# BUTSpeechFIT/TS-ASR-Whisper

Measured on AMD Instinct MI355X. Metric: train utterances/sec (30 s clips) whisper-large-v3-turbo DiCoW, higher is better.
Workload: dtype bf16; 1 GPU; whisper-large-v3-turbo DiCoW fine-tune step, per-GPU batch 16, L=128, decoder frozen, bf16 AMP; global_batch=16, parallelism=dp1, split_streams=False, trainable_params=637306880

## Files before the change

include/dicow_hip.h:

```cpp
#ifndef DICOW_HIP_H
#define DICOW_HIP_H

#include <stdint.h>

#ifdef __cplusplus
extern "C" {
#endif

#define DICOW_OK 0
#define DICOW_ERR_INVALID (-1)
#define DICOW_ERR_LAUNCH (-2)

#define DICOW_ABI_VERSION 7

int dicow_abi_version(void);
int dicow_set_gemm_cus(int n);
int dicow_gemm_dispatch_log(char* buf, int cap);
const char* dicow_last_error(void);

int dicow_cast_f32_to_bf16(const float* src, void* dst, int64_t n, void* stream);
int dicow_cast_transpose_f32_to_bf16(const float* src, void* dst, int64_t ld, void* dst_t, int64_t ld_t, int R, int C,
                                     void* stream);
#define DICOW_CAST_GROUP_MAX 8
typedef struct { const float* src; void* dst; void* dst_t; int R, C; int64_t ld, ld_t; } dicow_cast_problem;
// ... 172 lines not shown
    float* dq_colsum; float* dv_colsum; void* cs_ws; int64_t cs_ws_bytes;
    int q_log2;
    void* fused_ws; int64_t fused_ws_bytes;
    int fused_mode;
} dicow_attn_bwd_args;
int dicow_attn_bwd(const dicow_attn_bwd_args* a, void* stream);
int64_t dicow_attn_bwd_colsum_ws_bytes(int B, int H, int Lq, int Lk);
int64_t dicow_attn_bwd_fused_ws_bytes(int B, int H, int Lq, int Lk);
const char* dicow_attn_bwd_route(const dicow_attn_bwd_args* a);
int dicow_attn_bwd_fused_eligible(int B, int H, int Lq, int Lk, int causal, int fused_mode);
int dicow_attn_bwd_fused_status(const void* fused_ws);


typedef struct {
    const void* logits; int64_t ld; int rows; int V;
    const int64_t* labels; const int64_t* upp_labels;
    int soft;
    const int32_t* ts_index;
    const int32_t* ts_ids;
    const float* ts_w;
    int n_ts;
    float* lse; float* row_loss; int32_t* choice;
    float* loss_sum; float* count;
    void* d_logits;
} dicow_ce_args;
int dicow_ce_loss_fwd(const dicow_ce_args* a, void* stream);
int dicow_ce_loss_bwd(const dicow_ce_args* a, const float* grad_scale, void* stream);

typedef struct {
    const void* logits; int64_t ld; int B, Tn, C;
    const int64_t* labels; int Lc; int blank;
    float* lse;
    float* alpha; float* beta;
    int Smax;
    float* nll; float* tlen;
    float* loss_sum;
    void* d_logits;
} dicow_ctc_args;
int64_t dicow_ctc_ws_bytes(int B, int Tn, int Lc);
int dicow_ctc_loss_fwd(const dicow_ctc_args* a, void* stream);
int dicow_ctc_loss_bwd(const dicow_ctc_args* a, const float* grad_scale, void* stream);

int dicow_embed_fwd(const int64_t* ids, const float* tok, const float* pos, float* out, int B, int Lq, int D, void* stream);
int dicow_embed_bwd(const int64_t* ids, const float* g, float* d_tok, float* d_pos, int B, int Lq, int D, void* stream);

int dicow_gelu_bwd_bf16(const void* g, const void* pre, void* out, int64_t n, void* stream);
int dicow_conv2_col2im_gelu_bwd(const void* dA2, const void* pre1, void* d_pre1, int B, int T2, int C, void* stream);

int64_t dicow_logmel_ws_bytes(int B, int n_samples);
int dicow_logmel(const float* wave, int B, int n_samples, const float* tw_cos, const float* tw_sin, const float* fb,
                 const int* mel_range, int M, float* out, void* ws, int64_t ws_bytes, void* stream);

#define DICOW_NOISE_MIX_CHUNK 8192
int64_t dicow_noise_mix_ws_bytes(int n_plan, int max_len);
int dicow_noise_mix(const float* wave, int64_t ld_wave, float* out, int64_t ld_out, const float* bank, const int64_t* clip_start,
                    const int* clip_len, const int* plan_i, const float* plan_snr, int n_plan, void* ws, int64_t ws_bytes, void* stream);

#define DICOW_DIAR_FRAME 320
#define DICOW_DIAR_BIN 1600
#define DICOW_DIAR_WINDOW 300
#define DICOW_DIAR_MAX_SPEAKERS 64
int64_t dicow_diar_table_ws_bytes(int E);
int64_t dicow_diar_targets_ws_bytes(int n_targets);
int64_t dicow_enrollment_windows_ws_bytes(int64_t n_samples, int n_targets);
int dicow_diar_frame_counts(const int64_t* bounds, const uint64_t* active, int E, int S, int64_t n_samples, int32_t* cnt, int32_t* excl,
                            void* ws, int64_t ws_bytes, void* stream);
int dicow_stno_from_counts(const int32_t* cnt, int S, int64_t n_samples, const int* targets, int n_targets, float* out, int64_t ld_out,
                           void* ws, int64_t ws_bytes, void* stream);
int dicow_enrollment_windows(const int32_t* cnt, const int32_t* excl, int S, int64_t n_samples, const int* targets, int n_targets,
                             int32_t* start, int32_t* count, int32_t* fallback, int32_t* weights, int64_t ld_w, void* ws, int64_t ws_bytes,
                             void* stream);

#define DICOW_ENR_MIX_MAX_TRACKS 8
int dicow_enrollment_mix(float* out, int64_t ld_out, int B, int n, const float* bank, const int64_t* clip_start, const int32_t* plan_dev,
                         const int32_t* plan_host, int n_tracks, const int32_t* clip_len_host, int n_clips, void* stream);

#define DICOW_RESAMPLE_LDS_BYTES 49152
#define DICOW_RESAMPLE_MAX_RATIO 1048576
#define DICOW_RESAMPLE_MAX_CHANNELS 512
int64_t dicow_resample_ws_bytes(int n_segs, int n);
int dicow_resample(const void* in, int in_int16, int C, int channel, int64_t in_frames, float* out, int64_t out_samples, const float* taps_t,
                   const int32_t* first, int o, int n, int width, int S, const int64_t* segs, int n_segs, int frames_per_tile, void* ws,
                   int64_t ws_bytes, void* stream);

#define DICOW_EDIT_MAX_LEN 65535
#define DICOW_EDIT_K 8
#define DICOW_EDIT_LANES 512
#define DICOW_EDIT_LANES_NARROW 64
int64_t dicow_edit_distance_ws_bytes(const int64_t* pairs, int n_pairs);
int dicow_edit_distance(const int32_t* ref_ids, int64_t n_ref, const int32_t* hyp_ids, int64_t n_hyp, const int32_t* ref_iv, const int32_t* hyp_iv,
                        const int64_t* pairs, int n_pairs, int32_t* out, int lanes, int along, void* ws, int64_t ws_bytes, void* stream);

#define DICOW_ORC_MAX_STREAMS 8
#define DICOW_ORC_K 8
#define DICOW_ORC_MAX_WORDS 65527
#define DICOW_ORC_MAX_STATES 4194304
#define DICOW_ORC_MAX_WS_BYTES 1073741824LL
#define DICOW_ORC_DESC_BYTES 288
#define DICOW_ORC_UTT_BYTES 16
int64_t dicow_orc_distance_ws_bytes(const int64_t* problems, int n_problems, const int64_t* utts, const int64_t* streams, int want_assignment);
int dicow_orc_distance(const int32_t* ref_ids, int64_t n_ref, const int32_t* hyp_ids, int64_t n_hyp, const int32_t* ref_iv, const int32_t* hyp_iv,
                       const int64_t* problems, int n_problems, const int64_t* utts, const int64_t* streams, int32_t* out, int32_t* assignment,
                       void* ws, int64_t ws_bytes, void* stream);

#define DICOW_DIAR_SCORE_CHUNK 256
#define DICOW_DIAR_SCORE_ROW 12
#define DICOW_DIAR_SCORE_OUT_WORDS 4232
#define DICOW_DIAR_SCORE_DESC_BYTES 120
#define DICOW_DIAR_SCORE_MAX_E 16777216
#define DICOW_DIAR_SCORE_MAX_TICK 1099511627776LL
#define DICOW_DIAR_SCORE_MAX_WS_BYTES 4294967296LL
int64_t dicow_diar_score_ws_bytes(const int64_t* bounds, int64_t n_bounds, const uint64_t* active, int64_t n_active, const int64_t* unscored,
                                  int64_t n_unscored, const int64_t* problems, int n_problems, int chunk);
int dicow_diar_score(const int64_t* bounds, int64_t n_bounds, const uint64_t* active, int64_t n_active, const int64_t* unscored,
                     int64_t n_unscored, const int64_t* problems, int n_problems, int chunk, int64_t* out, void* ws, int64_t ws_bytes,
                     void* stream);

int dicow_stno_noise_rescale(float* stno, const int* rows, const float* noise, int n_rows, int C, int T, float sd,
                             void* stream);
int dicow_stno_segment_augment(float* stno, const int* segs, const float* coef, int n_seg, int C, int T, void* stream);
int dicow_specaug_joint(const float* mel, const float* stno, float* mel_out, float* stno_out, int B, int M, int T, int sub,
                        int center, int warped, const int* fmask, int n_fmask, const int* tmask, int n_tmask,
                        int n_maskable, void* stream);

typedef struct {
    const void* logits; int in_bf16; int64_t ld; const float* lse; const int* alias;
    const int* rows; const int* cs; const int* decoded_len; const int* last; const float* r_prev;
    float* psi; float* r;
    int n, C, T, blank, eos;
} dicow_ctc_prefix_args;
int dicow_ctc_frame_lse(const void* logits, int in_bf16, int64_t rows, int V1, int64_t ld, float* lse, void* stream);
int dicow_ctc_prefix_init(const void* logits, int in_bf16, int64_t ld, const float* lse, int B, int T, int blank_col, float* r0,
                          void* stream);
int dicow_ctc_prefix_score(const dicow_ctc_prefix_args* a, void* stream);

int dicow_whisper_timestamp_rules(float* scores, int64_t ld, int B, int V, const int64_t* input_ids, int L, int begin_index,
                                  int timestamp_begin, int eos, int no_timestamps, int max_initial_timestamp_index,
                                  int detect_from_logprob, void* stream);

int dicow_repetition_rules(float* scores, int64_t ld, int rows, int V, const int64_t* input_ids, int64_t ids_stride, int L,
                           float penalty, int ngram, void* stream);

int dicow_ctc_greedy_decode(const void* logits, int in_bf16, int64_t batch_stride, int64_t ld, int B, int Tn, int V1, int64_t blank,
                            int64_t pad_id, int* ws, int64_t* out, int64_t out_stride, void* stream);

int dicow_sumsq_f32(const float* x, int64_t n, float* out, void* stream);
int dicow_fabric_emulate(void* buf, int64_t bytes, double gbps, int workgroups, int passes, void* stream);
int dicow_adamw_f32(float* p, const float* g, float* m, float* v, int64_t n, float lr, float beta1, float beta2,
                    float eps, float weight_decay, int step, const float* gnorm_sq, float max_norm, void* stream);
int dicow_adamw_hyper(int* counters, float* hyper, const int* is_pre, int n_runs, int preheat_only, double lr, double mult,
                      int warmup_steps, int max_steps, int cosine, double beta1, double beta2, void* stream);
int dicow_adamw_f32_dev(float* p, const float* g, float* m, float* v, int64_t n, const float* hyper, float beta1, float beta2,
                        float eps, float weight_decay, const float* gnorm_sq, float max_norm, void* stream);

#define DICOW_MT_CHUNK 2048
#define DICOW_MT_MAX_CLASSES 32
#define DICOW_MT_ALIGNED_ALL 1
#define DICOW_MT_ALIGNED_G   2
typedef struct {
    float* p; float* g; float* m; float* v;
    int64_t n;
    int32_t cls;
    int32_t flags;
} dicow_mt_tensor;
typedef struct { int64_t start; int32_t tensor; int32_t len; } dicow_mt_chunk;
typedef struct {
    float decay[DICOW_MT_MAX_CLASSES]; float step_size[DICOW_MT_MAX_CLASSES]; float bc2_sqrt[DICOW_MT_MAX_CLASSES];
    float lerp_w[DICOW_MT_MAX_CLASSES]; float beta2[DICOW_MT_MAX_CLASSES]; float one_minus_beta2[DICOW_MT_MAX_CLASSES];
    float eps[DICOW_MT_MAX_CLASSES];
    int32_t n_classes;
} dicow_mt_adamw_classes;
int dicow_multi_chunk_elems(void);
int dicow_multi_adamw_f32(const dicow_mt_tensor* tensors, const dicow_mt_chunk* chunks, int64_t n_chunks,
                          const dicow_mt_adamw_classes* cls, int cls_base, const float* clip_coef, void* stream);
int64_t dicow_multi_sumsq_ws_bytes(int64_t n_chunks);
int dicow_multi_sumsq_f32(const dicow_mt_tensor* tensors, const dicow_mt_chunk* chunks, int64_t n_chunks, void* ws, int64_t ws_bytes,
                          float* out, float max_norm, void* stream);
int dicow_multi_scale_f32(const dicow_mt_tensor* tensors, const dicow_mt_chunk* chunks, int64_t n_chunks, const float* coef, void* stream);


#ifdef DICOW_EXPERIMENTAL_ABI
#define DICOW_EPI_LNSTAT  2048
#define DICOW_EPI_LNFOLD  4096
#define DICOW_LN_SLOTS 16
int dicow_gemm_nt_lnstat_ok(const dicow_gemm_args* a);
int dicow_lnfold_prep(const float* W, const float* gamma, const float* beta, const float* bias, void* Wf, int64_t ldw, float* c, float* bf,
                      int N, int K, void* stream);
#endif

#ifdef __cplusplus
}
#endif
#endif
```

ts-asr-whisper_amd/_lib.py:

```python
import ctypes as C
import os

_HERE = os.path.dirname(os.path.abspath(__file__))
LIB_PATH = os.environ.get("DICOW_HIP_LIB") or os.path.join(_HERE, "libdicow_hip.so")
_lib = None

c_vp, c_i, c_i64, c_f, c_d = C.c_void_p, C.c_int, C.c_int64, C.c_float, C.c_double


class FddtLnFwdArgs(C.Structure):
    _fields_ = [("h_in", c_vp), ("in_bf16", c_i), ("mode", c_i), ("stno", c_vp), ("stno_bstride", c_i64),
                ("w", c_vp * 4), ("b", c_vp * 4), ("pos", c_vp), ("h_out", c_vp), ("ln_w", c_vp), ("ln_b", c_vp),
                ("y_bf16", c_vp), ("y_f32", c_vp), ("mean", c_vp), ("rstd", c_vp),
                ("rows", c_i), ("T", c_i), ("D", c_i), ("eps", c_f)]


class FddtLnBwdArgs(C.Structure):
    _fields_ = [("h_in", c_vp), ("in_bf16", c_i), ("mode", c_i), ("stno", c_vp), ("stno_bstride", c_i64),
                ("w", c_vp * 4), ("b", c_vp * 4), ("pos", c_vp), ("ln_w", c_vp), ("mean", c_vp), ("rstd", c_vp),
                ("d_y", c_vp), ("dy_f32", c_i), ("g_res", c_vp), ("g_out", c_vp), ("g_out_bf16", c_vp),
                ("dln_w", c_vp), ("dln_b", c_vp), ("dw", c_vp * 4), ("db", c_vp * 4), ("colsum_out", c_vp),
                ("dpos_rows", c_vp), ("rows", c_i), ("T", c_i), ("D", c_i), ("ws", c_vp), ("ws_bytes", c_i64)]


class GemmArgs(C.Structure):
    _fields_ = [("A", c_vp), ("B", c_vp), ("C", c_vp), ("bias", c_vp), ("residual", c_vp), ("aux", c_vp),
                ("M", c_i), ("N", c_i), ("K", c_i),
                ("lda", c_i64), ("ldb", c_i64), ("ldc", c_i64), ("ldr", c_i64), ("ldaux", c_i64),
                ("batch", c_i), ("strideA", c_i64), ("strideB", c_i64), ("strideC", c_i64), ("strideAux", c_i64),
                ("flags", c_i), ("scale", c_f), ("scale_ncols", c_i),
                ("colsum_out", c_vp), ("colsum_ws", c_vp), ("colsum_ws_bytes", c_i64),
                ("fddt_w", c_vp * 4), ("fddt_b", c_vp * 4), ("fddt_rowmask", c_vp),
                ("lnstat", c_vp), ("ln_c", c_vp), ("ln_inv_dim", c_f), ("ln_eps", c_f), ("ln_nslots", c_i)]


class GemmTnArgs(C.Structure):
    _fields_ = [("A", c_vp), ("B", c_vp), ("C", c_vp), ("Mk", c_i), ("N1", c_i), ("N2", c_i),
                ("lda", c_i64), ("ldb", c_i64), ("ldc", c_i64),
                ("batch", c_i), ("strideA", c_i64), ("strideB", c_i64), ("accumulate", c_i),
                ("C_seg", c_vp * 2), ("seg_rows", c_i), ("ws", c_vp), ("ws_bytes", c_i64)]


TN_GROUP_MAX = 24
CAST_GROUP_MAX = 8


class CastProblem(C.Structure):
    _fields_ = [("src", c_vp), ("dst", c_vp), ("dst_t", c_vp), ("R", c_i), ("C", c_i), ("ld", c_i64), ("ld_t", c_i64)]


class GemmTnGroupArgs(C.Structure):
    _fields_ = [("n", c_i), ("p", GemmTnArgs * TN_GROUP_MAX), ("ws", c_vp), ("ws_bytes", c_i64)]


class AttnFwdArgs(C.Structure):
    _fields_ = [("q", c_vp), ("k", c_vp), ("v", c_vp), ("o", c_vp), ("lse", c_vp),
                ("q_bs", c_i64), ("q_rs", c_i64), ("k_bs", c_i64), ("k_rs", c_i64),
                ("v_bs", c_i64), ("v_rs", c_i64), ("o_bs", c_i64), ("o_rs", c_i64),
                ("B", c_i), ("H", c_i), ("Lq", c_i), ("Lk", c_i), ("causal", c_i), ("q_log2", c_i)]


class AttnDecodeArgs(C.Structure):
    _fields_ = [("q", c_vp), ("o", c_vp), ("k", c_vp), ("v", c_vp),
                ("q_rs", c_i64), ("o_rs", c_i64), ("k_bs", c_i64), ("k_rs", c_i64), ("v_bs", c_i64), ("v_rs", c_i64),
                ("anc", c_vp), ("anc_rs", c_i64), ("R", c_i), ("H", c_i), ("Lk", c_i), ("group", c_i), ("n_slots", c_i)]


ATTN_DECODE_MAX_GROUP = 8

NOISE_MIX_CHUNK = 8192

DIAR_FRAME, DIAR_BIN, DIAR_WINDOW, DIAR_MAX_SPEAKERS = 320, 1600, 300, 64

ENR_MIX_MAX_TRACKS = 8

RESAMPLE_LDS_BYTES, RESAMPLE_MAX_RATIO, RESAMPLE_MAX_CHANNELS = 49152, 1 << 20, 512

EDIT_MAX_LEN, EDIT_K, EDIT_LANES, EDIT_LANES_NARROW = 65535, 8, 512, 64

ORC_MAX_STREAMS, ORC_K, ORC_MAX_WORDS, ORC_MAX_STATES, ORC_MAX_WS_BYTES, ORC_DESC_BYTES, ORC_UTT_BYTES = 8, 8, 65527, 1 << 22, 1 << 30, 288, 16

DIAR_SCORE_CHUNK, DIAR_SCORE_ROW, DIAR_SCORE_OUT_WORDS, DIAR_SCORE_DESC_BYTES = 256, 12, 4232, 120
DIAR_SCORE_MAX_E, DIAR_SCORE_MAX_TICK, DIAR_SCORE_MAX_WS_BYTES = 1 << 24, 1 << 40, 1 << 32

LORA_MAX_R, LORA_MAX_SEG = 192, 24
LORA_BLOCK, LORA_OUT_F32, LORA_GELU, LORA_MUL_AUX = 1, 2, 4, 8


class LoraDownArgs(C.Structure):
    _fields_ = [("X", c_vp), ("V", c_vp), ("T", c_vp), ("ldx", c_i64), ("ldv", c_i64), ("ldt", c_i64),
                ("M", c_i), ("K", c_i), ("R", c_i), ("r", c_i), ("flags", c_i)]


class LoraUpArgs(C.Structure):
    _fields_ = [("T", c_vp), ("U", c_vp), ("P", c_vp), ("Y", c_vp), ("aux", c_vp),
                ("ldt", c_i64), ("ldu", c_i64), ("ldp", c_i64), ("ldy", c_i64), ("ldaux", c_i64),
                ("M", c_i), ("N", c_i), ("R", c_i), ("r", c_i), ("flags", c_i), ("seg_scale", c_f * LORA_MAX_SEG)]


class LoraWgradArgs(C.Structure):
    _fields_ = [("T", c_vp), ("P", c_vp), ("G", c_vp * LORA_MAX_SEG), ("ldt", c_i64), ("ldp", c_i64), ("g_rs", c_i64), ("g_cs", c_i64),
                ("M", c_i), ("N", c_i), ("R", c_i), ("r", c_i), ("flags", c_i), ("scale", c_f), ("accumulate", c_i),
                ("ws", c_vp), ("ws_bytes", c_i64)]


class AttnBwdArgs(C.Structure):
    _fields_ = [("q", c_vp), ("k", c_vp), ("v", c_vp), ("o", c_vp), ("d_o", c_vp), ("lse", c_vp), ("delta", c_vp),
                ("dq", c_vp), ("dk", c_vp), ("dv", c_vp),
                ("q_bs", c_i64), ("q_rs", c_i64), ("k_bs", c_i64), ("k_rs", c_i64), ("v_bs", c_i64), ("v_rs", c_i64),
                ("o_bs", c_i64), ("o_rs", c_i64), ("do_bs", c_i64), ("do_rs", c_i64),
                ("dq_bs", c_i64), ("dq_rs", c_i64), ("dk_bs", c_i64), ("dk_rs", c_i64), ("dv_bs", c_i64), ("dv_rs", c_i64),
                ("B", c_i), ("H", c_i), ("Lq", c_i), ("Lk", c_i), ("causal", c_i), ("dq_scale", c_f),
                ("dq_colsum", c_vp), ("dv_colsum", c_vp), ("cs_ws", c_vp), ("cs_ws_bytes", c_i64), ("q_log2", c_i),
                ("fused_ws", c_vp), ("fused_ws_bytes", c_i64), ("fused_mode", c_i)]


class CeArgs(C.Structure):
    _fields_ = [("logits", c_vp), ("ld", c_i64), ("rows", c_i), ("V", c_i), ("labels", c_vp), ("upp_labels", c_vp),
                ("soft", c_i), ("ts_index", c_vp), ("ts_ids", c_vp), ("ts_w", c_vp), ("n_ts", c_i),
                ("lse", c_vp), ("row_loss", c_vp), ("choice", c_vp), ("loss_sum", c_vp), ("count", c_vp),
                ("d_logits", c_vp)]


class CtcArgs(C.Structure):
    _fields_ = [("logits", c_vp), ("ld", c_i64), ("B", c_i), ("Tn", c_i), ("C", c_i), ("labels", c_vp), ("Lc", c_i),
                ("blank", c_i), ("lse", c_vp), ("alpha", c_vp), ("beta", c_vp), ("Smax", c_i), ("nll", c_vp), ("tlen", c_vp),
                ("loss_sum", c_vp), ("d_logits", c_vp)]


class CtcPrefixArgs(C.Structure):
    _fields_ = [("logits", c_vp), ("in_bf16", c_i), ("ld", c_i64), ("lse", c_vp), ("alias", c_vp), ("rows", c_vp), ("cs", c_vp),
                ("decoded_len", c_vp), ("last", c_vp), ("r_prev", c_vp), ("psi", c_vp), ("r", c_vp), ("n", c_i), ("C", c_i),
                ("T", c_i), ("blank", c_i), ("eos", c_i)]


MT_MAX_CLASSES = 32


class MtAdamwClasses(C.Structure):
    _fields_ = [("decay", c_f * MT_MAX_CLASSES), ("step_size", c_f * MT_MAX_CLASSES), ("bc2_sqrt", c_f * MT_MAX_CLASSES),
                ("lerp_w", c_f * MT_MAX_CLASSES), ("beta2", c_f * MT_MAX_CLASSES), ("one_minus_beta2", c_f * MT_MAX_CLASSES),
                ("eps", c_f * MT_MAX_CLASSES), ("n_classes", C.c_int32)]


EPI_BIAS, EPI_GELU, EPI_RESIDUAL, EPI_OUT_F32, EPI_SCALE_N, EPI_GELU_BWD, EPI_ACCUM = 1, 2, 4, 8, 16, 32, 64
EPI_GELU_DAUX, EPI_MUL_AUX, EPI_COLSUM, EPI_FDDT = 128, 256, 512, 1024
EPI_LNSTAT, EPI_LNFOLD, LN_SLOTS = 2048, 4096, 16

_SIGS = {
    "dicow_set_gemm_cus": [c_i],
    "dicow_cast_transpose_group": [C.POINTER(CastProblem), c_i, c_vp],
    "dicow_gemm_dispatch_log": [c_vp, c_i],
    "dicow_cast_f32_to_bf16": [c_vp, c_vp, c_i64, c_vp],
    "dicow_cast_transpose_f32_to_bf16": [c_vp, c_vp, c_i64, c_vp, c_i64, c_i, c_i, c_vp],
    "dicow_conv_weight_pack": [c_vp, c_vp, c_vp, c_i, c_i, c_i, c_vp],
    "dicow_conv_weight_unpack_grad": [c_vp, c_vp, c_i, c_i, c_i, c_vp],
    "dicow_mel_to_timemajor": [c_vp, c_vp, c_i, c_i, c_i, c_vp],
    "dicow_colsum_bf16": [c_vp, c_i64, c_vp, c_i, c_i, c_vp, c_i64, c_vp],
    "dicow_sum_over_batch": [c_vp, c_vp, c_i, c_i64, c_vp],
    "dicow_scb_split": [c_vp, c_vp, c_vp, c_vp, c_i64, c_i, c_i, c_i, c_vp],
    "dicow_scb_merge_fwd": [c_vp, c_vp, c_vp, c_vp, c_i, c_i, c_i, c_vp],
    "dicow_scb_gate_bwd": [c_vp, c_vp, c_vp, c_vp, c_vp, c_i, c_i, c_i, c_vp, c_i64, c_vp],
    "dicow_scb_merge_bwd": [c_vp, c_vp, c_vp, c_i64, c_vp, c_vp, c_i, c_i, c_i, c_vp],
    "dicow_fddt_ln_fwd": [C.POINTER(FddtLnFwdArgs), c_vp],
    "dicow_fddt_ln_bwd": [C.POINTER(FddtLnBwdArgs), c_vp],
    "dicow_fddt_full_combine_fwd": [c_vp, c_vp, c_i, c_vp, c_i64, c_i, c_vp, c_i, c_i, c_i, c_vp],
    "dicow_fddt_full_combine_bwd": [c_vp, c_vp, c_i64, c_i, c_vp, c_vp, c_i, c_i, c_i, c_vp],
    "dicow_gemm_nt": [C.POINTER(GemmArgs), c_vp],
    "dicow_gemm_nt_is_persistent": [C.POINTER(GemmArgs)],
    "dicow_gemm_tn": [C.POINTER(GemmTnArgs), c_vp],
    "dicow_gemm_tn_group": [C.POINTER(GemmTnGroupArgs), c_vp],
    "dicow_attn_fwd": [C.POINTER(AttnFwdArgs), c_vp],
    "dicow_attn_decode": [C.POINTER(AttnDecodeArgs), c_vp],
    "dicow_lora_down": [C.POINTER(LoraDownArgs), c_vp],
    "dicow_lora_up": [C.POINTER(LoraUpArgs), c_vp],
    "dicow_lora_wgrad": [C.POINTER(LoraWgradArgs), c_vp],
    "dicow_attn_bwd": [C.POINTER(AttnBwdArgs), c_vp],
    "dicow_attn_bwd_fused_status": [c_vp],
    "dicow_attn_bwd_fused_eligible": [c_i, c_i, c_i, c_i, c_i, c_i],
    "dicow_ce_loss_fwd": [C.POINTER(CeArgs), c_vp],
    "dicow_ce_loss_bwd": [C.POINTER(CeArgs), c_vp, c_vp],
    "dicow_ctc_loss_fwd": [C.POINTER(CtcArgs), c_vp],
    "dicow_ctc_loss_bwd": [C.POINTER(CtcArgs), c_vp, c_vp],
    "dicow_embed_fwd": [c_vp, c_vp, c_vp, c_vp, c_i, c_i, c_i, c_vp],
    "dicow_embed_bwd": [c_vp, c_vp, c_vp, c_vp, c_i, c_i, c_i, c_vp],
    "dicow_gelu_bwd_bf16": [c_vp, c_vp, c_vp, c_i64, c_vp],
    "dicow_conv2_col2im_gelu_bwd": [c_vp, c_vp, c_vp, c_i, c_i, c_i, c_vp],
    "dicow_logmel": [c_vp, c_i, c_i, c_vp, c_vp, c_vp, c_vp, c_i, c_vp, c_vp, c_i64, c_vp],
    "dicow_stno_noise_rescale": [c_vp, c_vp, c_vp, c_i, c_i, c_i, c_f, c_vp],
    "dicow_stno_segment_augment": [c_vp, c_vp, c_vp, c_i, c_i, c_i, c_vp],
    "dicow_specaug_joint": [c_vp, c_vp, c_vp, c_vp, c_i, c_i, c_i, c_i, c_i, c_i, c_vp, c_i, c_vp, c_i, c_i, c_vp],
    "dicow_ctc_frame_lse": [c_vp, c_i, c_i64, c_i, c_i64, c_vp, c_vp],
    "dicow_ctc_prefix_init": [c_vp, c_i, c_i64, c_vp, c_i, c_i, c_i, c_vp, c_vp],
    "dicow_ctc_prefix_score": [C.POINTER(CtcPrefixArgs), c_vp],
    "dicow_whisper_timestamp_rules": [c_vp, c_i64, c_i, c_i, c_vp, c_i, c_i, c_i, c_i, c_i, c_i, c_i, c_vp],
    "dicow_repetition_rules": [c_vp, c_i64, c_i, c_i, c_vp, c_i64, c_i, c_f, c_i, c_vp],
    "dicow_ctc_greedy_decode": [c_vp, c_i, c_i64, c_i64, c_i, c_i, c_i, c_i64, c_i64, c_vp, c_vp, c_i64, c_vp],
    "dicow_noise_mix": [c_vp, c_i64, c_vp, c_i64, c_vp, c_vp, c_vp, c_vp, c_vp, c_i, c_vp, c_i64, c_vp],
    "dicow_diar_frame_counts": [c_vp, c_vp, c_i, c_i, c_i64, c_vp, c_vp, c_vp, c_i64, c_vp],
    "dicow_stno_from_counts": [c_vp, c_i, c_i64, c_vp, c_i, c_vp, c_i64, c_vp, c_i64, c_vp],
    "dicow_enrollment_windows": [c_vp, c_vp, c_i, c_i64, c_vp, c_i, c_vp, c_vp, c_vp, c_vp, c_i64, c_vp, c_i64, c_vp],
    "dicow_enrollment_mix": [c_vp, c_i64, c_i, c_i, c_vp, c_vp, c_vp, c_vp, c_i, c_vp, c_i, c_vp],
    "dicow_resample": [c_vp, c_i, c_i, c_i, c_i64, c_vp, c_i64, c_vp, c_vp, c_i, c_i, c_i, c_i, c_vp, c_i, c_i, c_vp, c_i64, c_vp],
    "dicow_edit_distance": [c_vp, c_i64, c_vp, c_i64, c_vp, c_vp, c_vp, c_i, c_vp, c_i, c_i, c_vp, c_i64, c_vp],
    "dicow_orc_distance": [c_vp, c_i64, c_vp, c_i64, c_vp, c_vp, c_vp, c_i, c_vp, c_vp, c_vp, c_vp, c_vp, c_i64, c_vp],
    "dicow_diar_score": [c_vp, c_i64, c_vp, c_i64, c_vp, c_i64, c_vp, c_i, c_i, c_vp, c_vp, c_i64, c_vp],
    "dicow_sumsq_f32": [c_vp, c_i64, c_vp, c_vp],
    "dicow_fabric_emulate": [c_vp, c_i64, c_d, c_i, c_i, c_vp],
    "dicow_adamw_f32": [c_vp, c_vp, c_vp, c_vp, c_i64, c_f, c_f, c_f, c_f, c_f, c_i, c_vp, c_f, c_vp],
    "dicow_adamw_hyper": [c_vp, c_vp, c_vp, c_i, c_i, c_d, c_d, c_i, c_i, c_i, c_d, c_d, c_vp],
    "dicow_adamw_f32_dev": [c_vp, c_vp, c_vp, c_vp, c_i64, c_vp, c_f, c_f, c_f, c_f, c_vp, c_f, c_vp],
    "dicow_multi_chunk_elems": [],
    "dicow_multi_adamw_f32": [c_vp, c_vp, c_i64, C.POINTER(MtAdamwClasses), c_i, c_vp, c_vp],
    "dicow_multi_sumsq_f32": [c_vp, c_vp, c_i64, c_vp, c_i64, c_vp, c_f, c_vp],
    "dicow_multi_scale_f32": [c_vp, c_vp, c_i64, c_vp, c_vp],
}


_SIGS_EXPERIMENTAL = {
    "dicow_gemm_nt_lnstat_ok": [C.POINTER(GemmArgs)],
    "dicow_lnfold_prep": [c_vp, c_vp, c_vp, c_vp, c_vp, c_i64, c_vp, c_vp, c_i, c_i, c_vp],
}


class DicowError(RuntimeError):
    pass


def lib():
    global _lib
    if _lib is None:
        if not os.path.exists(LIB_PATH):
            raise DicowError(f"{LIB_PATH} is missing: build it with ts-asr-whisper_amd/csrc/build.sh "
                             "(or __graft_entry__.build()); there is no CPU fallback")
        l = C.CDLL(LIB_PATH)
        l.dicow_abi_version.restype = c_i
        l.dicow_last_error.restype = C.c_char_p
        for name, at in _SIGS.items():
            fn = getattr(l, name)
            fn.argtypes = at
            fn.restype = c_i
        for name, at in _SIGS64.items():
            fn = getattr(l, name)
            fn.argtypes = at
            fn.restype = c_i64
        for name, at in _SIGS_STR.items():
            fn = getattr(l, name)
            fn.argtypes = at
            fn.restype = C.c_char_p
        l._dicow_experimental = True
        for name, at in _SIGS_EXPERIMENTAL.items():
            try:
                fn = getattr(l, name)
            except AttributeError:
                l._dicow_experimental = False
                continue
            fn.argtypes = at
            fn.restype = c_i
        _lib = l
    return _lib


def has_experimental():
    return bool(lib()._dicow_experimental)


_SIGS64 = {
    "dicow_colsum_ws_bytes": [c_i, c_i],
    "dicow_gemm_nt_colsum_ws_bytes": [c_i, c_i],
    "dicow_attn_bwd_colsum_ws_bytes": [c_i, c_i, c_i, c_i],
    "dicow_attn_bwd_fused_ws_bytes": [c_i, c_i, c_i, c_i],
    "dicow_fddt_ln_bwd_ws_bytes": [c_i, c_i],
    "dicow_gemm_tn_ws_bytes": [C.POINTER(GemmTnArgs)],
    "dicow_gemm_nt_splitk_ws_bytes": [C.POINTER(GemmArgs)],
    "dicow_gemm_tn_group_ws_bytes": [C.POINTER(GemmTnGroupArgs)],
    "dicow_logmel_ws_bytes": [c_i, c_i],
    "dicow_scb_gate_bwd_ws_bytes": [],
    "dicow_ctc_ws_bytes": [c_i, c_i, c_i],
    "dicow_multi_sumsq_ws_bytes": [c_i64],
    "dicow_lora_wgrad_ws_bytes": [c_i, c_i, c_i, c_i, c_i],
    "dicow_noise_mix_ws_bytes": [c_i, c_i],
    "dicow_diar_table_ws_bytes": [c_i],
    "dicow_diar_targets_ws_bytes": [c_i],
    "dicow_enrollment_windows_ws_bytes": [c_i64, c_i],
    "dicow_resample_ws_bytes": [c_i, c_i],
    "dicow_edit_distance_ws_bytes": [c_vp, c_i],
    "dicow_orc_distance_ws_bytes": [c_vp, c_i, c_vp, c_vp, c_i],
    "dicow_diar_score_ws_bytes": [c_vp, c_i64, c_vp, c_i64, c_vp, c_i64, c_vp, c_i, c_i],
}


_SIGS_STR = {
    "dicow_fddt_ln_fwd_route": [C.POINTER(FddtLnFwdArgs)],
    "dicow_fddt_ln_bwd_route": [C.POINTER(FddtLnBwdArgs)],
    "dicow_attn_fwd_route": [C.POINTER(AttnFwdArgs)],
    "dicow_attn_bwd_route": [C.POINTER(AttnBwdArgs)],
}


def declared_symbols():
    return ["dicow_abi_version", "dicow_last_error"] + list(_SIGS) + list(_SIGS64) + list(_SIGS_STR)


def check(rc, what):
    if rc != 0:
        raise DicowError(f"{what} failed ({rc}): {lib().dicow_last_error().decode()}")


def ptr(t):
    return None if t is None else t.data_ptr()


def stream():
    import torch
    return torch.cuda.current_stream().cuda_stream


def call(name, *args):
    check(getattr(lib(), name)(*args), name)


def call_struct(name, st):
    check(getattr(lib(), name)(C.byref(st), stream()), name)
```

ts-asr-whisper_amd/csrc/elementwise.hip:

```cpp
#include <stdarg.h>
#include "common.h"

static thread_local char g_err[512] = "";

void dicow_set_error(const char* fmt, ...) {
    va_list ap;
    va_start(ap, fmt);
    vsnprintf(g_err, sizeof(g_err), fmt, ap);
    va_end(ap);
}

extern "C" int dicow_abi_version(void) { return DICOW_ABI_VERSION; }
extern "C" const char* dicow_last_error(void) { return g_err; }

__global__ void cast_f32_bf16_kernel(const float* __restrict__ src, unsigned short* __restrict__ dst, int64_t n) {
    const int64_t n4 = n >> 2;
    const int64_t stride = (int64_t)gridDim.x * blockDim.x;
    for (int64_t i = (int64_t)blockIdx.x * blockDim.x + threadIdx.x; i < n4; i += stride) {
        const float4 v = reinterpret_cast<const float4*>(src)[i];
        reinterpret_cast<uint2*>(dst)[i] = make_uint2(pack_bf16x2(v.x, v.y), pack_bf16x2(v.z, v.w));
    }
    for (int64_t i = (n4 << 2) + (int64_t)blockIdx.x * blockDim.x + threadIdx.x; i < n; i += stride)
        dst[i] = f2bfbits(src[i]);
}
// ... 358 lines not shown
    const int64_t id = ids[row];
    const float* gr = g + (int64_t)row * D;
    for (int i = threadIdx.x; i < D; i += blockDim.x) {
        const float v = gr[i];
        if (d_tok) atomicAdd(d_tok + id * D + i, v);
        if (d_pos) atomicAdd(d_pos + (int64_t)l * D + i, v);
    }
}

extern "C" int dicow_embed_bwd(const int64_t* ids, const float* g, float* d_tok, float* d_pos, int B, int Lq, int D, void* stream) {
    DICOW_REQUIRE(ids && g && B > 0 && Lq > 0 && D > 0, "embed_bwd: bad args");
    if (!d_tok && !d_pos) return DICOW_OK;
    hipLaunchKernelGGL(embed_bwd_kernel, dim3(B * Lq), dim3(256), 0, (hipStream_t)stream, ids, g, d_tok, d_pos, Lq, D);
    DICOW_CHECK_LAUNCH("embed_bwd");
    return DICOW_OK;
}

__global__ void gelu_bwd_bf16_kernel(const unsigned short* __restrict__ g, const unsigned short* __restrict__ pre,
                                     unsigned short* __restrict__ out, int64_t n) {
    const int64_t n4 = n >> 2;
    for (int64_t i = (int64_t)blockIdx.x * blockDim.x + threadIdx.x; i < n4; i += (int64_t)gridDim.x * blockDim.x) {
        const uint2 a = reinterpret_cast<const uint2*>(g)[i], b = reinterpret_cast<const uint2*>(pre)[i];
        const float r0 = __uint_as_float(a.x << 16) * gelu_erf_grad(__uint_as_float(b.x << 16));
        const float r1 = __uint_as_float(a.x & 0xffff0000u) * gelu_erf_grad(__uint_as_float(b.x & 0xffff0000u));
        const float r2 = __uint_as_float(a.y << 16) * gelu_erf_grad(__uint_as_float(b.y << 16));
        const float r3 = __uint_as_float(a.y & 0xffff0000u) * gelu_erf_grad(__uint_as_float(b.y & 0xffff0000u));
        reinterpret_cast<uint2*>(out)[i] = make_uint2(pack_bf16x2(r0, r1), pack_bf16x2(r2, r3));
    }
}

extern "C" int dicow_gelu_bwd_bf16(const void* g, const void* pre, void* out, int64_t n, void* stream) {
    DICOW_REQUIRE(g && pre && out && n > 0 && n % 4 == 0, "gelu_bwd_bf16: bad args (n %% 4)");
    int grid = (int)((n / 4 + 255) / 256); if (grid > 8192) grid = 8192;
    hipLaunchKernelGGL(gelu_bwd_bf16_kernel, dim3(grid), dim3(256), 0, (hipStream_t)stream, (const unsigned short*)g,
                       (const unsigned short*)pre, (unsigned short*)out, n);
    DICOW_CHECK_LAUNCH("gelu_bwd_bf16");
    return DICOW_OK;
}

__global__ void conv2_col2im_gelu_bwd_kernel(const unsigned short* __restrict__ dA2, const unsigned short* __restrict__ pre1,
                                             unsigned short* __restrict__ d_pre1, int T2, int C) {
    const int b = blockIdx.y, s = blockIdx.x;
    const int p = s + 1;
    const unsigned short* base = dA2 + (int64_t)b * T2 * 3 * C;
    const unsigned short* src0 = nullptr; const unsigned short* src1 = nullptr;
    if (p & 1) {
        const int t = (p - 1) >> 1;
        if (t < T2) src0 = base + (int64_t)t * 3 * C + C;
    } else {
        const int t = p >> 1;
        if (t < T2) src0 = base + (int64_t)t * 3 * C;
        if (t - 1 >= 0) src1 = base + (int64_t)(t - 1) * 3 * C + 2 * C;
    }
    const int64_t off = ((int64_t)b * 2 * T2 + s) * C;
    for (int c = threadIdx.x * 2; c < C; c += blockDim.x * 2) {
        float g0 = 0.f, g1 = 0.f;
        if (src0) { const unsigned u = *reinterpret_cast<const unsigned*>(src0 + c); g0 += __uint_as_float(u << 16); g1 += __uint_as_float(u & 0xffff0000u); }
        if (src1) { const unsigned u = *reinterpret_cast<const unsigned*>(src1 + c); g0 += __uint_as_float(u << 16); g1 += __uint_as_float(u & 0xffff0000u); }
        if (pre1) {
            const unsigned pu = *reinterpret_cast<const unsigned*>(pre1 + off + c);
            g0 *= gelu_erf_grad(__uint_as_float(pu << 16));
            g1 *= gelu_erf_grad(__uint_as_float(pu & 0xffff0000u));
        }
        *reinterpret_cast<unsigned*>(d_pre1 + off + c) = pack_bf16x2(g0, g1);
    }
}

extern "C" int dicow_conv2_col2im_gelu_bwd(const void* dA2, const void* pre1, void* d_pre1, int B, int T2, int C, void* stream) {
    DICOW_REQUIRE(dA2 && d_pre1 && B > 0 && T2 > 0 && C % 2 == 0, "conv2_col2im_gelu_bwd: bad args");
    hipLaunchKernelGGL(conv2_col2im_gelu_bwd_kernel, dim3(2 * T2, B), dim3(256), 0, (hipStream_t)stream,
                       (const unsigned short*)dA2, (const unsigned short*)pre1, (unsigned short*)d_pre1, T2, C);
    DICOW_CHECK_LAUNCH("conv2_col2im_gelu_bwd");
    return DICOW_OK;
}

#define SUMSQ_MAX_BLOCKS 2048
__device__ float g_sumsq_part[SUMSQ_MAX_BLOCKS];
__device__ unsigned g_sumsq_ticket = 0;

__global__ void __launch_bounds__(256) sumsq_kernel(const float* __restrict__ x, int64_t n, float* __restrict__ out) {
    __shared__ float red[4];
    __shared__ bool last;
    float s = 0.f;
    const int64_t n4 = n >> 2;
    for (int64_t i = (int64_t)blockIdx.x * blockDim.x + threadIdx.x; i < n4; i += (int64_t)gridDim.x * blockDim.x) {
        const float4 v = reinterpret_cast<const float4*>(x)[i];
        s += v.x * v.x + v.y * v.y + v.z * v.z + v.w * v.w;
    }
    for (int64_t i = (n4 << 2) + (int64_t)blockIdx.x * blockDim.x + threadIdx.x; i < n; i += (int64_t)gridDim.x * blockDim.x)
        s += x[i] * x[i];
    s = wave_sum(s);
    if ((threadIdx.x & 63) == 0) red[threadIdx.x >> 6] = s;
    __syncthreads();
    if (threadIdx.x == 0) {
        g_sumsq_part[blockIdx.x] = (red[0] + red[1]) + (red[2] + red[3]);
        __threadfence();
        last = atomicAdd(&g_sumsq_ticket, 1u) == gridDim.x - 1;
    }
    __syncthreads();
    if (!last) return;
    __threadfence();
    float t = 0.f;
    for (int i = threadIdx.x; i < (int)gridDim.x; i += 256) t += __builtin_nontemporal_load(&g_sumsq_part[i]);
    t = wave_sum(t);
    if ((threadIdx.x & 63) == 0) red[threadIdx.x >> 6] = t;
    __syncthreads();
    if (threadIdx.x == 0) {
        out[0] += (red[0] + red[1]) + (red[2] + red[3]);
        g_sumsq_ticket = 0;
    }
}

__global__ void __launch_bounds__(256) fabric_emulate_kernel(f32x4_t* buf, int64_t n16, double ticks_per_f4_per_block, int passes) {
    const int64_t per = (n16 + gridDim.x - 1) / gridDim.x, lo = per * blockIdx.x, hi = lo + per < n16 ? lo + per : n16;
    const long long t0 = wall_clock64();
    int64_t done = 0;
    for (int p = 0; p < passes; ++p)
        for (int64_t i = lo; i < hi; i += 256 * 16) {
            f32x4_t v[16];
#pragma unroll
            for (int k = 0; k < 16; ++k) { const int64_t j = i + k * 256 + threadIdx.x; if (j < hi) v[k] = __builtin_nontemporal_load(buf + j); }
#pragma unroll
            for (int k = 0; k < 16; ++k) { const int64_t j = i + k * 256 + threadIdx.x; if (j < hi) __builtin_nontemporal_store(v[k], buf + j); }
            done += (hi - i < 256 * 16 ? hi - i : 256 * 16);
            const long long due = t0 + (long long)((double)done * ticks_per_f4_per_block / passes);
            while (wall_clock64() < due) __builtin_amdgcn_s_sleep(32);
        }
}

extern "C" int dicow_fabric_emulate(void* buf, int64_t bytes, double gbps, int workgroups, int passes, void* stream) {
    DICOW_REQUIRE(buf && bytes > 0 && bytes % 16 == 0 && gbps > 0.0 && workgroups > 0 && workgroups <= 1024 && passes > 0 && passes <= 8,
                  "fabric_emulate: bad arguments");
    const int64_t n16 = bytes / 16;
    const double ticks_total = (double)bytes / (gbps * 1e9) * 1e8;
    const double per_block_f4 = (double)((n16 + workgroups - 1) / workgroups);
    hipLaunchKernelGGL(fabric_emulate_kernel, dim3(workgroups), dim3(256), 0, (hipStream_t)stream, reinterpret_cast<f32x4_t*>(buf), n16,
                       ticks_total / per_block_f4, passes);
    DICOW_CHECK_LAUNCH("fabric_emulate");
    return DICOW_OK;
}

extern "C" int dicow_sumsq_f32(const float* x, int64_t n, float* out, void* stream) {
    DICOW_REQUIRE(x && out && n > 0, "sumsq_f32: bad args");
    int grid = (int)((n / 4 + 255) / 256); if (grid < 1) grid = 1; if (grid > SUMSQ_MAX_BLOCKS) grid = SUMSQ_MAX_BLOCKS;
    hipLaunchKernelGGL(sumsq_kernel, dim3(grid), dim3(256), 0, (hipStream_t)stream, x, n, out);
    DICOW_CHECK_LAUNCH("sumsq_f32");
    return DICOW_OK;
}

#ifndef ADAMW_NT
#define ADAMW_NT 0
#endif
typedef __attribute__((ext_vector_type(4))) float f32x4a_t;
__global__ void adamw_kernel(float* __restrict__ p, const float* __restrict__ g, float* __restrict__ m, float* __restrict__ v,
                             int64_t n, float lr, float b1, float b2, float eps, float wd, float bc1, float bc2,
                             const float* __restrict__ gnorm_sq, float max_norm, const float* __restrict__ hyper) {
    if (hyper) { lr = hyper[0]; bc1 = hyper[1]; bc2 = hyper[2]; }
    float clip = 1.f;
    if (gnorm_sq && max_norm > 0.f) {
        const float c = max_norm / (sqrtf(gnorm_sq[0]) + 1e-6f);
        clip = c < 1.f ? c : 1.f;
    }
    const int64_t n4 = n >> 2;
    for (int64_t i = (int64_t)blockIdx.x * blockDim.x + threadIdx.x; i < n4; i += (int64_t)gridDim.x * blockDim.x) {
        float4 pp, gg, mm, vv;
        if (ADAMW_NT & 1) {
            const f32x4a_t p_ = __builtin_nontemporal_load(reinterpret_cast<const f32x4a_t*>(p) + i), g_ = __builtin_nontemporal_load(reinterpret_cast<const f32x4a_t*>(g) + i);
            const f32x4a_t m_ = __builtin_nontemporal_load(reinterpret_cast<const f32x4a_t*>(m) + i), v_ = __builtin_nontemporal_load(reinterpret_cast<const f32x4a_t*>(v) + i);
            pp = make_float4(p_.x, p_.y, p_.z, p_.w); gg = make_float4(g_.x, g_.y, g_.z, g_.w);
            mm = make_float4(m_.x, m_.y, m_.z, m_.w); vv = make_float4(v_.x, v_.y, v_.z, v_.w);
        } else {
            pp = reinterpret_cast<float4*>(p)[i]; gg = reinterpret_cast<const float4*>(g)[i];
            mm = reinterpret_cast<float4*>(m)[i]; vv = reinterpret_cast<float4*>(v)[i];
        }
        float* pa = &pp.x; float* ga = &gg.x; float* ma = &mm.x; float* va = &vv.x;
#pragma unroll
        for (int e = 0; e < 4; ++e) {
            const float gr = ga[e] * clip;
            pa[e] *= 1.f - lr * wd;
            ma[e] = b1 * ma[e] + (1.f - b1) * gr;
            va[e] = b2 * va[e] + (1.f - b2) * gr * gr;
            const float denom = sqrtf(va[e]) / sqrtf(bc2) + eps;
            pa[e] -= (lr / bc1) * (ma[e] / denom);
        }
        if (ADAMW_NT & 2) {
            __builtin_nontemporal_store(f32x4a_t{pp.x, pp.y, pp.z, pp.w}, reinterpret_cast<f32x4a_t*>(p) + i);
            __builtin_nontemporal_store(f32x4a_t{mm.x, mm.y, mm.z, mm.w}, reinterpret_cast<f32x4a_t*>(m) + i);
            __builtin_nontemporal_store(f32x4a_t{vv.x, vv.y, vv.z, vv.w}, reinterpret_cast<f32x4a_t*>(v) + i);
        } else {
            reinterpret_cast<float4*>(p)[i] = pp; reinterpret_cast<float4*>(m)[i] = mm; reinterpret_cast<float4*>(v)[i] = vv;
        }
    }
    for (int64_t i = (n4 << 2) + (int64_t)blockIdx.x * blockDim.x + threadIdx.x; i < n; i += (int64_t)gridDim.x * blockDim.x) {
        const float gr = g[i] * clip;
        float pv = p[i] * (1.f - lr * wd);
        const float mv = b1 * m[i] + (1.f - b1) * gr, vv2 = b2 * v[i] + (1.f - b2) * gr * gr;
        pv -= (lr / bc1) * (mv / (sqrtf(vv2) / sqrtf(bc2) + eps));
        p[i] = pv; m[i] = mv; v[i] = vv2;
    }
}

extern "C" int dicow_adamw_f32(float* p, const float* g, float* m, float* v, int64_t n, float lr, float beta1, float beta2,
                               float eps, float weight_decay, int step, const float* gnorm_sq, float max_norm, void* stream) {
    DICOW_REQUIRE(p && g && m && v && n > 0 && step >= 1, "adamw_f32: bad args");
    const float bc1 = 1.f - powf(beta1, (float)step), bc2 = 1.f - powf(beta2, (float)step);
    int grid = (int)((n / 4 + 255) / 256); if (grid < 1) grid = 1; if (grid > 4096) grid = 4096;
    hipLaunchKernelGGL(adamw_kernel, dim3(grid), dim3(256), 0, (hipStream_t)stream, p, g, m, v, n, lr, beta1, beta2, eps,
                       weight_decay, bc1, bc2, gnorm_sq, max_norm, (const float*)nullptr);
    DICOW_CHECK_LAUNCH("adamw_f32");
    return DICOW_OK;
}

__global__ void adamw_hyper_kernel(int* __restrict__ counters, float* __restrict__ hyper, const int* __restrict__ is_pre, int n_runs,
                                   int preheat_only, double lr, double mult, int warmup, int max_steps, int cosine, double b1, double b2) {
    const int k = counters[0] + 1;
    __syncthreads();
    if (threadIdx.x == 0) counters[0] = k;
    const int ss = k - 1;
    double l = lr;
    if (ss < warmup) l = lr * (double)ss / (double)(warmup > 1 ? warmup : 1);
    else if (cosine && max_steps > 0) {
        const double prog = (double)(ss - warmup) / (double)((max_steps - warmup) > 1 ? (max_steps - warmup) : 1);
        const double c = 0.5 * (1.0 + cos(3.14159265358979323846 * prog));
        l = lr * (c > 0.0 ? c : 0.0);
    }
    for (int i = threadIdx.x; i < n_runs; i += blockDim.x) {
        const int pre = is_pre[i];
        if (preheat_only && !pre) continue;
        const int t = counters[1 + i] + 1;
        counters[1 + i] = t;
        hyper[3 * i] = (float)(l * (pre ? mult : 1.0));
        hyper[3 * i + 1] = (float)(1.0 - pow(b1, (double)t));
        hyper[3 * i + 2] = (float)(1.0 - pow(b2, (double)t));
    }
}

extern "C" int dicow_adamw_hyper(int* counters, float* hyper, const int* is_pre, int n_runs, int preheat_only, double lr, double mult,
                                 int warmup_steps, int max_steps, int cosine, double beta1, double beta2, void* stream) {
    DICOW_REQUIRE(counters && hyper && is_pre && n_runs > 0, "adamw_hyper: bad args");
    const int block = n_runs >= 1024 ? 1024 : (n_runs + 63) / 64 * 64;
    hipLaunchKernelGGL(adamw_hyper_kernel, dim3(1), dim3(block), 0, (hipStream_t)stream, counters, hyper, is_pre, n_runs, preheat_only,
                       lr, mult, warmup_steps, max_steps, cosine, beta1, beta2);
    DICOW_CHECK_LAUNCH("adamw_hyper");
    return DICOW_OK;
}

extern "C" int dicow_adamw_f32_dev(float* p, const float* g, float* m, float* v, int64_t n, const float* hyper, float beta1,
                                   float beta2, float eps, float weight_decay, const float* gnorm_sq, float max_norm, void* stream) {
    DICOW_REQUIRE(p && g && m && v && n > 0 && hyper, "adamw_f32_dev: bad args");
    int grid = (int)((n / 4 + 255) / 256); if (grid < 1) grid = 1; if (grid > 4096) grid = 4096;
    hipLaunchKernelGGL(adamw_kernel, dim3(grid), dim3(256), 0, (hipStream_t)stream, p, g, m, v, n, 0.f, beta1, beta2, eps,
                       weight_decay, 1.f, 1.f, gnorm_sq, max_norm, hyper);
    DICOW_CHECK_LAUNCH("adamw_f32_dev");
    return DICOW_OK;
}

__device__ __forceinline__ float4 bf4_to_f4(uint2 u) {
    return make_float4(__uint_as_float(u.x << 16), __uint_as_float(u.x & 0xffff0000u), __uint_as_float(u.y << 16), __uint_as_float(u.y & 0xffff0000u));
}
__global__ void scb_split_kernel(const float* __restrict__ hf, unsigned short* __restrict__ q_in, unsigned short* __restrict__ kv_in,
                                 unsigned short* __restrict__ cat, int64_t td, int D, int64_t ldcat, int Bp) {
    const int64_t n4 = (int64_t)Bp * td / 4;
    for (int64_t i = (int64_t)blockIdx.x * blockDim.x + threadIdx.x; i < n4; i += (int64_t)gridDim.x * blockDim.x) {
        const int64_t e = i * 4, b = e / td, off = e - b * td;
        const float4 m = *reinterpret_cast<const float4*>(hf + (2 * b) * td + off);
        const float4 r = *reinterpret_cast<const float4*>(hf + (2 * b + 1) * td + off);
        const uint2 mb = make_uint2(pack_bf16x2(m.x, m.y), pack_bf16x2(m.z, m.w));
        *reinterpret_cast<uint2*>(q_in + e) = mb;
        *reinterpret_cast<uint2*>(kv_in + e) = make_uint2(pack_bf16x2(r.x, r.y), pack_bf16x2(r.z, r.w));
        const int64_t row = e / D; const int col = (int)(e - row * D);
        *reinterpret_cast<uint2*>(cat + row * ldcat + D + col) = mb;
    }
}
__global__ void scb_merge_fwd_kernel(const float* __restrict__ hf, const unsigned short* __restrict__ upd, const float* __restrict__ gate,
                                     float* __restrict__ out, int64_t td, int Bp) {
    const float tg = tanhf(gate[0]);
    const int64_t n4 = (int64_t)2 * Bp * td / 4;
    for (int64_t i = (int64_t)blockIdx.x * blockDim.x + threadIdx.x; i < n4; i += (int64_t)gridDim.x * blockDim.x) {
        const int64_t e = i * 4, slot = e / td, off = e - slot * td;
        float4 v = *reinterpret_cast<const float4*>(hf + e);
        if ((slot & 1) == 0) {
            const float4 u = bf4_to_f4(*reinterpret_cast<const uint2*>(upd + (slot >> 1) * td + off));
            v.x += u.x * tg; v.y += u.y * tg; v.z += u.z * tg; v.w += u.w * tg;
        }
        *reinterpret_cast<float4*>(out + e) = v;
    }
}
__global__ void __launch_bounds__(256) scb_gate_bwd_kernel(const float* __restrict__ g, const unsigned short* __restrict__ upd,
                                                           const float* __restrict__ gate, unsigned short* __restrict__ d_upd,
                                                           float* __restrict__ partial, int64_t td, int Bp) {
    __shared__ float red[4];
    const float tg = tanhf(gate[0]);
    const int64_t n4 = (int64_t)Bp * td / 4;
    float acc = 0.f;
    for (int64_t i = (int64_t)blockIdx.x * blockDim.x + threadIdx.x; i < n4; i += (int64_t)gridDim.x * blockDim.x) {
        const int64_t e = i * 4, b = e / td, off = e - b * td;
        const float4 gq = *reinterpret_cast<const float4*>(g + (2 * b) * td + off);
        const float4 u = bf4_to_f4(*reinterpret_cast<const uint2*>(upd + e));
        acc += (gq.x * u.x + gq.y * u.y) + (gq.z * u.z + gq.w * u.w);
        *reinterpret_cast<uint2*>(d_upd + e) = make_uint2(pack_bf16x2(gq.x * tg, gq.y * tg), pack_bf16x2(gq.z * tg, gq.w * tg));
    }
    acc = wave_sum(acc);
    if ((threadIdx.x & 63) == 0) red[threadIdx.x >> 6] = acc;
    __syncthreads();
    if (threadIdx.x == 0) partial[blockIdx.x] = (red[0] + red[1]) + (red[2] + red[3]);
}
__global__ void scb_gate_finish_kernel(const float* __restrict__ partial, int n, const float* __restrict__ gate, float* __restrict__ d_gate) {
    __shared__ float red[256];
    float t = 0.f;
    for (int i = threadIdx.x; i < n; i += 256) t += partial[i];
    red[threadIdx.x] = t;
    __syncthreads();
    for (int o = 128; o > 0; o >>= 1) { if ((int)threadIdx.x < o) red[threadIdx.x] += red[threadIdx.x + o]; __syncthreads(); }
    if (threadIdx.x == 0) { const float tg = tanhf(gate[0]); d_gate[0] += red[0] * (1.f - tg * tg); }
}
__global__ void scb_merge_bwd_kernel(const float* __restrict__ g, const float* __restrict__ d_qin, const unsigned short* __restrict__ d_cat,
                                     int64_t ldcat, const float* __restrict__ d_kvin, float* __restrict__ gin, int64_t td, int D, int Bp) {
    const int64_t n4 = (int64_t)2 * Bp * td / 4;
    for (int64_t i = (int64_t)blockIdx.x * blockDim.x + threadIdx.x; i < n4; i += (int64_t)gridDim.x * blockDim.x) {
        const int64_t e = i * 4, slot = e / td, off = e - slot * td, b = slot >> 1, pe = b * td + off;
        float4 v = *reinterpret_cast<const float4*>(g + e);
        if ((slot & 1) == 0) {
            const float4 a = *reinterpret_cast<const float4*>(d_qin + pe);
            const int64_t row = pe / D; const int col = (int)(pe - row * D);
            const float4 c = bf4_to_f4(*reinterpret_cast<const uint2*>(d_cat + row * ldcat + D + col));
            v.x += a.x + c.x; v.y += a.y + c.y; v.z += a.z + c.z; v.w += a.w + c.w;
        } else {
            const float4 a = *reinterpret_cast<const float4*>(d_kvin + pe);
            v.x += a.x; v.y += a.y; v.z += a.z; v.w += a.w;
        }
        *reinterpret_cast<float4*>(gin + e) = v;
    }
}
static int scb_grid(int64_t n4) { int64_t g = (n4 + 255) / 256; return (int)(g > 2048 ? 2048 : (g < 1 ? 1 : g)); }
#define SCB_CHECK(name) DICOW_REQUIRE(Bp > 0 && T > 0 && D > 0 && D % 4 == 0, name ": bad shape")
extern "C" int dicow_scb_split(const float* hf, void* q_in, void* kv_in, void* cat, int64_t ldcat, int Bp, int T, int D, void* stream) {
    DICOW_REQUIRE(hf && q_in && kv_in && cat && ldcat >= 2 * D && ldcat % 4 == 0, "scb_split: bad args");
    SCB_CHECK("scb_split");
    const int64_t td = (int64_t)T * D;
    hipLaunchKernelGGL(scb_split_kernel, dim3(scb_grid(Bp * td / 4)), dim3(256), 0, (hipStream_t)stream, hf, (unsigned short*)q_in,
                       (unsigned short*)kv_in, (unsigned short*)cat, td, D, ldcat, Bp);
    DICOW_CHECK_LAUNCH("scb_split");
    return DICOW_OK;
}
extern "C" int dicow_scb_merge_fwd(const float* hf, const void* upd, const float* gate, float* out, int Bp, int T, int D, void* stream) {
    DICOW_REQUIRE(hf && upd && gate && out, "scb_merge_fwd: null operand");
    SCB_CHECK("scb_merge_fwd");
    const int64_t td = (int64_t)T * D;
    hipLaunchKernelGGL(scb_merge_fwd_kernel, dim3(scb_grid(2 * Bp * td / 4)), dim3(256), 0, (hipStream_t)stream, hf,
                       (const unsigned short*)upd, gate, out, td, Bp);
    DICOW_CHECK_LAUNCH("scb_merge_fwd");
    return DICOW_OK;
}
extern "C" int64_t dicow_scb_gate_bwd_ws_bytes(void) { return 1024 * 4; }
extern "C" int dicow_scb_gate_bwd(const float* g, const void* upd, const float* gate, void* d_upd, float* d_gate, int Bp, int T, int D,
                                  void* ws, int64_t ws_bytes, void* stream) {
    DICOW_REQUIRE(g && upd && gate && d_upd && ws && ws_bytes >= 1024 * 4, "scb_gate_bwd: bad args (ws: dicow_scb_gate_bwd_ws_bytes)");
    SCB_CHECK("scb_gate_bwd");
    const int64_t td = (int64_t)T * D;
    int grid = scb_grid(Bp * td / 4); if (grid > 1024) grid = 1024;
    hipLaunchKernelGGL(scb_gate_bwd_kernel, dim3(grid), dim3(256), 0, (hipStream_t)stream, g, (const unsigned short*)upd, gate,
                       (unsigned short*)d_upd, (float*)ws, td, Bp);
    DICOW_CHECK_LAUNCH("scb_gate_bwd");
    if (d_gate) {
        hipLaunchKernelGGL(scb_gate_finish_kernel, dim3(1), dim3(256), 0, (hipStream_t)stream, (const float*)ws, grid, gate, d_gate);
        DICOW_CHECK_LAUNCH("scb_gate_finish");
    }
    return DICOW_OK;
}
extern "C" int dicow_scb_merge_bwd(const float* g, const float* d_qin, const void* d_cat, int64_t ldcat, const float* d_kvin, float* gin,
                                   int Bp, int T, int D, void* stream) {
    DICOW_REQUIRE(g && d_qin && d_cat && d_kvin && gin && ldcat >= 2 * D && ldcat % 4 == 0, "scb_merge_bwd: bad args");
    SCB_CHECK("scb_merge_bwd");
    const int64_t td = (int64_t)T * D;
    hipLaunchKernelGGL(scb_merge_bwd_kernel, dim3(scb_grid(2 * Bp * td / 4)), dim3(256), 0, (hipStream_t)stream, g, d_qin,
                       (const unsigned short*)d_cat, ldcat, d_kvin, gin, td, D, Bp);
    DICOW_CHECK_LAUNCH("scb_merge_bwd");
    return DICOW_OK;
}

#ifdef DICOW_EXPERIMENTS
__global__ void __launch_bounds__(256) lnfold_prep_kernel(const float* __restrict__ W, const float* __restrict__ gamma,
                                                          const float* __restrict__ beta, const float* __restrict__ bias,
                                                          unsigned short* __restrict__ Wf, int64_t ldw, float* __restrict__ c,
                                                          float* __restrict__ bf, int K) {
    __shared__ float red[2][4];
    const int n = blockIdx.x;
    const float* w = W + (int64_t)n * K;
    unsigned short* o = Wf + (int64_t)n * ldw;
    float sc = 0.f, sb = 0.f;
    for (int k = threadIdx.x * 2; k < K; k += 512) {
        const float w0 = w[k], w1 = w[k + 1];
        const unsigned pf = pack_bf16x2(w0 * gamma[k], w1 * gamma[k + 1]);
        *reinterpret_cast<unsigned*>(o + k) = pf;
        sc += __uint_as_float(pf << 16) + __uint_as_float(pf & 0xffff0000u);
        const unsigned pw = pack_bf16x2(w0, w1);
        sb = fmaf(beta[k], __uint_as_float(pw << 16), sb);
        sb = fmaf(beta[k + 1], __uint_as_float(pw & 0xffff0000u), sb);
    }
    sc = wave_sum_dpp(sc); sb = wave_sum_dpp(sb);
    if ((threadIdx.x & 63) == 0) { red[0][threadIdx.x >> 6] = sc; red[1][threadIdx.x >> 6] = sb; }
    __syncthreads();
    if (threadIdx.x == 0) {
        c[n] = (red[0][0] + red[0][1]) + (red[0][2] + red[0][3]);
        bf[n] = (bias ? bias[n] : 0.f) + ((red[1][0] + red[1][1]) + (red[1][2] + red[1][3]));
    }
// ... 13 lines not shown
```

ts-asr-whisper_amd/engine.py:

```python
import contextlib
import os
from types import SimpleNamespace as NS

import torch

from . import _lib as L
from . import ops

BF16, F32 = torch.bfloat16, torch.float32
CLS = ("silence_linear", "target_linear", "non_target_linear", "overlap_linear")


def _e(shape, dtype, dev):
    return torch.empty(shape, dtype=dtype, device=dev)


def _ceil(a, b):
    return (a + b - 1) // b * b


WGRAD_SIDE_STREAM = os.environ.get("DICOW_WGRAD_STREAM", "0") == "1"
WGRAD_STREAM_PRIORITY = int(os.environ.get("DICOW_WGRAD_STREAM_PRIORITY", "-1"))
_WGRAD_STREAMS = {}


def wgrad_stream(dev):
    cur = torch.cuda.current_stream(dev)
    key = (dev.index, cur.cuda_stream)
    st = _WGRAD_STREAMS.get(key)
    if st is None:
        st = _WGRAD_STREAMS[key] = torch.cuda.Stream(device=dev, priority=WGRAD_STREAM_PRIORITY)
    return st


SPLIT_FWD = os.environ.get("DICOW_SPLIT_FWD", "1") != "0"
SPLIT_FWD_MIN_ROWS = int(os.environ.get("DICOW_SPLIT_FWD_MIN_ROWS", "16000"))
SPLIT_DEC = os.environ.get("DICOW_SPLIT_DEC", "1") != "0"
SPLIT_BWD = os.environ.get("DICOW_SPLIT_BWD", "1") != "0"
SPLIT_BWD_WGRAD = os.environ.get("DICOW_SPLIT_BWD_WGRAD", "alt")
SPLIT_BWD_MEM_FRACTION = float(os.environ.get("DICOW_SPLIT_BWD_MEM_FRACTION", "0.6"))
SPLIT_IN_CAPTURE = os.environ.get("DICOW_SPLIT_IN_CAPTURE", "0") == "1"
SPLIT_FWD_PARTS = int(os.environ.get("DICOW_SPLIT_FWD_PARTS", "2"))
_FWD_STREAMS = {}


def _split_allowed():
    return SPLIT_IN_CAPTURE or not torch.cuda.is_current_stream_capturing()


def fwd_side_stream(dev, k=0):
    cur = torch.cuda.current_stream(dev)
    key = (dev.index, cur.cuda_stream, k)
    st = _FWD_STREAMS.get(key)
    if st is None:
        st = _FWD_STREAMS[key] = torch.cuda.Stream(device=dev, priority=-1)
    return st


def _fwd_parts(B, T, dev):
    n = SPLIT_FWD_PARTS if (SPLIT_FWD_PARTS > 2 and B % SPLIT_FWD_PARTS == 0) else 2
    main_st, Bp = torch.cuda.current_stream(dev), B // n
    parts = []
    for k in range(n):
        st = main_st if k == 0 else fwd_side_stream(dev, k - 1)
        if k:
            st.wait_stream(main_st)
        parts.append((st, slice(k * Bp * T, (k + 1) * Bp * T), slice(k * Bp, (k + 1) * Bp)))
    return main_st, parts, Bp


class GradSink:

    def __init__(self, params, dev, extra_rows=None):
        self.index, self.direct = {}, {}
        off = 0
        extra_rows = extra_rows or {}
        for p in params:
            if p is None or not p.requires_grad or id(p) in self.index or id(p) in self.direct:
                continue
            if getattr(p, "_direct_grad", None) is not None:
                self.direct[id(p)] = p._direct_grad
                continue
            n = p.numel() + extra_rows.get(id(p), 0)
            self.index[id(p)] = (off, p.shape, p.numel())
            off += _ceil(n, 64)
        self.flat = torch.zeros(max(off, 1), dtype=F32, device=dev)

    def get(self, p):
        if p is None:
            return None
        if id(p) in self.direct:
            return self.direct[id(p)]
        if id(p) not in self.index:
            return None
        off, shape, n = self.index[id(p)]
        return self.flat[off:off + n].view(shape)

    def result(self, p):
        return None if (p is None or id(p) in self.direct) else self.get(p)

    def is_direct(self, p):
        return p is not None and id(p) in self.direct

    def raw(self, p, n):
        if id(p) in self.direct:
            d = self.direct[id(p)]
            assert d.numel() == n, "GradSink.raw: a flat-store gradient has no padding rows"
            return d.view(-1)
        off, _, _ = self.index[id(p)]
        return self.flat[off:off + n]


class LinW:
    __slots__ = ("w", "wt", "b", "N", "K")


_BIAS_COPIES = None


def prep_linear(weights, biases, dev, need_t=True, n_pad=None, scale_info=None, bias_buf=None):
    K = weights[0].shape[1]
    Ns = [w.shape[0] for w in weights]
    N = sum(Ns)
    Np = N if n_pad is None else n_pad
    lw = LinW()
    lw.N, lw.K = Np, K
    lw.w = torch.zeros(Np, K, dtype=BF16, device=dev) if Np != N else _e((Np, K), BF16, dev)
    lw.wt = (torch.zeros(K, Np, dtype=BF16, device=dev) if Np != N else _e((K, Np), BF16, dev)) if need_t else None
    off = 0
    for w, n in zip(weights, Ns):
        ops.cast_transpose_bf16(w.detach(), out=lw.w[off:off + n], out_t=None if lw.wt is None else lw.wt[:, off:off + n],
                                ld=K, ld_t=Np)
        off += n
    if biases is None or all(b is None for b in biases):
        lw.b = None
    else:
        if bias_buf is not None and _BIAS_COPIES is not None and len(Ns) > 1:
            off = 0
            for b, n in zip(biases, Ns):
                if b is not None:
                    _BIAS_COPIES.append((bias_buf[off:off + n], b.detach()))
                off += n
            lw.b = bias_buf
        else:
            parts = [(b.detach() if b is not None else torch.zeros(n, dtype=F32, device=dev)) for b, n in zip(biases, Ns)]
            lw.b = parts[0] if len(parts) == 1 else torch.cat(parts)
    return lw


def prep_attention(att, dev, fuse_qkv=True, bias_buf=None):
    a = NS()
    if fuse_qkv:
        a.qkv = prep_linear([att.q_proj.weight, att.k_proj.weight, att.v_proj.weight],
                            [att.q_proj.bias, None, att.v_proj.bias], dev, bias_buf=bias_buf)
    else:
        a.q = prep_linear([att.q_proj.weight], [att.q_proj.bias], dev)
        a.kv = prep_linear([att.k_proj.weight, att.v_proj.weight], [None, att.v_proj.bias], dev)
    a.o = prep_linear([att.out_proj.weight], [att.out_proj.bias], dev)
    return a


def fddt_ptrs(fddt, cfg):
    if fddt is None:
        return ops.MODE_NONE, (None,) * 4, (None,) * 4
    w, b = [], []
    for c in CLS:
        m = getattr(fddt, c, None)
        if fddt.bias_only:
            w.append(None)
            b.append(None if m is None else m)
        else:
            w.append(None if m is None else m.weight)
            b.append(None if m is None else m.bias)
    return (ops.MODE_BIAS if fddt.bias_only else ops.MODE_DIAG), tuple(w), tuple(b)


def fddt_is_full(fddt):
    return fddt is not None and not fddt.is_diagonal


def prep_full_fddt(fddt, dev):
    D = fddt.d_model
    w = NS(use=0)
    w.Wc = torch.zeros(4 * D, D, dtype=BF16, device=dev)
    w.Wct = torch.zeros(D, 4 * D, dtype=BF16, device=dev)
    w.bias = torch.zeros(4 * D, dtype=F32, device=dev)
    for c, name in enumerate(CLS):
        m = getattr(fddt, name, None)
        if m is not None:
            w.use |= 1 << c
            ops.cast_transpose_bf16(m.weight.detach(), out=w.Wc[c * D:(c + 1) * D], out_t=w.Wct[:, c * D:(c + 1) * D], ld=D, ld_t=4 * D)
            w.bias[c * D:(c + 1) * D] = m.bias.detach()
    return w


def full_fddt_fwd(w, h, stno, bstride, rows, T, D):
    hb = h if h.dtype == BF16 else ops.cast_bf16(h)
    y4 = _e((rows, 4 * D), BF16, h.device)
    ops.gemm_nt(hb, w.Wc, y4, rows, 4 * D, D, bias=w.bias)
    out = _e((rows, D), F32, h.device)
    L.call("dicow_fddt_full_combine_fwd", y4.data_ptr(), h.data_ptr(), int(h.dtype == BF16), stno.data_ptr(), bstride, w.use,
           out.data_ptr(), rows, T, D, L.stream())
    return out, hb


def full_fddt_bwd(fddt, w, hb, g, stno, bstride, G, rows, T, D):
    dev = g.device
    d_y4 = torch.zeros(rows, 4 * D, dtype=BF16, device=dev)
    gh = _e((rows, D), F32, dev)
    L.call("dicow_fddt_full_combine_bwd", g.data_ptr(), stno.data_ptr(), bstride, w.use, d_y4.data_ptr(), gh.data_ptr(), rows, T, D,
           L.stream())
    ops.gemm_nt(d_y4, w.Wct, gh, rows, D, 4 * D, flags=L.EPI_ACCUM)
    for c, name in enumerate(CLS):
        m = getattr(fddt, name, None)
        if m is None:
            continue
        sl = d_y4[:, c * D:(c + 1) * D]
        if G.get(m.bias) is not None:
            ops.colsum_bf16(sl, G.get(m.bias))
        if G.get(m.weight) is not None:
            ops.gemm_tn(sl, hb, G.get(m.weight), rows, D, D, lda=4 * D, ldb=D, ldc=D)
    return gh


QK_LOG2 = os.environ.get("DICOW_QK_LOG2", "1") != "0"
FUSE_NEXT_FDDT = True
LN_FOLD = os.environ.get("DICOW_LN_FOLD", "0") == "1"
Q_SCALE = 0.125 * (ops.LOG2E if QK_LOG2 else 1.0)


def linear_fwd(x, lw, M, out_dtype=BF16, residual=None, gelu_aux=None, flags=0, scale=1.0, scale_ncols=0, out=None, fddt=None):
    dev = x.device
    if out is None:
        out = _e((M, lw.N), out_dtype, dev)
    ops.gemm_nt(x, lw.w, out, M, lw.N, lw.K, bias=lw.b, residual=residual, aux=gelu_aux,
                flags=flags | ((L.EPI_GELU | L.EPI_GELU_DAUX) if gelu_aux is not None else 0), scale=scale, scale_ncols=scale_ncols, fddt=fddt)
    return out


def linear_dgrad(dy, lw, M, aux=None, out=None, out_dtype=BF16, accumulate=False, dy_cols=None, colsum_out=None):
    N = lw.N if dy_cols is None else dy_cols
    if out is None:
        out = _e((M, lw.K), out_dtype, dy.device)
    flags = (L.EPI_MUL_AUX if aux is not None else 0) | (L.EPI_ACCUM if accumulate else 0)
    ops.gemm_nt(dy, lw.wt, out, M, lw.K, N, lda=dy.stride(0), ldb=lw.wt.stride(0), aux=aux, flags=flags, colsum_out=colsum_out)
    return out


def _first_writer(*params):
    if not params or not all(getattr(p, "_grad_overwrite", False) for p in params):
        return False
    for p in params:
        p._grad_overwrite = False
    return True


def linear_wgrad(dy, x, gw, M, n_rows=None, group=None, param=None):
    if gw is None:
        return
    N = dy.shape[1] if n_rows is None else n_rows
    acc = not (param is not None and _first_writer(param))
    if group is not None:
        group.add(dy, x, gw, M, N, x.shape[1], lda=dy.stride(0), ldb=x.stride(0), ldc=gw.stride(0), accumulate=acc)
        return
    ops.gemm_tn(dy, x, gw, M, N, x.shape[1], lda=dy.stride(0), ldb=x.stride(0), ldc=gw.stride(0), accumulate=acc)


class LoraW:
    __slots__ = ("mods", "r", "s", "R", "K", "N", "A", "Bt")

    def refresh(self):
        r = self.r
        for j, m in enumerate(self.mods):
            ops.cast_transpose_bf16(m.lora_A.weight.detach(), out=self.A[j * r:(j + 1) * r], ld=self.K)
            ops.cast_transpose_bf16(m.lora_B.weight.detach(), out_t=self.Bt[j * r:(j + 1) * r], ld_t=self.N)


def prep_lora(mods, dev):
    has = [hasattr(m, "lora_A") for m in mods]
    if not any(has):
        return None
    if not all(has) or len({(m.r, m.lora_alpha) for m in mods}) != 1:
        raise NotImplementedError("LoRA: the projections of one fused Linear (q/k/v, k/v) must all carry adapters of one rank and alpha")
    la = LoraW()
    la.mods, la.r, la.s = list(mods), mods[0].r, mods[0].scaling
    la.R, la.K, la.N = la.r * len(mods), mods[0].in_features, mods[0].out_features
    la.A, la.Bt = _e((la.R, la.K), BF16, dev), _e((la.R, la.N), BF16, dev)
    la.refresh()
    return la


def lora_fwd(x, la, y, M, q_scale=None, gelu=False, gelu_aux=None):
    if la is None:
        return None
    t = _e((M, la.R), BF16, x.device)
    ops.lora_down(x, la.A, t, la.r)
    scales = [la.s] * len(la.mods)
    if q_scale is not None:
        scales[0] *= q_scale
    ops.lora_up(t, la.Bt, y, y, la.r, scales, block=True, gelu=gelu, aux=gelu_aux)
    return t


def lora_bwd(dy, x, t, la, M, G, dx=None, mul_aux=None, dx_out=None):
    if la is None:
        return
    r = la.r
    dt = _e((M, la.R), BF16, dy.device)
    ops.lora_down(dy, la.Bt, dt, r, block=True)
    gB = [G.get(m.lora_B.weight) for m in la.mods]
    gA = [G.get(m.lora_A.weight) for m in la.mods]
    if any(g is not None for g in gB):
        ops.lora_wgrad(t, dy, gB, r, la.s, block=True, g_rs=1, g_cs=r,
                       accumulate=not _first_writer(*[m.lora_B.weight for m, g in zip(la.mods, gB) if g is not None]))
    if any(g is not None for g in gA):
        ops.lora_wgrad(dt, x, gA, r, la.s, g_rs=la.K,
                       accumulate=not _first_writer(*[m.lora_A.weight for m, g in zip(la.mods, gA) if g is not None]))
    if dx is not None:
        ops.lora_up(dt, la.A, dx, dx if dx_out is None else dx_out, r, [la.s], mul_aux=mul_aux is not None, aux=mul_aux)


def qkv_wgrad(d_qkv, x, gq, gk, gv, M, D, group=None, params=None):
    if gq is not None and gk is not None and gv is not None and D % 128 == 0:
        acc = not (params is not None and _first_writer(*params))
        kw = dict(lda=d_qkv.stride(0), ldb=x.stride(0), ldc=D, C_seg=(gk, gv), seg_rows=D, accumulate=acc)
        if group is not None:
            group.add(d_qkv, x, gq, M, 3 * D, D, **kw)
        else:
            ops.gemm_tn(d_qkv, x, gq, M, 3 * D, D, **kw)
        return
    pq, pk, pv = params if params is not None else (None, None, None)
    linear_wgrad(d_qkv[:, :D], x, gq, M, group=group, param=pq)
    linear_wgrad(d_qkv[:, D:2 * D], x, gk, M, group=group, param=pk)
    linear_wgrad(d_qkv[:, 2 * D:], x, gv, M, group=group, param=pv)


def bias_grad(dy, gb):
    if gb is not None:
        ops.colsum_bf16(dy, gb)


def heads(t, B, Lx, H):
    return t.as_strided((B, Lx, H, 64), (Lx * t.stride(0), t.stride(0), 64, 1), t.storage_offset())


def plain_layer_fwd(lyr, w, h, B, T, H, F_):
    rows, D = h.shape
    dev = h.device
    s = NS(h_in=h)
    s.xln, s.mean, s.rstd = _e((rows, D), BF16, dev), _e((rows,), F32, dev), _e((rows,), F32, dev)
    ln = lyr.self_attn_layer_norm
    ops.fddt_ln_fwd(h, rows, D, mode=ops.MODE_NONE, ln_w=ln.weight.detach(), ln_b=ln.bias.detach(), y_bf16=s.xln, mean=s.mean,
                    rstd=s.rstd)
    s.qkv = linear_fwd(s.xln, w.att.qkv, rows, flags=L.EPI_SCALE_N, scale=Q_SCALE, scale_ncols=D)
    s.o, s.lse = _e((rows, D), BF16, dev), _e((B, H, T), F32, dev)
    ops.attn_fwd(heads(s.qkv[:, :D], B, T, H), heads(s.qkv[:, D:2 * D], B, T, H), heads(s.qkv[:, 2 * D:], B, T, H),
                 heads(s.o, B, T, H), s.lse, q_log2=QK_LOG2)
    s.h2 = linear_fwd(s.o, w.att.o, rows, out_dtype=F32, residual=h)
    s.xln2, s.mean2, s.rstd2 = _e((rows, D), BF16, dev), _e((rows,), F32, dev), _e((rows,), F32, dev)
    ln2 = lyr.final_layer_norm
    ops.fddt_ln_fwd(s.h2, rows, D, mode=ops.MODE_NONE, ln_w=ln2.weight.detach(), ln_b=ln2.bias.detach(), y_bf16=s.xln2,
                    mean=s.mean2, rstd=s.rstd2)
    s.u = _e((rows, F_), BF16, dev)
    s.a = linear_fwd(s.xln2, w.fc1, rows, gelu_aux=s.u)
    return linear_fwd(s.a, w.fc2, rows, out_dtype=F32, residual=s.h2), s


def plain_layer_bwd(lyr, w, s, gb, G, B, T, H):
    rows, D = gb.shape
    dev = gb.device
    g = gb.float()
    bias_grad(gb, G.get(lyr.fc2.bias))
    linear_wgrad(gb, s.a, G.get(lyr.fc2.weight), rows)
    d_u = linear_dgrad(gb, w.fc2, rows, aux=s.u, colsum_out=G.get(lyr.fc1.bias))
    linear_wgrad(d_u, s.xln2, G.get(lyr.fc1.weight), rows)
    d_xln2 = linear_dgrad(d_u, w.fc1, rows)
    g2, g2b = _e((rows, D), F32, dev), _e((rows, D), BF16, dev)
    ln2, att = lyr.final_layer_norm, lyr.self_attn
    ops.fddt_ln_bwd(s.h2, rows, D, mode=ops.MODE_NONE, ln_w=ln2.weight.detach(), mean=s.mean2, rstd=s.rstd2, d_y=d_xln2, g_res=g,
                    g_out=g2, g_out_bf16=g2b, dln_w=G.get(ln2.weight), dln_b=G.get(ln2.bias), colsum_out=G.get(att.out_proj.bias))
    linear_wgrad(g2b, s.o, G.get(att.out_proj.weight), rows)
    d_o = linear_dgrad(g2b, w.att.o, rows)
    d_qkv, delta = _e((rows, 3 * D), BF16, dev), _e((2, B, H, T), F32, dev)
    qkv = s.qkv
    ops.attn_bwd(heads(qkv[:, :D], B, T, H), heads(qkv[:, D:2 * D], B, T, H), heads(qkv[:, 2 * D:], B, T, H),
                 heads(s.o, B, T, H), heads(d_o, B, T, H), s.lse, delta, heads(d_qkv[:, :D], B, T, H),
                 heads(d_qkv[:, D:2 * D], B, T, H), heads(d_qkv[:, 2 * D:], B, T, H), dq_scale=0.125, q_log2=QK_LOG2,
                 dq_colsum=G.get(att.q_proj.bias), dv_colsum=G.get(att.v_proj.bias))
    qkv_wgrad(d_qkv, s.xln, G.get(att.q_proj.weight), G.get(att.k_proj.weight), G.get(att.v_proj.weight), rows, D)
    d_xln = linear_dgrad(d_qkv, w.att.qkv, rows)
    g0 = _e((rows, D), F32, dev)
    ln = lyr.self_attn_layer_norm
    ops.fddt_ln_bwd(s.h_in, rows, D, mode=ops.MODE_NONE, ln_w=ln.weight.detach(), mean=s.mean, rstd=s.rstd, d_y=d_xln, g_res=g2,
                    g_out=g0, dln_w=G.get(ln.weight), dln_b=G.get(ln.bias))
    return g0


def conv_stem_fwd(enc, W, input_features, need_grad=True):
    dev = input_features.device
    B, M, Tin = input_features.shape
    T, D = Tin // 2, enc.conv1.weight.shape[0]
    xt = torch.zeros(B * (Tin + 2) * M + W.k1, dtype=BF16, device=dev)
    ops.mel_to_timemajor(input_features.to(F32), out=xt)
    g1p = _e((B, Tin + 2, D), BF16, dev)
    g1p[:, 0].zero_()
    g1p[:, Tin + 1].zero_()
    pre1 = _e((B, Tin, D), BF16, dev) if need_grad else None
    ops.gemm_nt(xt, W.conv1, g1p[:, 1:], Tin, D, W.k1, lda=M, bias=enc.conv1.bias.detach(), aux=pre1, flags=L.EPI_GELU,
                batch=B, strideA=(Tin + 2) * M, strideC=(Tin + 2) * D, strideAux=Tin * D)
    x2 = _e((B * T, D), BF16, dev)
    pre2 = _e((B * T, D), BF16, dev) if need_grad else None
    ops.gemm_nt(g1p, W.conv2, x2, T, D, 3 * D, lda=2 * D, bias=enc.conv2.bias.detach(), aux=pre2, flags=L.EPI_GELU,
                batch=B, strideA=(Tin + 2) * D, strideC=T * D, strideAux=T * D)
    return x2, NS(xt=xt, g1p=g1p, pre1=pre1, pre2=pre2, B=B, T=T, M=M)


def conv_stem_bwd(enc, W, st, d_x2, G):
    dev = d_x2.device
    B, T, M = st.B, st.T, st.M
    Tin, rows, D = 2 * T, B * T, d_x2.shape[1]
    d_pre2 = _e((rows, D), BF16, dev)
    ops.gelu_bwd_bf16(d_x2, st.pre2, d_pre2)
    bias_grad(d_pre2, G.get(enc.conv2.bias))
    gw2 = G.get(enc.conv2.weight)
    if gw2 is not None:
        tmp = torch.zeros(D, 3 * D, dtype=F32, device=dev)
        ops.gemm_tn(d_pre2, st.g1p, tmp, T, D, 3 * D, lda=D, ldb=2 * D, batch=B, strideA=T * D, strideB=(Tin + 2) * D)
        ops.conv_weight_unpack_grad(tmp, gw2)
    dA2 = _e((rows, 3 * D), BF16, dev)
    ops.gemm_nt(d_pre2, W.conv2_t, dA2, rows, 3 * D, D)
    d_pre1 = _e((B, Tin, D), BF16, dev)
    ops.conv2_col2im_gelu_bwd(dA2, st.pre1, d_pre1, B, T, D)
    bias_grad(d_pre1.view(B * Tin, D), G.get(enc.conv1.bias))
    gw1 = G.get(enc.conv1.weight)
    if gw1 is not None:
        tmp = torch.zeros(D, W.k1, dtype=F32, device=dev)
        ops.gemm_tn(d_pre1, st.xt, tmp, Tin, D, W.k1, lda=D, ldb=M, batch=B, strideA=Tin * D, strideB=(Tin + 2) * M)
        ops.conv_weight_unpack_grad(tmp, gw1)


class EncoderEngine:
    def __init__(self, enc):
        self.enc = enc
        self.cfg = enc.config

    def prepare(self):
        enc, cfg = self.enc, self.cfg
        dev = enc.conv1.weight.device
        D, M = cfg.d_model, cfg.num_mel_bins
        W = NS()
        W.k1 = _ceil(3 * M, 64)
        W.conv1, W.conv1_t = ops.conv_weight_pack(enc.conv1.weight.detach(), W.k1, want_t=True)
        W.conv2, W.conv2_t = ops.conv_weight_pack(enc.conv2.weight.detach(), 3 * D, want_t=True)
        W.layers = []
        global _BIAS_COPIES
        if getattr(self, "_qkv_bias", None) is None or self._qkv_bias[0].device != dev:
            self._qkv_bias = [torch.zeros(3 * D, dtype=F32, device=dev) for _ in enc.layers]
        _BIAS_COPIES = []
        for li, lyr in enumerate(enc.layers):
            w = NS()
            with ops.cast_group():
                w.att = prep_attention(lyr.self_attn, dev, bias_buf=self._qkv_bias[li])
                w.fc1 = prep_linear([lyr.fc1.weight], [lyr.fc1.bias], dev)
                w.fc2 = prep_linear([lyr.fc2.weight], [lyr.fc2.bias], dev)
            W.layers.append(w)
        if _BIAS_COPIES:
            torch._foreach_copy_([d for d, _ in _BIAS_COPIES], [s_ for _, s_ in _BIAS_COPIES])
        _BIAS_COPIES = None
        W.scb = []
        if cfg.use_enrollments and cfg.scb_layers:
            for blk in enc.ca_enrolls:
                s = NS()
                with ops.cast_group():
                    s.att = prep_attention(blk.cae.cross_attn, dev, fuse_qkv=False)
                    s.f0 = prep_linear([blk.cae.ffn[0].weight], [blk.cae.ffn[0].bias], dev)
                    s.f3 = prep_linear([blk.cae.ffn[3].weight], [blk.cae.ffn[3].bias], dev)
                W.scb.append(s)
        W.full_init = prep_full_fddt(enc.initial_fddt, dev) if (cfg.use_fddt and cfg.use_pre_pos_fddt and fddt_is_full(enc.initial_fddt)) else None
        W.full = [prep_full_fddt(f, dev) if fddt_is_full(f) else None for f in (enc.fddts if cfg.use_fddt else [])]
        W.fold = None
        self.W = W
        return W

    def prepare_fold(self):
        W, enc = self.W, self.enc
        if W.fold is not None:
            return W.fold
        dev = enc.conv1.weight.device
        D, F_ = self.cfg.d_model, self.cfg.encoder_ffn_dim
        fold = []
        for lyr in enc.layers:
            f = NS()
            att, ln1, ln2 = lyr.self_attn, lyr.self_attn_layer_norm, lyr.final_layer_norm
            f.qkv_w, f.qkv_c, f.qkv_b = _e((3 * D, D), BF16, dev), _e((3 * D,), F32, dev), _e((3 * D,), F32, dev)
            for k, (lin, has_b) in enumerate(((att.q_proj, True), (att.k_proj, False), (att.v_proj, True))):
                sl = slice(k * D, (k + 1) * D)
                ops.lnfold_prep(lin.weight.detach(), ln1.weight.detach(), ln1.bias.detach(), lin.bias.detach() if has_b else None,
                                f.qkv_w[sl], f.qkv_c[sl], f.qkv_b[sl])
            f.fc1_w, f.fc1_c, f.fc1_b = _e((F_, D), BF16, dev), _e((F_,), F32, dev), _e((F_,), F32, dev)
            ops.lnfold_prep(lyr.fc1.weight.detach(), ln2.weight.detach(), ln2.bias.detach(), lyr.fc1.bias.detach(), f.fc1_w, f.fc1_c, f.fc1_b)
            f.eps1, f.eps2 = float(ln1.eps), float(ln2.eps)
            fold.append(f)
        W.fold = fold
        return fold

    def forward(self, input_features, stno_mask, enrollments=None, need_grad=True):
        cfg = self.cfg
        B, T = input_features.shape[0], cfg.max_source_positions
        if (SPLIT_FWD and not need_grad and enrollments is None and not cfg.use_enrollments and input_features.is_cuda and B % 2 == 0
                and B * T >= SPLIT_FWD_MIN_ROWS and input_features.dim() == 3 and input_features.shape[2] == 2 * T
                and _split_allowed()):
            dev, D = input_features.device, cfg.d_model
            enc_out, enc_bf = _e((B * T, D), F32, dev), _e((B * T, D), BF16, dev)
            stno_mask = stno_mask.to(device=dev)
            main_st, parts, _ = _fwd_parts(B, T, dev)
            S = None
            for st_, r, bsl in parts:
                with torch.cuda.stream(st_):
                    _, Sh = self._forward_impl(input_features[bsl], stno_mask[bsl], None, False, out=(enc_out[r], enc_bf[r]))
                    del Sh.layers
                S = S or Sh
            for st_, _, _ in parts[1:]:
                main_st.wait_stream(st_)
            S.B0, S.B_out, S.enc_bf, S.h_last = B, B, enc_bf, None
            return enc_out.view(B, T, D), S
        return self._forward_impl(input_features, stno_mask, enrollments, need_grad)

    def _forward_impl(self, input_features, stno_mask, enrollments=None, need_grad=True, out=None):
        enc, cfg, W = self.enc, self.cfg, self.W
        dev = input_features.device
        if enrollments is not None:
            input_features = torch.stack((input_features, enrollments["input_features"].to(dev)), dim=1).flatten(0, 1)
            stno_mask = torch.stack((stno_mask, enrollments["stno_mask"].to(dev)), dim=1).flatten(0, 1)
        B, M, Tin = input_features.shape
        T, D, H, F_ = cfg.max_source_positions, cfg.d_model, cfg.encoder_attention_heads, cfg.encoder_ffn_dim
        if Tin != 2 * T:
            raise ValueError(f"Whisper expects the mel input features to be of length {2 * T}, but found {Tin}. "
                             f"Make sure to pad the input mel features to {2 * T}.")
        stno = stno_mask.to(device=dev, dtype=F32).contiguous()
        S = NS(B0=B, T=T, stno=stno, layers=[], scb=[])
        x2, stem = conv_stem_fwd(enc, W, input_features, need_grad=need_grad)
        if need_grad:
            S.stem, S.x2 = stem, x2
        rows = B * T
        pos = enc.embed_positions.weight
        init_fddt = enc.initial_fddt if (cfg.use_fddt and cfg.use_pre_pos_fddt) else None
        mode, fw, fb = fddt_ptrs(init_fddt, cfg)
        h = _e((rows, D), F32, dev)
        if W.full_init is not None:
            hf0, S.x2b = full_fddt_fwd(W.full_init, x2, stno, 4 * T, rows, T, D)
            ops.fddt_ln_fwd(hf0, rows, D, mode=ops.MODE_NONE, T=T, pos=pos.detach(), h_out=h)
        else:
            ops.fddt_ln_fwd(x2, rows, D, mode=mode, stno=stno, T=T, w=fw, b=fb, pos=pos.detach(), h_out=h)
        bstride = 4 * T
        Bc = B
        fuse_next = (FUSE_NEXT_FDDT and not need_grad and cfg.use_fddt and not cfg.use_enrollments and all(f is None for f in W.full)
                     and ops.gemm_nt(h, W.layers[0].fc2.w, h, rows, D, F_, residual=h, bias=W.layers[0].fc2.b, query_persistent=True))
        rowmask = None
        if fuse_next:
            rowmask = torch.zeros(_ceil(rows, 192) + 64, 4, dtype=F32, device=dev)
            rowmask[:rows].view(B, T, 4).copy_(stno.permute(0, 2, 1))
        fold = None
        if (LN_FOLD and not need_grad and not cfg.use_enrollments and all(f is None for f in W.full) and D % 320 == 0 and D <= 1280
                and ops.gemm_nt(h, W.layers[0].fc2.w, h, rows, D, F_, residual=h, bias=W.layers[0].fc2.b, query_lnstat=True)
                and ops.gemm_nt(h, W.layers[0].att.o.w, h, rows, D, D, residual=h, bias=W.layers[0].att.o.b, query_lnstat=True)
                and ops.gemm_nt(h, W.layers[0].att.qkv.w, h, rows, 3 * D, D, query_persistent=True)):
            fold = self.prepare_fold()
            stat1 = torch.zeros(rows, L.LN_SLOTS, 2, dtype=F32, device=dev)
            stat2 = torch.zeros(rows, L.LN_SLOTS, 2, dtype=F32, device=dev)
        hb = None
        fddt_done = False
        split_ok = (SPLIT_FWD and need_grad and fold is None and not fuse_next and all(f is None for f in W.full)
                    and _split_allowed())
        split_from = cfg.scb_layers if (cfg.use_enrollments and cfg.scb_layers) else 0
        halves = None
        for i, lyr in enumerate(enc.layers):
            w = W.layers[i]
            Ls = NS(h_in=h, B=Bc, bstride=bstride)
            rows = Bc * T
            if split_ok and halves is None and i == split_from and Bc % 2 == 0 and rows >= SPLIT_FWD_MIN_ROWS:
                S.split_from, S.split_sstep = i, bstride // (4 * T)
                main_st, halves, Bh = _fwd_parts(Bc, T, dev)
                rh, sstep = Bh * T, bstride // (4 * T)
            if halves is not None:
                fd = enc.fddts[i] if (cfg.use_fddt and i < len(enc.fddts)) else None
                mode, fw, fb = fddt_ptrs(fd, cfg)
                ln, ln2 = lyr.self_attn_layer_norm, lyr.final_layer_norm
                xln, mean, rstd = _e((rows, D), BF16, dev), _e((rows,), F32, dev), _e((rows,), F32, dev)
                hp = _e((rows, D), F32, dev) if mode != ops.MODE_NONE else h
                qkv, o, lse = _e((rows, 3 * D), BF16, dev), _e((rows, D), BF16, dev), _e((Bc, H, T), F32, dev)
                h2, xln2 = _e((rows, D), F32, dev), _e((rows, D), BF16, dev)
                mean2, rstd2 = _e((rows,), F32, dev), _e((rows,), F32, dev)
                u, a, hn = _e((rows, F_), BF16, dev), _e((rows, F_), BF16, dev), _e((rows, D), F32, dev)
                for st_, r, bsl in halves:
                    with torch.cuda.stream(st_):
                        ops.fddt_ln_fwd(h[r], rh, D, mode=mode, stno=stno[bsl.start * sstep:], stno_bstride=bstride, T=T, w=fw, b=fb,
                                        h_out=hp[r] if mode != ops.MODE_NONE else None, ln_w=ln.weight.detach(),
                                        ln_b=ln.bias.detach(), y_bf16=xln[r], mean=mean[r], rstd=rstd[r])
                        linear_fwd(xln[r], w.att.qkv, rh, flags=L.EPI_SCALE_N, scale=Q_SCALE, scale_ncols=D, out=qkv[r])
                        ops.attn_fwd(heads(qkv[r][:, :D], Bh, T, H), heads(qkv[r][:, D:2 * D], Bh, T, H), heads(qkv[r][:, 2 * D:], Bh, T, H),
                                     heads(o[r], Bh, T, H), lse[bsl], q_log2=QK_LOG2)
                        linear_fwd(o[r], w.att.o, rh, out_dtype=F32, residual=hp[r], out=h2[r])
                        ops.fddt_ln_fwd(h2[r], rh, D, mode=ops.MODE_NONE, ln_w=ln2.weight.detach(), ln_b=ln2.bias.detach(), y_bf16=xln2[r],
                                        mean=mean2[r], rstd=rstd2[r])
                        linear_fwd(xln2[r], w.fc1, rh, gelu_aux=u[r], out=a[r])
                        linear_fwd(a[r], w.fc2, rh, out_dtype=F32, residual=h2[r], out=hn[r])
                h = hn
                Ls.rows, Ls.B_after, Ls.hp, Ls.xln, Ls.mean, Ls.rstd = rows, Bc, hp, xln, mean, rstd
                Ls.qkv, Ls.o, Ls.lse, Ls.h2, Ls.xln2, Ls.mean2, Ls.rstd2, Ls.u, Ls.a = qkv, o, lse, h2, xln2, mean2, rstd2, u, a
                S.layers.append(Ls)
                continue
            fd = enc.fddts[i] if (cfg.use_fddt and i < len(enc.fddts)) else None
            mode, fw, fb = fddt_ptrs(fd, cfg)
            if fddt_done:
                mode, fw, fb = ops.MODE_NONE, (None,) * 4, (None,) * 4
            nfd = enc.fddts[i + 1] if (fuse_next and i + 1 < len(enc.layers) and i + 1 < len(enc.fddts)) else None
            nmode, nfw, nfb = fddt_ptrs(nfd, cfg)
            fuse_here = nfd is not None and nmode == ops.MODE_DIAG and all(t is not None for t in nfw) and all(t is not None for t in nfb)
            use_scb = cfg.use_enrollments and cfg.scb_layers is not None and i < cfg.scb_layers
            wfull = W.full[i] if (fd is not None and i < len(W.full)) else None
            if wfull is not None:
                h, Ls.full_hb = full_fddt_fwd(wfull, h, stno, bstride, rows, T, D)
                Ls.h_in = h
                mode, fw, fb = ops.MODE_NONE, (None,) * 4, (None,) * 4
            xln = _e((rows, D), BF16, dev)
            mean, rstd = _e((rows,), F32, dev), _e((rows,), F32, dev)
            ln = lyr.self_attn_layer_norm
            fold1 = fold is not None and hb is not None and mode == ops.MODE_NONE
            if fold1:
                hp = h
            elif not use_scb:
                hp = _e((rows, D), F32, dev) if mode != ops.MODE_NONE else h
                ops.fddt_ln_fwd(h, rows, D, mode=mode, stno=stno, stno_bstride=bstride, T=T, w=fw, b=fb,
                                h_out=hp if mode != ops.MODE_NONE else None, ln_w=ln.weight.detach(),
                                ln_b=ln.bias.detach(), y_bf16=xln, mean=mean, rstd=rstd)
# ... 875 lines not shown
```

ts-asr-whisper_amd/modeling.py:

```python
import math
import re
from collections import OrderedDict
from types import SimpleNamespace as NS_
from typing import Optional

import torch
from torch import nn

from . import _lib as L
from . import ops
from .config import DiCoWConfig, _HF

if _HF:
    from transformers import PreTrainedModel as _ModelBase, GenerationConfig as _GenerationConfig
else:
    _ModelBase, _GenerationConfig = nn.Module, None
from .engine import EncoderEngine, DecoderEngine, CtcEngine, GradSink, fddt_ptrs, CLS, prep_full_fddt, full_fddt_fwd, full_fddt_bwd

F32, BF16 = torch.float32, torch.bfloat16


class ModelOutput(OrderedDict):

    def __getattr__(self, k):
# ... 171 lines not shown
    def __init__(self, d_model, non_target_rate=0.01, fddt_init=None, is_diagonal=False, bias_only=False, use_silence=True,
                 use_target=True, use_overlap=True, use_non_target=True):
        super().__init__()

        def make(val):
            if bias_only:
                return nn.Parameter(torch.zeros(d_model))
            if is_diagonal:
                return DiagonalLinear(d_model, bias=True, fddt_init=fddt_init, init_eye_val=val)
            return DenseLinear(d_model, d_model, bias=True, fddt_init=fddt_init, init_eye_val=val)

        if use_target:
            self.target_linear = make(1.0)
        if use_non_target:
            self.non_target_linear = make(non_target_rate)
        if use_overlap:
            self.overlap_linear = make(1.0)
        if use_silence:
            self.silence_linear = make(non_target_rate)
        self.use_silence, self.use_target, self.use_overlap, self.use_non_target = use_silence, use_target, use_overlap, use_non_target
        self.bias_only, self.is_diagonal, self.d_model = bias_only, is_diagonal or bias_only, d_model

    def forward(self, hidden_states, stno_mask):
        if not self.is_diagonal:
            return self._forward_full(hidden_states, stno_mask)
        params = [p for p in self.parameters()]
        return _FDDTFn.apply(self, hidden_states, stno_mask, *params)

    def _forward_full(self, hidden_states, stno_mask):
        params = [p for p in self.parameters()]
        return _FDDTFullFn.apply(self, hidden_states, stno_mask, *params)


class _FDDTFullFn(torch.autograd.Function):
    @staticmethod
    def forward(ctx, mod, hidden, stno, *params):
        _require_cuda(hidden, "FDDT")
        B, T, D = hidden.shape
        if D % 64 != 0:
            raise L.DicowError("full FDDT needs d_model % 64 == 0")
        dev = hidden.device
        h = hidden.contiguous().to(F32).view(B * T, D)
        st = stno.to(device=dev, dtype=F32).contiguous()
        w = prep_full_fddt(mod, dev)
        out, hb = full_fddt_fwd(w, h, st, 4 * T, B * T, T, D)
        ctx.mod, ctx.w, ctx.hb, ctx.st, ctx.params, ctx.shape = mod, w, hb, st, params, (B, T, D)
        return out.view(B, T, D)

    @staticmethod
    def backward(ctx, g):
        B, T, D = ctx.shape
        G = GradSink(ctx.params, g.device)
        gh = full_fddt_bwd(ctx.mod, ctx.w, ctx.hb, g.contiguous().to(F32).view(B * T, D), ctx.st, 4 * T, G, B * T, T, D)
        return (None, gh.view(B, T, D), None) + tuple(G.result(p) for p in ctx.params)


def _refuse_unsupported(where, **kw):
    bad = [k for k, v in kw.items() if v is not None]
    if bad:
        raise NotImplementedError(f"{where}: {', '.join(bad)} not supported by the HIP path (per-head masks, attention / "
                                  "hidden-state outputs, decoder masks / positions have no kernels here)")


class _EncoderFn(torch.autograd.Function):
    @staticmethod
    def forward(ctx, enc, input_features, stno, enrollments, need_grad, *params):
        eng = enc._engine()
        out, S = eng.forward(input_features, stno, enrollments, need_grad=need_grad)
        ctx.enc, ctx.S, ctx.params = enc, (S if need_grad else None), params
        return out

    @staticmethod
    def backward(ctx, d_enc):
        enc, S = ctx.enc, ctx.S
        G = GradSink(ctx.params, d_enc.device)
        D = enc.config.d_model
        enc._engine(prepare=False).backward(S, d_enc.contiguous().view(-1, D).to(F32), G)
        return (None, None, None, None, None) + tuple(G.result(p) for p in ctx.params)


class DiCoWEncoder(nn.Module):
    def __init__(self, config: DiCoWConfig):
        super().__init__()
        self.config = config
        d, f = config.d_model, config.encoder_ffn_dim
        self.conv1 = nn.Conv1d(config.num_mel_bins, d, kernel_size=3, padding=1)
        self.conv2 = nn.Conv1d(d, d, kernel_size=3, stride=2, padding=1)
        self.embed_positions = nn.Embedding(config.max_source_positions, d)
        self.embed_positions.requires_grad_(False)
        self.layers = nn.ModuleList([EncoderLayer(d, f) for _ in range(config.encoder_layers)])
        self.layer_norm = nn.LayerNorm(d)
        self.ctc_weight = config.ctc_weight
        if config.ctc_weight > 0.0:
            if config.additional_layer:
                self.additional_layer = EncoderLayer(d, f)
            if config.additional_self_attention_layer:
                self.additional_self_attention_layer = Attention(d)
            if config.pre_ctc_sub_sample:
                self.subsample_conv1 = nn.Conv1d(d, d, kernel_size=3, stride=2, padding=1, bias=False)
                self.subsample_conv2 = nn.Conv1d(d, d, kernel_size=3, stride=2, padding=1, bias=False)
            self.lm_head = nn.Linear(d, config.vocab_size + 1, bias=False)
        self.first_task_token = config.vocab_size - 30 * 50 - 1 - 6
        if config.use_fddt:
            def mk(rate):
                return FDDT(d_model=d, non_target_rate=rate, fddt_init=config.fddt_init, is_diagonal=config.fddt_is_diagonal,
                            bias_only=config.fddt_bias_only, use_silence=config.fddt_use_silence,
                            use_target=config.fddt_use_target, use_overlap=config.fddt_use_overlap,
                            use_non_target=config.fddt_use_non_target)
            self.fddts = nn.ModuleList([mk(1.0) for _ in range(config.num_fddts)])
            if config.use_pre_pos_fddt:
                self.initial_fddt = mk(config.non_target_fddt_value)
        if config.use_enrollments and config.scb_layers is not None:
            self.ca_enrolls = nn.ModuleList([SpeakerCommunicationBlock(config) for _ in range(config.scb_layers)])
        self._eng = None
        self._sig = None
        self._ctc_eng = None
        self._ctc_sig = None

    _CTC_PREFIXES = ("additional_layer.", "additional_self_attention_layer.", "subsample_conv", "lm_head.")
    main_input_name = "input_features"

    def get_loss(self, logits, labels):
        if int(labels.max()) >= self.config.vocab_size:
            raise ValueError(f"Label values must be <= vocab_size: {self.config.vocab_size}")
        lab = labels.to(logits.device)
        if self.config.remove_timestamps_from_ctc:
            keep = lab < self.first_task_token
            order = torch.argsort((~keep).to(torch.int8), dim=1, stable=True)
            lab = torch.gather(lab, 1, order)
            cnt = keep.sum(dim=1, keepdim=True)
            lab = torch.where(torch.arange(lab.shape[1], device=lab.device)[None, :] < cnt, lab, torch.full_like(lab, -100))
            lab = lab[:, :max(int(cnt.max()), 1)]
        valid = lab >= 0
        lab = torch.gather(lab, 1, torch.argsort((~valid).to(torch.int8), dim=1, stable=True)).contiguous()
        return _CtcLossFn.apply(self, logits, lab)

    def ctc_parameters(self):
        return [p for n, p in self.named_parameters() if n.startswith(self._CTC_PREFIXES)]

    def _ctc_engine(self, prepare=True):
        if self._ctc_eng is None:
            self._ctc_eng = CtcEngine(self)
        if prepare:
            sig = _param_sig(self.ctc_parameters())
            if sig != self._ctc_sig:
                self._ctc_eng.prepare()
                self._ctc_sig = sig
        return self._ctc_eng

    def _engine(self, prepare=True):
        if self._eng is None:
            self._eng = EncoderEngine(self)
        if prepare:
            ctc_ids = {id(p) for p in self.ctc_parameters()} if self.ctc_weight > 0.0 else set()
            sig = _param_sig([p for p in self.parameters() if id(p) not in ctc_ids])
            if sig != self._sig:
                self._eng.prepare()
                self._sig = sig
        return self._eng

    def get_max_len(self):
        return self.config.max_source_positions * 2

    def forward(self, input_features, attention_mask=None, head_mask=None, output_attentions=None, output_hidden_states=None,
                return_dict=None, stno_mask=None, return_logits=False, enrollments=None):
        _require_cuda(input_features, "DiCoWEncoder")
        if stno_mask is None:
            if self.config.use_fddt or enrollments is not None:
                raise ValueError("stno_mask is required")
            stno_mask = torch.zeros(input_features.shape[0], 4, self.config.max_source_positions, dtype=F32, device=input_features.device)
        _refuse_unsupported("DiCoWEncoder.forward", head_mask=head_mask, output_attentions=output_attentions or None,
                            output_hidden_states=output_hidden_states or None)
        ctc_ids = {id(p) for p in self.ctc_parameters()} if self.ctc_weight > 0.0 else set()
        params = [p for p in self.parameters() if id(p) not in ctc_ids]
        need_grad = torch.is_grad_enabled() and (input_features.requires_grad or any(p.requires_grad for p in params))
        out = _EncoderFn.apply(self, input_features, stno_mask, enrollments, need_grad, *params)
        if return_logits:
            if self.ctc_weight <= 0.0:
                raise L.DicowError("return_logits needs the CTC head (ctc_weight > 0)")
            logits = _CtcLogitsFn.apply(self, out, *self.ctc_parameters())
            return ModelOutput(loss=None, logits=logits, hidden_states=out)
        if return_dict is False:
            return (out,)
        return ModelOutput(last_hidden_state=out, hidden_states=None, attentions=None)

    def ctc_logits_into(self, input_features, stno_mask, out):
        if torch.is_grad_enabled():
            raise L.DicowError("ctc_logits_into keeps nothing for a backward pass: call it under torch.no_grad()")
        if self.ctc_weight <= 0.0:
            raise L.DicowError("ctc_logits_into needs the CTC head (ctc_weight > 0)")
        enc_out = self.forward(input_features, stno_mask=stno_mask).last_hidden_state
        enc_bf, enc_f, B, T = _ctc_head_input(enc_out)
        self._ctc_engine().encode_logits(enc_bf, B, T, enc_f, out=out)
        return out

    def ctc_logits_layout(self):
        if self.ctc_weight <= 0.0:
            raise L.DicowError("ctc_logits_layout needs the CTC head (ctc_weight > 0)")
        eng = self._ctc_engine()
        return eng.frames(self.config.max_source_positions), eng.W.cpad


def freeze_for_ctc_pretraining(encoder):
    head = {id(p) for p in encoder.ctc_parameters()}
    if not head:
        raise L.DicowError("freeze_for_ctc_pretraining: the encoder has no CTC head (ctc_weight > 0)")
    for p in encoder.parameters():
        p.requires_grad_(id(p) in head)
    return encoder


def _ctc_head_input(enc_out):
    B, T, D = enc_out.shape
    enc_f = enc_out.contiguous().to(F32).view(B * T, D)
    return ops.cast_bf16(enc_f).view(B * T, D), enc_f, B, T


class _CtcFn(torch.autograd.Function):

    @staticmethod
    def forward(ctx, enc, enc_out, ctc_labels, *params):
        eng = enc._ctc_engine()
        B, T, D = enc_out.shape
        enc_f = enc_out.contiguous().to(F32).view(B * T, D)
        enc_bf = ops.cast_bf16(enc_f).view(B * T, D)
        loss, S = eng.forward(enc_bf, B, T, ctc_labels, enc_f)
        ctx.enc, ctx.S, ctx.params = enc, S, params
        return loss

    @staticmethod
    def backward(ctx, g_loss):
        enc, S = ctx.enc, ctx.S
        G = GradSink(ctx.params, g_loss.device)
        d_enc = enc._ctc_engine(prepare=False).backward(S, g_loss, G)
        hook = getattr(enc, "_segment_hook", None)
        if hook is not None:
            hook("ctc")
        return (None, d_enc.view(S.B, S.T, -1), None) + tuple(G.result(p) for p in ctx.params)


class _CtcLogitsFn(torch.autograd.Function):

    @staticmethod
    def forward(ctx, enc, enc_out, *params):
        eng = enc._ctc_engine()
        enc_bf, enc_f, B, T = _ctc_head_input(enc_out)
        S = eng.encode_logits(enc_bf, B, T, enc_f)
        ctx.enc, ctx.S, ctx.params = enc, S, params
        return S.logits.view(B, S.Tn, -1)[:, :, :enc.config.vocab_size + 1]

    @staticmethod
    def backward(ctx, g):
        enc, S = ctx.enc, ctx.S
        eng = enc._ctc_engine(prepare=False)
        cpad, V1 = eng.W.cpad, enc.config.vocab_size + 1
        pad = getattr(enc, "_ctc_dlogits", None)
        if pad is not None and pad.shape == (S.B * S.Tn, cpad) and g.data_ptr() == pad.data_ptr() and g.stride() == (S.Tn * cpad, cpad, 1):
            d = pad
        else:
            d = torch.zeros(S.B * S.Tn, cpad, dtype=BF16, device=g.device)
            d.view(S.B, S.Tn, cpad)[:, :, :V1].copy_(g)
        enc._ctc_dlogits = None
        G = GradSink(ctx.params, g.device)
        d_enc = eng.backward_from_logits(S, d, G)
        hook = getattr(enc, "_segment_hook", None)
        if hook is not None:
            hook("ctc")
        return (None, d_enc.view(S.B, S.T, -1)) + tuple(G.result(p) for p in ctx.params)


class _CtcLossFn(torch.autograd.Function):

    @staticmethod
    def forward(ctx, enc, logits, labels):
        B, Tn, V1 = logits.shape
        dev = logits.device
        if logits.dtype == BF16 and logits.stride(2) == 1 and logits.stride(0) == Tn * logits.stride(1) and logits.stride(1) % 2 == 0:
            buf, ld = logits, logits.stride(1)
        else:
            ld = (V1 + 127) // 128 * 128
            buf = torch.zeros(B, Tn, ld, dtype=BF16, device=dev)
            buf[:, :, :V1].copy_(logits)
        lab = labels.contiguous()
        S = NS_(B=B, Tn=Tn, ld=ld, buf=buf)
        S.lse, S.nll, S.tlen = (torch.empty(n, dtype=F32, device=dev) for n in (B * Tn, B, B))
        S.ab = torch.empty(2, B, Tn, 2 * lab.shape[1] + 1, dtype=F32, device=dev)
        S.acc = torch.zeros(1, dtype=F32, device=dev)
        S.labels = lab
        S.ctc = ops.ctc_args(buf, ld, B, Tn, V1, lab, S.lse, S.ab[0], S.ab[1], S.nll, S.tlen, S.acc)
        ops.ctc_loss_fwd(S.ctc)
        ctx.enc, ctx.S, ctx.V1 = enc, S, V1
        return S.acc[0] / B

    @staticmethod
    def backward(ctx, g):
        enc, S = ctx.enc, ctx.S
        d = torch.empty(S.B * S.Tn, S.ld, dtype=BF16, device=g.device)
        S.ctc.d_logits = d.data_ptr()
        ops.ctc_loss_bwd(S.ctc, g.to(F32).reshape(1))
        enc._ctc_dlogits = d
        return None, d.view(S.B, S.Tn, S.ld)[:, :, :ctx.V1], None


def prepare_ctc_labels(labels, config, prefix_tokens, first_task_token):
    lab = labels.clone()
    for tok in prefix_tokens:
        if bool((lab[:, 0] == tok).all()):
            lab = lab[:, 1:]
    lab[lab == config.eos_token_id] = -100
    if config.remove_timestamps_from_ctc:
        keep = lab < first_task_token
        order = torch.argsort((~keep).to(torch.int8), dim=1, stable=True)
# ... 630 lines not shown
```

ts-asr-whisper_amd/ops.py:

```python
import ctypes as C
import os
from typing import Optional, Sequence

import torch

from . import _lib as L

BF16 = torch.bfloat16
F32 = torch.float32


def _req(t: torch.Tensor, dtype, name: str):
    if not t.is_cuda:
        raise L.DicowError(f"{name}: tensor must live on the GPU (no CPU fallback)")
    if t.dtype != dtype:
        raise L.DicowError(f"{name}: expected {dtype}, got {t.dtype}")
    return t


def _p(t):
    return None if t is None else t.data_ptr()


_WS = {}
# ... 402 lines not shown
def lora_wgrad(t, p, outs, r, scale, *, block=False, accumulate=True, g_rs=None, g_cs=1):
    _lora_2d(t, BF16, "lora_wgrad.t")
    _lora_2d(p, BF16, "lora_wgrad.p")
    a = L.LoraWgradArgs()
    a.T, a.P = t.data_ptr(), p.data_ptr()
    a.ldt, a.ldp = t.stride(0), p.stride(0)
    a.M, a.R, a.r, a.flags = t.shape[0], t.shape[1], int(r), L.LORA_BLOCK if block else 0
    nseg = max(a.R // max(a.r, 1), 1)
    assert p.shape[0] == a.M and len(outs) == nseg and nseg <= L.LORA_MAX_SEG, "lora_wgrad: shapes disagree"
    a.N = p.shape[1] // nseg if block else p.shape[1]
    assert not block or p.shape[1] == nseg * a.N
    a.g_rs, a.g_cs = (a.N if g_rs is None else g_rs), g_cs
    for j, g in enumerate(outs):
        if g is not None:
            _req(g, F32, "lora_wgrad.out")
            assert g.is_contiguous() and g.numel() == a.r * a.N, "lora_wgrad.out: need a contiguous r x N (or N x r) fp32 tensor"
            a.G[j] = g.data_ptr()
    a.scale, a.accumulate = float(scale), int(bool(accumulate))
    need = L.lib().dicow_lora_wgrad_ws_bytes(a.M, a.N, a.R, a.r, a.flags)
    ws = workspace(max(need, 1), t.device)
    a.ws, a.ws_bytes = ws.data_ptr(), ws.numel()
    L.call_struct("dicow_lora_wgrad", a)


_FWS = {}
ATTN_BWD_FUSED = os.environ.get("DICOW_ATTN_BWD_FUSED", "1") != "0"


def attn_bwd_fused_ws(B, H, Lq, Lk, device):
    n = L.lib().dicow_attn_bwd_fused_ws_bytes(B, H, Lq, Lk)
    key = (device.type, device.index, torch.cuda.current_stream(device).cuda_stream)
    t = _FWS.get(key)
    if t is None or t.numel() < n:
        t = torch.zeros(n + 4096, dtype=torch.uint8, device=device)
        _FWS[key] = t
    off = (-t.data_ptr()) % 4096
    return t[off:off + n]


def attn_bwd_fused_status(device=None) -> int:
    torch.cuda.synchronize(device)
    st = 0
    for (_, idx, _), t in _FWS.items():
        if device is None or idx == torch.device(device).index:
            off = (-t.data_ptr()) % 4096
            st |= L.lib().dicow_attn_bwd_fused_status(t.data_ptr() + off)
    return st


def attn_bwd(q, k, v, o, d_o, lse, delta, dq, dk, dv, causal=False, dq_scale=1.0, dq_colsum=None, dv_colsum=None, q_log2=False,
             fused=None):
    assert delta.numel() >= 2 * lse.numel(), "attn_bwd: delta workspace must hold 2*B*H*Lq floats"
    a = L.AttnBwdArgs()
    a.q, a.k, a.v, a.o, a.d_o = q.data_ptr(), k.data_ptr(), v.data_ptr(), o.data_ptr(), d_o.data_ptr()
    a.lse, a.delta = lse.data_ptr(), delta.data_ptr()
    a.dq, a.dk, a.dv = dq.data_ptr(), dk.data_ptr(), dv.data_ptr()
    a.q_bs, a.q_rs = _bs_rs(q, "q")
    a.k_bs, a.k_rs = _bs_rs(k, "k")
    a.v_bs, a.v_rs = _bs_rs(v, "v")
    a.o_bs, a.o_rs = _bs_rs(o, "o")
    a.do_bs, a.do_rs = _bs_rs(d_o, "d_o")
    a.dq_bs, a.dq_rs = _bs_rs(dq, "dq")
    a.dk_bs, a.dk_rs = _bs_rs(dk, "dk")
    a.dv_bs, a.dv_rs = _bs_rs(dv, "dv")
    a.B, a.Lq, a.H = q.shape[0], q.shape[1], q.shape[2]
    a.Lk, a.causal, a.dq_scale, a.q_log2 = k.shape[1], int(causal), dq_scale, int(q_log2)
    if dq_colsum is not None or dv_colsum is not None:
        ws = workspace(L.lib().dicow_attn_bwd_colsum_ws_bytes(a.B, a.H, a.Lq, a.Lk), q.device)
        a.dq_colsum, a.dv_colsum, a.cs_ws, a.cs_ws_bytes = _p(dq_colsum), _p(dv_colsum), ws.data_ptr(), ws.numel()
    want = ATTN_BWD_FUSED if fused is None else fused
    a.fused_mode = int(want == "force")
    if want and L.lib().dicow_attn_bwd_fused_eligible(a.B, a.H, a.Lq, a.Lk, a.causal, a.fused_mode):
        fws = attn_bwd_fused_ws(a.B, a.H, a.Lq, a.Lk, q.device)
        a.fused_ws, a.fused_ws_bytes = fws.data_ptr(), fws.numel()
    L.call_struct("dicow_attn_bwd", a)


def ce_args(logits, ld, rows, V, labels, upp_labels, soft, ts, lse, row_loss, choice, loss_sum, count, d_logits=None):
    _req(labels, torch.int64, "ce.labels")
    if upp_labels is not None:
        _req(upp_labels, torch.int64, "ce.upp_labels")
    a = L.CeArgs()
    a.logits, a.ld, a.rows, a.V = logits.data_ptr(), ld, rows, V
    a.labels, a.upp_labels, a.soft = labels.data_ptr(), _p(upp_labels), int(soft)
    if ts is not None:
        a.ts_index, a.ts_ids, a.ts_w, a.n_ts = ts["index"].data_ptr(), ts["ids"].data_ptr(), ts["w"].data_ptr(), ts["ids"].numel()
    a.lse, a.row_loss, a.choice = lse.data_ptr(), row_loss.data_ptr(), choice.data_ptr()
    a.loss_sum, a.count, a.d_logits = loss_sum.data_ptr(), count.data_ptr(), _p(d_logits)
    return a


def ce_loss_fwd(a):
    L.call_struct("dicow_ce_loss_fwd", a)


def ce_loss_bwd(a, grad_scale):
    L.check(L.lib().dicow_ce_loss_bwd(C.byref(a), grad_scale.data_ptr(), L.stream()), "dicow_ce_loss_bwd")


def embed_fwd(ids, tok, pos, out):
    B, Lq = ids.shape
    L.call("dicow_embed_fwd", ids.data_ptr(), tok.data_ptr(), pos.data_ptr(), out.data_ptr(), B, Lq, tok.shape[1], L.stream())


def embed_bwd(ids, g, d_tok, d_pos, D):
    B, Lq = ids.shape
    L.call("dicow_embed_bwd", ids.data_ptr(), g.data_ptr(), _p(d_tok), _p(d_pos), B, Lq, D, L.stream())


def gelu_bwd_bf16(g, pre, out):
    L.call("dicow_gelu_bwd_bf16", g.data_ptr(), pre.data_ptr(), out.data_ptr(), g.numel(), L.stream())


def conv2_col2im_gelu_bwd(dA2, pre1, d_pre1, B, T2, Cc):
    L.call("dicow_conv2_col2im_gelu_bwd", dA2.data_ptr(), _p(pre1), d_pre1.data_ptr(), B, T2, Cc, L.stream())


def ctc_args(logits, ld, B, Tn, Cc, labels, lse, alpha, beta, nll, tlen, loss_sum):
    _req(labels, torch.int64, "ctc.labels")
    a = L.CtcArgs()
    a.logits, a.ld, a.B, a.Tn, a.C = logits.data_ptr(), ld, B, Tn, Cc
    a.labels, a.Lc, a.blank = labels.data_ptr(), labels.shape[1], Cc - 1
    a.lse, a.alpha, a.beta, a.Smax = lse.data_ptr(), alpha.data_ptr(), beta.data_ptr(), 2 * labels.shape[1] + 1
    a.nll, a.tlen, a.loss_sum = nll.data_ptr(), tlen.data_ptr(), loss_sum.data_ptr()
    return a


def ctc_loss_fwd(a):
    L.call_struct("dicow_ctc_loss_fwd", a)


def ctc_loss_bwd(a, grad_scale):
    L.check(L.lib().dicow_ctc_loss_bwd(C.byref(a), grad_scale.data_ptr(), L.stream()), "dicow_ctc_loss_bwd")


def fabric_emulate(buf, gbps, workgroups=16, passes=2):
    L.call("dicow_fabric_emulate", buf.data_ptr(), buf.numel() * buf.element_size(), float(gbps), int(workgroups), int(passes), L.stream())


def sumsq(x, out):
    L.call("dicow_sumsq_f32", x.data_ptr(), x.numel(), out.data_ptr(), L.stream())


def adamw(p, g, m, v, lr, beta1, beta2, eps, wd, step, gnorm_sq=None, max_norm=0.0):
    L.call("dicow_adamw_f32", p.data_ptr(), g.data_ptr(), m.data_ptr(), v.data_ptr(), p.numel(), lr, beta1, beta2, eps, wd,
           step, _p(gnorm_sq), max_norm, L.stream())


def adamw_dev(p, g, m, v, hyper, beta1, beta2, eps, wd, gnorm_sq=None, max_norm=0.0):
    L.call("dicow_adamw_f32_dev", p.data_ptr(), g.data_ptr(), m.data_ptr(), v.data_ptr(), p.numel(), hyper.data_ptr(), beta1, beta2,
           eps, wd, _p(gnorm_sq), max_norm, L.stream())


def multi_adamw(tensors_ptr, chunks_ptr, n_chunks, classes, cls_base=0, clip_coef=None):
    L.check(L.lib().dicow_multi_adamw_f32(tensors_ptr, chunks_ptr, n_chunks, C.byref(classes), cls_base, _p(clip_coef), L.stream()),
            "dicow_multi_adamw_f32")


def multi_sumsq_ws_bytes(n_chunks) -> int:
    return int(L.lib().dicow_multi_sumsq_ws_bytes(n_chunks))


def multi_sumsq(tensors_ptr, chunks_ptr, n_chunks, ws, out, max_norm):
    _req(out, F32, "multi_sumsq: out")
    L.call("dicow_multi_sumsq_f32", tensors_ptr, chunks_ptr, n_chunks, ws.data_ptr(), ws.numel(), out.data_ptr(), float(max_norm),
           L.stream())


def multi_scale(tensors_ptr, chunks_ptr, n_chunks, coef):
    L.call("dicow_multi_scale_f32", tensors_ptr, chunks_ptr, n_chunks, coef.data_ptr(), L.stream())
```

ts-asr-whisper_amd/trainer.py:

```python
import collections
import logging
import math
import os
import time

import torch
import torch.distributed as dist

from . import ops
from . import tracing
from .engine import GradSink

F32 = torch.float32
log = logging.getLogger(__name__)


def freeze_by_keyword(model, frozen_keywords=("decoder",)):
    for n, p in model.named_parameters():
        p.requires_grad_("lora_" in n or not any(k in n for k in frozen_keywords))
    model.tie_weights()


def _backward_order(model):
    enc = model.model.encoder
    groups = []
    ctc_ids = set()
    if getattr(enc, "ctc_weight", 0.0) > 0.0:
        ctc = enc.ctc_parameters()
        ctc_ids = {id(p) for p in ctc}
        groups.append(("ctc", ctc))
    groups.append(("final_ln", list(enc.layer_norm.parameters())))
    nl = len(enc.layers)
    for i in range(nl - 1, -1, -1):
        ps = list(enc.layers[i].parameters())
        ps = [p for p in ps if p.dim() == 2] + [p for p in ps if p.dim() != 2]
        if hasattr(enc, "fddts") and i < len(enc.fddts):
            ps += list(enc.fddts[i].parameters())
        if hasattr(enc, "ca_enrolls") and i < len(enc.ca_enrolls):
            ps += list(enc.ca_enrolls[i].parameters())
        groups.append((f"layer{i}", ps))
    tail = []
    if hasattr(enc, "initial_fddt"):
        tail += list(enc.initial_fddt.parameters())
    tail += [enc.embed_positions.weight] + list(enc.conv2.parameters()) + list(enc.conv1.parameters())
    groups.append(("stem", tail))
    return groups


REFERENCE_PREHEAT_PREFIXES = ("model.encoder.additional_layer", "model.encoder.additional_self_attention_layer", "model.encoder.lm_head",
                              "model.encoder.subsample_conv1", "model.encoder.subsample_conv2", "model.encoder.fddts",
                              "model.encoder.initial_fddt", "model.encoder.ca_enrolls")


class FlatStore:

    def __init__(self, model, preheat_prefixes=None):
        preheat_prefixes = REFERENCE_PREHEAT_PREFIXES if preheat_prefixes is None else tuple(preheat_prefixes)
        names = {id(p): n for n, p in model.named_parameters()}
        dev = next(model.parameters()).device
        self.segments = []
        self.runs = []
        entries, off, seen = [], 0, set()
        grouped = _backward_order(model)
        enc_ids = {id(p) for _, ps in grouped for p in ps}
        rest = [p for p in model.parameters() if p.requires_grad and id(p) not in enc_ids]
        if rest:
            grouped = [("decoder", rest)] + grouped
        for gname, ps in grouped:
            start = off
            for p in ps:
                if not p.requires_grad or id(p) in seen:
                    continue
                seen.add(id(p))
                n = p.numel()
                pre = any(names[id(p)].startswith(pp) for pp in preheat_prefixes)
                entries.append((p, off, n, pre))
                off += (n + 63) // 64 * 64
            if off > start:
                self.segments.append((gname, start, off))
        self.numel = off
        self.params = torch.zeros(off, dtype=F32, device=dev)
        self.grads = torch.zeros(off, dtype=F32, device=dev)
        self.exp_avg = torch.zeros(off, dtype=F32, device=dev)
        self.exp_avg_sq = torch.zeros(off, dtype=F32, device=dev)
        self.entries = entries
        self._names = names
        for p, o, n, pre in entries:
            self.params[o:o + n].copy_(p.data.reshape(-1))
            p.data = self.params[o:o + n].view(p.shape)
            p.grad = self.grads[o:o + n].view(p.shape)
            p._direct_grad = p.grad
            pad_end = o + (n + 63) // 64 * 64
            if self.runs and self.runs[-1][2] == pre and self.runs[-1][1] == o:
                self.runs[-1] = (self.runs[-1][0], pad_end, pre)
            else:
                self.runs.append((o, pad_end, pre))
        self.n_trainable = sum(n for _, _, n, _ in entries)
        enc = model.model.encoder
        over = {id(p) for lyr in enc.layers for p in lyr.parameters() if p.dim() == 2}
        self._over = [(p, o, n) for p, o, n, _ in entries if id(p) in over]
        keep, cur = [], 0
        for p, o, n in sorted(self._over, key=lambda t: t[1]):
            if o > cur:
                keep.append((cur, o))
            cur = max(cur, o + n)
        if cur < self.numel:
            keep.append((cur, self.numel))
        self._zero_ranges = keep
        self._zero_views = None

    def fingerprint(self):
        return [(self._names[id(p)], int(o), int(n)) for p, o, n, _ in self.entries]

    def zero_grad(self, first_writer=False):
        if not first_writer or not self._over:
            self.grads.zero_()
            for p, _, _ in self._over:
                p._grad_overwrite = False
            return
        if self._zero_views is None:
            self._zero_views = [self.grads[a:b] for a, b in self._zero_ranges if b > a]
        if self._zero_views:
            torch._foreach_zero_(self._zero_views)
        for p, o, n in self._over:
            p._grad_overwrite = bool(p.requires_grad)
            if not p.requires_grad:
                self.grads[o:o + n].zero_()

    def settle_range(self, a, b):
        n_left = 0
        for p, o, n in self._over:
            if a <= o < b and getattr(p, "_grad_overwrite", False):
                self.grads[o:o + n].zero_()
                p._grad_overwrite = False
                n_left += 1
        return n_left

    def settle_first_writers(self):
        n_left = 0
        for p, o, n in self._over:
            if getattr(p, "_grad_overwrite", False):
                self.grads[o:o + n].zero_()
                p._grad_overwrite = False
                n_left += 1
        return n_left


class FusedAdamW:

    def __init__(self, store, lr=2e-6, fddt_lr_multiplier=100.0, betas=(0.9, 0.999), eps=1e-8, weight_decay=0.0,
                 max_grad_norm=1.0, warmup_steps=0, max_steps=0, schedule="cosine"):
        self.s, self.lr, self.mult, self.betas, self.eps, self.wd = store, lr, fddt_lr_multiplier, betas, eps, weight_decay
        self.max_norm, self.warmup, self.max_steps, self.schedule = max_grad_norm, warmup_steps, max_steps, schedule
        self.t = 0
        self.run_t = [0] * len(store.runs)
        self.gnorm_sq = torch.zeros(1, dtype=F32, device=store.params.device)
        dev = store.params.device
        self.counters = torch.zeros(1 + len(store.runs), dtype=torch.int32, device=dev)
        self.hyper = torch.zeros(len(store.runs), 3, dtype=F32, device=dev)
        self.is_pre = torch.tensor([int(pre) for _, _, pre in store.runs], dtype=torch.int32, device=dev)

    def sync_counters(self):
        self.counters.copy_(torch.tensor([self.t] + list(self.run_t), dtype=torch.int32))

    def lr_at(self, k):
        sched_step = k - 1
        if sched_step < self.warmup:
            return self.lr * sched_step / max(1, self.warmup)
        if self.schedule == "cosine" and self.max_steps > 0:
            prog = (sched_step - self.warmup) / max(1, self.max_steps - self.warmup)
            return self.lr * max(0.0, 0.5 * (1.0 + math.cos(math.pi * prog)))
        return self.lr

    def applied_lr(self):
        return self.hyper[:, 0].detach().cpu().tolist()

    def advance(self, preheat_only=False):
        self.t += 1
        for i, (a, b, pre) in enumerate(self.s.runs):
            if not (preheat_only and not pre):
                self.run_t[i] += 1

    def launch(self, preheat_only=False):
        s = self.s
        L_ = ops.L
        L_.call("dicow_adamw_hyper", self.counters.data_ptr(), self.hyper.data_ptr(), self.is_pre.data_ptr(), len(s.runs),
                int(preheat_only), float(self.lr), float(self.mult), int(self.warmup), int(self.max_steps),
                int(self.schedule == "cosine"), float(self.betas[0]), float(self.betas[1]), L_.stream())
        self.gnorm_sq.zero_()
        ops.sumsq(s.grads, self.gnorm_sq)
        for i, (a, b, pre) in enumerate(s.runs):
            if preheat_only and not pre:
                continue
            ops.adamw_dev(s.params[a:b], s.grads[a:b], s.exp_avg[a:b], s.exp_avg_sq[a:b], self.hyper[i], self.betas[0], self.betas[1],
                          self.eps, 0.0 if pre else self.wd, gnorm_sq=self.gnorm_sq, max_norm=self.max_norm)

    def step(self, preheat_only=False):
        self.advance(preheat_only)
        self.launch(preheat_only)


def _bit_checksum(t):
    flat = t.detach().reshape(-1)
    if flat.numel() == 0:
        return 0
    view = {1: torch.uint8, 2: torch.int16, 4: torch.int32, 8: torch.int64}[flat.element_size()]
    bits = flat.view(view)
    total, step = 0, 1 << 24
    for a in range(0, bits.numel(), step):
        c = bits[a:a + step].to(torch.int64)
        idx = torch.arange(a, a + c.numel(), device=c.device, dtype=torch.int64)
        total = (total + int((c * (2 * (idx % 1000003) + 1)).sum().item())) & 0xFFFFFFFFFFFFFFFF
    return total


_SYNC_COALESCE_BELOW = 64 << 20


def sync_replicas(model, store=None, process_group=None, mode="broadcast", src=0, extra=()):
    if mode not in ("broadcast", "verify", "none"):
        raise ValueError(f"replica_sync must be 'broadcast', 'verify' or 'none', not {mode!r}")
    if mode == "none" or not dist.is_initialized():
        return 0
    world = dist.get_world_size(process_group)
    in_store = set()
    tensors = []
    if store is not None:
        in_store = {id(p) for p, _, _, _ in store.entries}
        tensors.append(store.params)
    seen = set()
    rest = []
    for t in list(model.parameters()) + list(model.buffers()):
        if id(t) in in_store or id(t) in seen or t.data_ptr() in seen:
            continue
        seen.add(id(t))
        seen.add(t.data_ptr())
        rest.append(t.data)
    rest += [t for t in extra if t is not None]
    src_global = dist.get_global_rank(process_group, src) if process_group is not None else src
    if mode == "verify":
        mine = 0
        for t in tensors + rest:
            mine = (mine * 1000003 + _bit_checksum(t)) & 0x7FFFFFFFFFFFFFFF
        dev = tensors[0].device if tensors else (rest[0].device if rest else torch.device("cpu"))
        got = [torch.zeros(1, dtype=torch.int64, device=dev) for _ in range(world)]
        dist.all_gather(got, torch.tensor([mine], dtype=torch.int64, device=dev), group=process_group)
        sums = [int(g.item()) for g in got]
        if len(set(sums)) != 1:
            bad = [r for r, v in enumerate(sums) if v != sums[src]]
            raise RuntimeError(f"data-parallel replicas differ at start-up: ranks {bad} do not hold rank {src}'s parameters / buffers "
                               f"(checksums {[hex(v) for v in sums]}); construct TrainStep with replica_sync='broadcast' or load the "
                               f"same checkpoint on every rank")
        log.info("replica check: %d ranks hold identical state (checksum %s)", world, hex(sums[0]))
        return 8 * world
    nbytes = 0
    if world > 1 or os.environ.get("DICOW_FORCE_REDUCE") == "1":
        for t in tensors:
            dist.broadcast(t, src=src_global, group=process_group)
            nbytes += t.numel() * t.element_size()
        by_dtype = collections.OrderedDict()
        for t in rest:
            if t.numel() * t.element_size() >= _SYNC_COALESCE_BELOW and t.is_contiguous():
                dist.broadcast(t, src=src_global, group=process_group)
                nbytes += t.numel() * t.element_size()
            else:
                by_dtype.setdefault((t.dtype, t.device), []).append(t)
        for (dt, dev), ts in by_dtype.items():
            flat = torch.cat([t.reshape(-1) for t in ts]) if len(ts) > 1 else ts[0].reshape(-1).clone()
            dist.broadcast(flat, src=src_global, group=process_group)
            off = 0
            for t in ts:
                t.copy_(flat[off:off + t.numel()].view(t.shape))
                off += t.numel()
            nbytes += flat.numel() * flat.element_size()
        log.info("replica sync: rank %d's state broadcast to %d ranks (%d bytes: %d in the flat store)", src, world, nbytes,
                 sum(t.numel() * t.element_size() for t in tensors))
    return nbytes


def nccl_pg_options():
    try:
        opts = dist.ProcessGroupNCCL.Options()
        opts.is_high_priority_stream = True
        return opts
    except Exception:
        return None


class GradReducer:

    def __init__(self, store, process_group=None):
        self.s = store
        self.pg = process_group
        self.world = dist.get_world_size(process_group) if dist.is_initialized() else 1
        self.force = os.environ.get("DICOW_FORCE_REDUCE") == "1" and dist.is_initialized()
        self.stream = None
        if (self.world > 1 or self.force) and torch.cuda.is_available():
            self.stream = torch.cuda.Stream(priority=-1 if os.environ.get("DICOW_REDUCER_STREAM_PRIORITY", "high") == "high" else 0)
        if self.stream is not None and self.world > 1:
            from . import ops
            reserve = int(os.environ.get("DICOW_RCCL_CUS", "16"))
            ncu = torch.cuda.get_device_properties(torch.cuda.current_device()).multi_processor_count
            ops.set_gemm_cus(max(ncu - reserve, ncu // 2))
        self._avg_in_collective = bool(dist.is_initialized() and dist.get_backend(process_group) == "nccl")
        self.seg = {name: (a, b) for name, a, b in store.segments}
        self.pending = []
        self.time_exposed = False
        self._exposed = []
        self.time_buckets = False
        self._bucket_ev = []
        self._bucket_cpu = []
        g = os.environ.get("DICOW_EMULATE_FABRIC_GBPS")
        self.emulate_gbps = float(g) if g else 0.0
        self.emulate_workgroups = int(os.environ.get("DICOW_EMULATE_FABRIC_WGS", "16"))
        self.preheat_only = False
        self.hold = False

    def segment_ready(self, name):
        if (self.world == 1 and not self.force) or name not in self.seg or self.preheat_only or self.hold:
            return
        a, b = self.seg[name]
        self.s.settle_range(a, b)
        if self.stream is None:
            buf = self.s.grads[a:b]
            t0 = time.perf_counter()
            dist.all_reduce(buf, group=self.pg)
            buf.div_(self.world)
            if self.time_buckets:
                self._bucket_cpu.append((name, time.perf_counter() - t0))
            return
        ev = torch.cuda.Event(enable_timing=self.time_buckets)
        ev.record()
        with torch.cuda.stream(self.stream):
            self.stream.wait_event(ev)
            if self.time_buckets:
                e_start = torch.cuda.Event(enable_timing=True)
                e_start.record()
            buf = self.s.grads[a:b]
            if self._avg_in_collective:
                dist.all_reduce(buf, op=dist.ReduceOp.AVG, group=self.pg)
            else:
                dist.all_reduce(buf, group=self.pg)
                buf.div_(self.world)
            if self.emulate_gbps > 0.0 and buf.is_cuda:
                n = (b - a) // 4 * 4
                if n > 0:
                    ops.fabric_emulate(buf[:n], self.emulate_gbps, self.emulate_workgroups)
            if self.time_buckets:
                e_end = torch.cuda.Event(enable_timing=True)
                e_end.record()
                self._bucket_ev.append((name, ev, e_start, e_end))

# ... 18 lines not shown
                e0.record()
                torch.cuda.current_stream().wait_stream(self.stream)
                e1.record()
                self._exposed.append((e0, e1))
            else:
                torch.cuda.current_stream().wait_stream(self.stream)

    def bucket_report(self, steps=1):
        rows = []
        if self._bucket_ev:
            torch.cuda.synchronize()
            rows = [(n, r.elapsed_time(s_), s_.elapsed_time(e)) for n, r, s_, e in self._bucket_ev]
        elif self._bucket_cpu:
            rows = [(n, 0.0, dt * 1e3) for n, dt in self._bucket_cpu]
        self._bucket_ev, self._bucket_cpu = [], []
        if not rows:
            return None
        steps = max(1, steps)
        per = {}
        for n, lag, dur in rows:
            t = per.setdefault(n, [0, 0.0, 0.0])
            t[0] += 1; t[1] += lag; t[2] += dur
        worst = sorted(per.items(), key=lambda kv: -kv[1][1] / kv[1][0])[:3]
        return {"buckets_per_step": len(rows) // steps,
                "start_lag_ms": {"mean": round(sum(r[1] for r in rows) / len(rows), 4), "max": round(max(r[1] for r in rows), 4),
                                 "sum_per_step": round(sum(r[1] for r in rows) / steps, 3)},
                "busy_ms_per_step": round(sum(r[2] for r in rows) / steps, 3),
                "longest_queued": [{"bucket": n, "lag_ms": round(v[1] / v[0], 4), "collective_ms": round(v[2] / v[0], 4)} for n, v in worst]}

    def exposed_ms(self):
        if not self._exposed:
            return 0.0
        torch.cuda.synchronize()
        ms = sum(a.elapsed_time(b) for a, b in self._exposed) / len(self._exposed)
        self._exposed = []
        return ms


_SPLIT_NOWAIT = os.environ.get("DICOW_SPLIT_NOWAIT") == "1"
_SPLIT_LEAD_FIRST = os.environ.get("DICOW_SPLIT_LEAD_FIRST", "1") == "1"
_SPLIT_GROUP = int(os.environ.get("DICOW_SPLIT_GROUP", "2"))


class SplitSync:

    def __init__(self, group=_SPLIT_GROUP):
        self.role, self.ev, self.group, self.free_until = None, {}, max(1, int(group)), None

    def reset(self):
        self.role, self.ev, self.free_until = None, {}, None

    def _gate(self, name):
        if not name.startswith("layer") or self.group == 1:
            return name
        i = int(name[5:])
        return f"layer{i - i % self.group}"

    def enter(self, name):
        if self.role == "follow" and not _SPLIT_NOWAIT:
            gate = self._gate(name)
            if gate == self.free_until:
                return
            ev = self.ev.get(gate)
            if ev is None:
                raise RuntimeError(f"SplitSync: the leader half never finished segment {gate!r} -- the two halves' backward passes differ")
            torch.cuda.current_stream().wait_event(ev)
            self.free_until = gate

    def done(self, name):
        if self.role == "lead" and self._gate(name) == name:
            ev = torch.cuda.Event()
            ev.record()
            self.ev[name] = ev


class TrainStep:

    def __init__(self, model, lr=2e-6, fddt_lr_multiplier=100.0, weight_decay=0.0, max_grad_norm=1.0, warmup_steps=0,
                 max_steps=0, frozen_keywords=("decoder",), preheat_prefixes=None,
                 process_group=None, augmenter=None, use_fddt_only_n_steps=0, graph=False, use_fddt_only_n_epochs=0,
                 steps_per_epoch=None, replica_sync="broadcast", split_streams=False, front_end=None):
        self.model = model
        self.split_streams = bool(split_streams)
        self._split_sync = SplitSync()
        self._split_side = None
        if use_fddt_only_n_epochs:
            if not steps_per_epoch:
                raise ValueError("use_fddt_only_n_epochs needs steps_per_epoch (optimizer steps in one pass over the training set)")
            use_fddt_only_n_steps = max(int(use_fddt_only_n_steps), int(use_fddt_only_n_epochs) * int(steps_per_epoch))
        self.first_writer = True
        self.graph = bool(graph)
        self._graphs = collections.OrderedDict()
        self.max_graphs = 8
        self._graph_pool = None
        self._eager_done = set()
        self.augmenter = augmenter
        self.front_end = front_end
        freeze_by_keyword(model, frozen_keywords)
        self.store = FlatStore(model, preheat_prefixes)
        self.opt = FusedAdamW(self.store, lr, fddt_lr_multiplier, weight_decay=weight_decay, max_grad_norm=max_grad_norm,
                              warmup_steps=warmup_steps, max_steps=max_steps)
        self.reducer = GradReducer(self.store, process_group)
        self.replica_sync = replica_sync
        self.replica_sync_bytes = sync_replicas(model, self.store, process_group, mode=replica_sync)
        if self.replica_sync_bytes and replica_sync == "broadcast":
            model.model.encoder._sig = None
            model.model.encoder._ctc_sig = None
            model._sig = None
        model.model.encoder._segment_hook = self.reducer.segment_ready
        model._segment_hook = self.reducer.segment_ready
        self.use_fddt_only_n_steps = use_fddt_only_n_steps
        self.warmup_phase = use_fddt_only_n_steps > 0
        names = {id(p): n for n, p in model.named_parameters()}
        self._preheat_is_vectors_only = all(p.dim() == 1 and "fddt" in names[id(p)] for p, _, _, pre in self.store.entries if pre)
        if self.warmup_phase:
            self._set_phase(preheat_only=True)

    def _set_phase(self, preheat_only):
        for p, _, _, pre in self.store.entries:
            p.requires_grad_(pre or not preheat_only)
        self.reducer.preheat_only = preheat_only
        self.model.model.encoder._sig = None
        self.model._sig = None

    def _invalidate_decoder_copies(self):
        base = lora = False
        for n, p in self.model.model.decoder.named_parameters():
            if p.requires_grad:
                if "lora_" in n:
                    lora = True
                else:
                    base = True
                    break
        if base:
            self.model._sig = None
        elif lora:
            self.model._lora_sig = None

    @property
    def global_step(self):
        return self.opt.t

    def begin_step(self):
        if self.warmup_phase and self.global_step >= self.use_fddt_only_n_steps:
            self._set_phase(preheat_only=False)
            self.warmup_phase = False
        self.store.zero_grad(first_writer=self.first_writer and not self.warmup_phase)

    def finish_step(self):
        with tracing.range("exchange"):
            self.reducer.finish()
        if self.first_writer and not self.warmup_phase:
            self.store.settle_first_writers()
        with tracing.range("optimizer"):
            self.opt.step(preheat_only=self.warmup_phase)
        enc = self.model.model.encoder
        if not (self.warmup_phase and self._preheat_is_vectors_only):
            enc._sig = None
            enc._ctc_sig = None
        self._invalidate_decoder_copies()

    def _micro(self, batch, scale):
        if self.split_streams and self._can_split(batch):
            return self._micro_split(batch, scale)
        if self.front_end is not None and "input_waves" in batch:
            batch = self.front_end(dict(batch))
        if self.augmenter is not None:
            batch = self.augmenter(dict(batch))
        with tracing.range("forward"):
            out = self.model(**batch)
        with tracing.range("backward"):
            (out.loss if scale == 1.0 else out.loss * scale).backward()
        return out.loss.detach()

    def _can_split(self, batch):
        cfg = self.model.config
        lab = batch.get("labels")
        return (self.split_streams and self.augmenter is None and self.front_end is None and cfg.ctc_weight == 0.0 and batch.get("enrollments") is None and
                lab is not None and lab.is_cuda and lab.shape[0] >= 2 and lab.shape[0] % 2 == 0 and
                all(not torch.is_tensor(v) or v.dim() == 0 or v.shape[0] == lab.shape[0] for v in batch.values()))

    def _micro_split(self, batch, scale):
        model, enc, sync = self.model, self.model.model.encoder, self._split_sync
        cur = torch.cuda.current_stream()
        if self._split_side is None:
            pf, pl = (int(x) for x in os.environ.get("DICOW_SPLIT_PRIO", "-1,-1").split(","))
            self._split_side = (torch.cuda.Stream(priority=pf), torch.cuda.Stream(priority=pl))
        s_f, s_l = self._split_side
        hb = batch["labels"].shape[0] // 2
        halves = [{k: (v[i * hb:(i + 1) * hb] if torch.is_tensor(v) and v.dim() > 0 else v) for k, v in batch.items()} for i in (0, 1)]
        if getattr(model, "_ts_tables", None) is not None:
            cnt = torch.stack([(h["labels"] != -100).sum() for h in halves]).to(torch.float32)
            wts = cnt / cnt.sum().clamp_min(1.0) * scale
        else:
            wts = torch.full((2,), 0.5 * scale, dtype=torch.float32, device=batch["labels"].device)
        enc._engine()
        model._engine()
        sync.reset()
        enc._split_sync = model._split_sync = sync
        try:
            with tracing.range("forward"):
                outs = [None, None]
                for i, st in (((1, s_l), (0, s_f)) if _SPLIT_LEAD_FIRST else ((0, s_f), (1, s_l))):
                    st.wait_stream(cur)
                    with torch.cuda.stream(st):
                        outs[i] = model(**halves[i])
            with tracing.range("backward"):
                hold = self.reducer.hold
                self.reducer.hold = True
                sync.role = "lead"
                with torch.cuda.stream(s_l):
                    (outs[1].loss * wts[1]).backward()
                self.reducer.hold = hold
                sync.role = "follow"
                with torch.cuda.stream(s_f):
                    (outs[0].loss * wts[0]).backward()
        finally:
            sync.role = None
            enc._split_sync = model._split_sync = None
        cur.wait_stream(s_l)
        cur.wait_stream(s_f)
        for o in outs:
            o.loss.record_stream(cur)
        return (outs[0].loss.detach() * wts[0] + outs[1].loss.detach() * wts[1]) / scale

    @staticmethod
    def _sig_of(batch):
        out = []
        for k in sorted(batch):
            v = batch[k]
            out.append((k, TrainStep._sig_of(v)) if isinstance(v, dict) else (k, tuple(v.shape), str(v.dtype)))
        return tuple(out)

    @staticmethod
    def _clone(batch):
        return {k: (TrainStep._clone(v) if isinstance(v, dict) else v.clone()) for k, v in batch.items()}

    @staticmethod
    def _copy_into(dst, src):
        for k, v in src.items():
            if isinstance(v, dict):
                TrainStep._copy_into(dst[k], v)
            else:
                dst[k].copy_(v, non_blocking=True)

    def _invalidate_weight_copies(self):
        enc = self.model.model.encoder
        enc._sig = None
        enc._ctc_sig = None
        self._invalidate_decoder_copies()

    def _graph_step(self, batch):
        if self.reducer.world > 1 or self.reducer.force:
            raise NotImplementedError("TrainStep(graph=True) captures the single-GPU step; the bucketed side-stream exchange is not captured")
        if self.model.config.ctc_weight > 0.0 or self.augmenter is not None or self.front_end is not None:
            raise NotImplementedError("TrainStep(graph=True): the CTC label preparation / the augmentation planner read device data on "
                                      "the host; their steps cannot be captured")
        if self.warmup_phase and self.global_step >= self.use_fddt_only_n_steps:
            self._set_phase(preheat_only=False)
            self.warmup_phase = False
        key = (self.warmup_phase, self._sig_of(batch))
        if key not in self._eager_done:
            self._eager_done.add(key)
            return self._eager_step([batch])
        if key not in self._graphs:
            while len(self._graphs) >= max(1, self.max_graphs):
                self._graphs.popitem(last=False)
            if self._graph_pool is None:
                self._graph_pool = torch.cuda.graph_pool_handle()
            static = self._clone(batch)
            self._invalidate_weight_copies()
            torch.cuda.synchronize()
            g = torch.cuda.CUDAGraph()
            with torch.cuda.graph(g, pool=self._graph_pool):
                self.store.zero_grad(first_writer=self.first_writer and not self.warmup_phase)
                out = self.model(**static)
                out.loss.backward()
                self.opt.launch(preheat_only=self.warmup_phase)
                loss = out.loss.detach()
            self._graphs[key] = (g, static, loss)
        self._graphs.move_to_end(key)
        g, static, loss = self._graphs[key]
        self._copy_into(static, batch)
        self.opt.advance(preheat_only=self.warmup_phase)
        g.replay()
        self._invalidate_weight_copies()
        return loss.clone()

    def step(self, batch, eager=False):
        micro = list(batch) if isinstance(batch, (list, tuple)) else [batch]
        if self.graph and not eager and len(micro) == 1:
            return self._graph_step(micro[0])
        return self._eager_step(micro)

    def _eager_step(self, micro):
        self.begin_step()
        loss = None
        for i, b in enumerate(micro):
            self.reducer.hold = i + 1 < len(micro)
            l = self._micro(b, 1.0 / len(micro))
            loss = l if loss is None else loss + l
        self.finish_step()
        return loss / len(micro)

    def logged_loss(self, loss):
        r = self.reducer
        if r.world == 1:
            return loss
        t = loss.detach().clone().float().reshape(1)
        dist.all_reduce(t, op=dist.ReduceOp.SUM, group=r.pg)
        return (t / r.world)[0]

    def state_dict(self):
        o = self.opt
        return {"global_step": o.t, "run_t": list(o.run_t), "warmup_phase": self.warmup_phase,
                "exp_avg": self.store.exp_avg.clone(), "exp_avg_sq": self.store.exp_avg_sq.clone(),
                "layout": [(a, b, pre) for a, b, pre in self.store.runs], "entries": self.store.fingerprint()}

    def resync(self):
        if self.replica_sync == "none" or self.reducer.world <= 1:
            return 0
        n = sync_replicas(self.model, self.store, self.reducer.pg, mode=self.replica_sync)
        self.model.model.encoder._sig = None
        self.model.model.encoder._ctc_sig = None
        self.model._sig = None
        return n

    def _sync_host_counters_phase(self, phase):
        keep = self.warmup_phase
        self.warmup_phase = phase
        try:
            return self._sync_host_counters()
        finally:
            self.warmup_phase = keep

    def _sync_host_counters(self):
        if self.replica_sync == "none" or self.reducer.world <= 1 or not dist.is_initialized():
            return
        dev = self.store.params.device
        mine = torch.tensor([int(self.opt.t), int(bool(self.warmup_phase))] + [int(x) for x in self.opt.run_t], dtype=torch.int64, device=dev)
        if self.replica_sync == "verify":
            got = [torch.zeros_like(mine) for _ in range(self.reducer.world)]
            dist.all_gather(got, mine, group=self.reducer.pg)
            bad = [r for r, g in enumerate(got) if not torch.equal(g, got[0])]
            if bad:
                raise RuntimeError(f"data-parallel replicas resumed with different step counters: ranks {bad} differ from rank 0 "
                                   f"(global_step / warmup_phase / per-run steps {[g.tolist()[:3] for g in got]})")
            return
        src = dist.get_global_rank(self.reducer.pg, 0) if self.reducer.pg is not None else 0
        dist.broadcast(mine, src=src, group=self.reducer.pg)
        vals = mine.tolist()
        self.opt.t, self.opt.run_t = int(vals[0]), [int(x) for x in vals[2:]]
        self.opt.sync_counters()
        return bool(vals[1])

    def load_state_dict(self, sd, allow_legacy_layout=False, sync_model=True):
        if [tuple(r) for r in sd["layout"]] != [tuple(r) for r in self.store.runs]:
            raise ValueError("optimizer state was saved for a different set of trainable parameters")
        if "entries" not in sd:
            if not allow_legacy_layout:
                raise ValueError("optimizer state has no per-parameter layout fingerprint (saved by an older version): the order of the "
                                 "parameters inside the flat buffers cannot be checked; pass allow_legacy_layout=True if it was saved by "
                                 "a version with today's parameter order (weight matrices before vectors inside a layer), or re-save it")
            log.warning("optimizer state without a layout fingerprint accepted on request: only the run boundaries were checked")
        elif [tuple(e) for e in sd["entries"]] != self.store.fingerprint():
            mine = {e[0]: e for e in self.store.fingerprint()}
            diff = [e[0] for e in sd["entries"] if tuple(e) != mine.get(e[0])][:4]
            raise ValueError(f"optimizer state was saved under a different flat-buffer layout (first differing parameters: {diff})")
        self.opt.t, self.opt.run_t = int(sd["global_step"]), list(sd["run_t"])
        self.opt.sync_counters()
        self.store.exp_avg.copy_(sd["exp_avg"])
        self.store.exp_avg_sq.copy_(sd["exp_avg_sq"])
        phase = bool(sd["warmup_phase"])
        if self.replica_sync != "none" and self.reducer.world > 1:
            if sync_model or self.replica_sync == "verify":
                if self.replica_sync == "broadcast":
                    try:
                        sync_replicas(self.model, self.store, self.reducer.pg, mode="verify")
                    except RuntimeError as ex:
                        log.warning("load_state_dict: the ranks' model weights differ before the resume broadcast -- rank 0's replace the others' (%s)", ex)
                sync_replicas(self.model, self.store, self.reducer.pg, mode=self.replica_sync,
                              extra=(self.store.exp_avg, self.store.exp_avg_sq, self.opt.counters))
            else:
                sync_replicas(torch.nn.Module(), None, self.reducer.pg, mode=self.replica_sync,
                              extra=(self.store.exp_avg, self.store.exp_avg_sq, self.opt.counters))
            p0 = self._sync_host_counters_phase(phase)
            phase = p0 if p0 is not None else phase
            self.model.model.encoder._sig = None
            self.model.model.encoder._ctc_sig = None
            self.model._sig = None
        sd = dict(sd, warmup_phase=phase)
        if bool(sd["warmup_phase"]) != self.warmup_phase:
            self._set_phase(preheat_only=bool(sd["warmup_phase"]))
            self.warmup_phase = bool(sd["warmup_phase"])
```

Before: 126.4 utt/s.

## Fuse AdamW update with bf16 weight-copy refresh into a single planned kernel

```diff
diff --git a/include/dicow_hip.h b/include/dicow_hip.h
--- a/include/dicow_hip.h
+++ b/include/dicow_hip.h
@@ -348,6 +348,19 @@
                       int warmup_steps, int max_steps, int cosine, double beta1, double beta2, void* stream);
 int dicow_adamw_f32_dev(float* p, const float* g, float* m, float* v, int64_t n, const float* hyper, float beta1, float beta2,
                         float eps, float weight_decay, const float* gnorm_sq, float max_norm, void* stream);
+typedef struct {
+    int64_t start, end;
+    void* dst; void* dst_t;
+    int64_t ld, ld_t;
+    int R, C;
+    int run;
+    float weight_decay;
+} dicow_refresh_item;
+int dicow_adamw_refresh_vector_ok(const dicow_refresh_item* item);
+int dicow_adamw_refresh_plan(const dicow_refresh_item* items, int n_items, int64_t numel, int n_runs, int* unit0);
+int dicow_adamw_refresh(float* p, const float* g, float* m, float* v, const dicow_refresh_item* items_dev, const int* unit0_dev,
+                        int n_items, int n_units, const float* hyper, float beta1, float beta2, float eps, const float* gnorm_sq,
+                        float max_norm, void* stream);
 
 #define DICOW_MT_CHUNK 2048
 #define DICOW_MT_MAX_CLASSES 32
diff --git a/ts-asr-whisper_amd/_lib.py b/ts-asr-whisper_amd/_lib.py
--- a/ts-asr-whisper_amd/_lib.py
+++ b/ts-asr-whisper_amd/_lib.py
@@ -47,6 +47,11 @@
 
 class CastProblem(C.Structure):
     _fields_ = [("src", c_vp), ("dst", c_vp), ("dst_t", c_vp), ("R", c_i), ("C", c_i), ("ld", c_i64), ("ld_t", c_i64)]
+
+
+class RefreshItem(C.Structure):
+    _fields_ = [("start", c_i64), ("end", c_i64), ("dst", c_vp), ("dst_t", c_vp), ("ld", c_i64), ("ld_t", c_i64),
+                ("R", c_i), ("C", c_i), ("run", c_i), ("weight_decay", c_f)]
 
 
 class GemmTnGroupArgs(C.Structure):
@@ -210,6 +215,9 @@
     "dicow_adamw_f32": [c_vp, c_vp, c_vp, c_vp, c_i64, c_f, c_f, c_f, c_f, c_f, c_i, c_vp, c_f, c_vp],
     "dicow_adamw_hyper": [c_vp, c_vp, c_vp, c_i, c_i, c_d, c_d, c_i, c_i, c_i, c_d, c_d, c_vp],
     "dicow_adamw_f32_dev": [c_vp, c_vp, c_vp, c_vp, c_i64, c_vp, c_f, c_f, c_f, c_f, c_vp, c_f, c_vp],
+    "dicow_adamw_refresh_vector_ok": [C.POINTER(RefreshItem)],
+    "dicow_adamw_refresh_plan": [C.POINTER(RefreshItem), c_i, c_i64, c_i, C.POINTER(c_i)],
+    "dicow_adamw_refresh": [c_vp, c_vp, c_vp, c_vp, c_vp, c_vp, c_i, c_i, c_vp, c_f, c_f, c_f, c_vp, c_f, c_vp],
     "dicow_multi_chunk_elems": [],
     "dicow_multi_adamw_f32": [c_vp, c_vp, c_i64, C.POINTER(MtAdamwClasses), c_i, c_vp, c_vp],
     "dicow_multi_sumsq_f32": [c_vp, c_vp, c_i64, c_vp, c_i64, c_vp, c_f, c_vp],
diff --git a/ts-asr-whisper_amd/csrc/elementwise.hip b/ts-asr-whisper_amd/csrc/elementwise.hip
--- a/ts-asr-whisper_amd/csrc/elementwise.hip
+++ b/ts-asr-whisper_amd/csrc/elementwise.hip
@@ -534,15 +534,28 @@
 #define ADAMW_NT 0
 #endif
 typedef __attribute__((ext_vector_type(4))) float f32x4a_t;
+__device__ __forceinline__ float adamw_clip(const float* __restrict__ gnorm_sq, float max_norm) {
+    float clip = 1.f;
+    if (gnorm_sq && max_norm > 0.f) {
+        const float c = max_norm / (sqrtf(gnorm_sq[0]) + 1e-6f);
+        clip = c < 1.f ? c : 1.f;
+    }
+    return clip;
+}
+__device__ __forceinline__ void adamw_update(float& p, float g, float& m, float& v, float clip, float lr, float b1, float b2, float eps,
+                                             float wd, float bc1, float bc2) {
+    const float gr = g * clip;
+    p *= 1.f - lr * wd;
+    m = b1 * m + (1.f - b1) * gr;
+    v = b2 * v + (1.f - b2) * gr * gr;
+    const float denom = sqrtf(v) / sqrtf(bc2) + eps;
+    p -= (lr / bc1) * (m / denom);
+}
 __global__ void adamw_kernel(float* __restrict__ p, const float* __restrict__ g, float* __restrict__ m, float* __restrict__ v,
                              int64_t n, float lr, float b1, float b2, float eps, float wd, float bc1, float bc2,
                              const float* __restrict__ gnorm_sq, float max_norm, const float* __restrict__ hyper) {
     if (hyper) { lr = hyper[0]; bc1 = hyper[1]; bc2 = hyper[2]; }
-    float clip = 1.f;
-    if (gnorm_sq && max_norm > 0.f) {
-        const float c = max_norm / (sqrtf(gnorm_sq[0]) + 1e-6f);
-        clip = c < 1.f ? c : 1.f;
-    }
+    const float clip = adamw_clip(gnorm_sq, max_norm);
     const int64_t n4 = n >> 2;
     for (int64_t i = (int64_t)blockIdx.x * blockDim.x + threadIdx.x; i < n4; i += (int64_t)gridDim.x * blockDim.x) {
         float4 pp, gg, mm, vv;
@@ -557,14 +570,7 @@
         }
         float* pa = &pp.x; float* ga = &gg.x; float* ma = &mm.x; float* va = &vv.x;
 #pragma unroll
-        for (int e = 0; e < 4; ++e) {
-            const float gr = ga[e] * clip;
-            pa[e] *= 1.f - lr * wd;
-            ma[e] = b1 * ma[e] + (1.f - b1) * gr;
-            va[e] = b2 * va[e] + (1.f - b2) * gr * gr;
-            const float denom = sqrtf(va[e]) / sqrtf(bc2) + eps;
-            pa[e] -= (lr / bc1) * (ma[e] / denom);
-        }
+        for (int e = 0; e < 4; ++e) adamw_update(pa[e], ga[e], ma[e], va[e], clip, lr, b1, b2, eps, wd, bc1, bc2);
         if (ADAMW_NT & 2) {
             __builtin_nontemporal_store(f32x4a_t{pp.x, pp.y, pp.z, pp.w}, reinterpret_cast<f32x4a_t*>(p) + i);
             __builtin_nontemporal_store(f32x4a_t{mm.x, mm.y, mm.z, mm.w}, reinterpret_cast<f32x4a_t*>(m) + i);
@@ -574,10 +580,8 @@
         }
     }
     for (int64_t i = (n4 << 2) + (int64_t)blockIdx.x * blockDim.x + threadIdx.x; i < n; i += (int64_t)gridDim.x * blockDim.x) {
-        const float gr = g[i] * clip;
-        float pv = p[i] * (1.f - lr * wd);
-        const float mv = b1 * m[i] + (1.f - b1) * gr, vv2 = b2 * v[i] + (1.f - b2) * gr * gr;
-        pv -= (lr / bc1) * (mv / (sqrtf(vv2) / sqrtf(bc2) + eps));
+        float pv = p[i], mv = m[i], vv2 = v[i];
+        adamw_update(pv, g[i], mv, vv2, clip, lr, b1, b2, eps, wd, bc1, bc2);
         p[i] = pv; m[i] = mv; v[i] = vv2;
     }
 }
@@ -634,6 +638,145 @@
     hipLaunchKernelGGL(adamw_kernel, dim3(grid), dim3(256), 0, (hipStream_t)stream, p, g, m, v, n, 0.f, beta1, beta2, eps,
                        weight_decay, 1.f, 1.f, gnorm_sq, max_norm, hyper);
     DICOW_CHECK_LAUNCH("adamw_f32_dev");
+    return DICOW_OK;
+}
+
+#define REFRESH_CHUNK 4096
+__global__ void __launch_bounds__(256) adamw_refresh_kernel(float* __restrict__ p, const float* __restrict__ g, float* __restrict__ m,
+                                                            float* __restrict__ v, const dicow_refresh_item* __restrict__ items,
+                                                            const int* __restrict__ unit0, int n_items, const float* __restrict__ hyper,
+                                                            float b1, float b2, float eps, const float* __restrict__ gnorm_sq, float max_norm) {
+    __shared__ unsigned short tile[64][68];
+    int lo = 0, hi = n_items - 1;
+    while (lo < hi) {
+        const int mid = (lo + hi + 1) >> 1;
+        if (unit0[mid] <= (int)blockIdx.x) lo = mid; else hi = mid - 1;
+    }
+    const dicow_refresh_item& it = items[lo];
+    const int u = (int)blockIdx.x - unit0[lo];
+    const int64_t start = it.start, end = it.end;
+    const int R = it.R, C = it.C;
+    const float wd = it.weight_decay;
+    const float* __restrict__ h = hyper + 3 * it.run;
+    const float lr = h[0], bc1 = h[1], bc2 = h[2];
+    const float clip = adamw_clip(gnorm_sq, max_norm);
+    float4 pp[4], gg[4], mm[4], vv[4];
+    if (R == 0) {
+        const int64_t base = start + (int64_t)u * REFRESH_CHUNK + (int64_t)threadIdx.x * 4;
+#pragma unroll
+        for (int k = 0; k < 4; ++k) {
+            const int64_t i = base + k * 1024;
+            if (i + 4 <= end) {
+                pp[k] = *reinterpret_cast<const float4*>(p + i); gg[k] = *reinterpret_cast<const float4*>(g + i);
+                mm[k] = *reinterpret_cast<const float4*>(m + i); vv[k] = *reinterpret_cast<const float4*>(v + i);
+            }
+        }
+#pragma unroll
+        for (int k = 0; k < 4; ++k) {
+            const int64_t i = base + k * 1024;
+            if (i + 4 <= end) {
+                float* pa = &pp[k].x; float* ga = &gg[k].x; float* ma = &mm[k].x; float* va = &vv[k].x;
+#pragma unroll
+                for (int e = 0; e < 4; ++e) adamw_update(pa[e], ga[e], ma[e], va[e], clip, lr, b1, b2, eps, wd, bc1, bc2);
+                *reinterpret_cast<float4*>(p + i) = pp[k]; *reinterpret_cast<float4*>(m + i) = mm[k]; *reinterpret_cast<float4*>(v + i) = vv[k];
+            } else {
+                for (int64_t j = i; j < end; ++j) {
+                    float pv = p[j], mv = m[j], vv2 = v[j];
+                    adamw_update(pv, g[j], mv, vv2, clip, lr, b1, b2, eps, wd, bc1, bc2);
+                    p[j] = pv; m[j] = mv; v[j] = vv2;
+                }
+            }
+        }
+        return;
+    }
+    unsigned short* __restrict__ dst = reinterpret_cast<unsigned short*>(it.dst);
+    unsigned short* __restrict__ dst_t = reinterpret_cast<unsigned short*>(it.dst_t);
+    const int64_t ld = it.ld, ld_t = it.ld_t;
+    const int ntc = (C + 63) / 64;
+    const int r0 = (u / ntc) * 64, c0 = (u % ntc) * 64;
+    const int tq = threadIdx.x & 15, tr = threadIdx.x >> 4;
+#pragma unroll
+    for (int k = 0; k < 4; ++k) {
+        const int r = r0 + k * 16 + tr, c = c0 + tq * 4;
+        if (r < R && c < C) {
+            const int64_t i = start + (int64_t)r * C + c;
+            pp[k] = *reinterpret_cast<const float4*>(p + i); gg[k] = *reinterpret_cast<const float4*>(g + i);
+            mm[k] = *reinterpret_cast<const float4*>(m + i); vv[k] = *reinterpret_cast<const float4*>(v + i);
+        }
+    }
+#pragma unroll
+    for (int k = 0; k < 4; ++k) {
+        const int il = k * 16 + tr, r = r0 + il, c = c0 + tq * 4;
+        uint2 q = make_uint2(0, 0);
+        if (r < R && c < C) {
+            const int64_t i = start + (int64_t)r * C + c;
+            float* pa = &pp[k].x; float* ga = &gg[k].x; float* ma = &mm[k].x; float* va = &vv[k].x;
+#pragma unroll
+            for (int e = 0; e < 4; ++e) adamw_update(pa[e], ga[e], ma[e], va[e], clip, lr, b1, b2, eps, wd, bc1, bc2);
+            *reinterpret_cast<float4*>(p + i) = pp[k]; *reinterpret_cast<float4*>(m + i) = mm[k]; *reinterpret_cast<float4*>(v + i) = vv[k];
+            q = make_uint2(pack_bf16x2(pp[k].x, pp[k].y), pack_bf16x2(pp[k].z, pp[k].w));
+            if (dst) *reinterpret_cast<uint2*>(dst + (int64_t)r * ld + c) = q;
+        }
+        *reinterpret_cast<uint2*>(&tile[il][tq * 4]) = q;
+    }
+    if (!dst_t) return;
+    __syncthreads();
+#pragma unroll
+    for (int k = 0; k < 4; ++k) {
+        const int il = k * 16 + tr, c = c0 + il, r = r0 + tq * 4;
+        if (c < C && r < R) {
+            const unsigned lo2 = (unsigned)tile[tq * 4][il] | ((unsigned)tile[tq * 4 + 1][il] << 16);
+            const unsigned hi2 = (unsigned)tile[tq * 4 + 2][il] | ((unsigned)tile[tq * 4 + 3][il] << 16);
+            *reinterpret_cast<uint2*>(dst_t + (int64_t)c * ld_t + r) = make_uint2(lo2, hi2);
+        }
+    }
+}
+
+static bool refresh_vector_ok(const dicow_refresh_item& q) {
+    return (q.R % 4 == 0) && (q.C % 4 == 0) && (q.ld % 4 == 0) && (q.ld_t % 4 == 0) && ((uintptr_t)q.dst % 8 == 0) &&
+           ((uintptr_t)q.dst_t % 8 == 0);
+}
+
+extern "C" int dicow_adamw_refresh_vector_ok(const dicow_refresh_item* item) {
+    return item && item->R > 0 && item->C > 0 && item->start % 4 == 0 && refresh_vector_ok(*item) ? 1 : 0;
+}
+
+extern "C" int dicow_adamw_refresh_plan(const dicow_refresh_item* items, int n_items, int64_t numel, int n_runs, int* unit0) {
+    DICOW_REQUIRE(items && unit0 && n_items >= 1 && numel > 0 && n_runs > 0, "adamw_refresh_plan: bad args");
+    int64_t prev_end = 0, units = 0;
+    for (int i = 0; i < n_items; ++i) {
+        const dicow_refresh_item& q = items[i];
+        DICOW_REQUIRE(q.start >= prev_end && q.end > q.start && q.end <= numel, "adamw_refresh_plan: item %d is empty, out of order, "
+                      "overlaps its predecessor or leaves the store", i);
+        DICOW_REQUIRE(q.start % 4 == 0, "adamw_refresh_plan: item %d does not start on a 16-byte boundary", i);
+        DICOW_REQUIRE(q.run >= 0 && q.run < n_runs, "adamw_refresh_plan: item %d names run %d of %d", i, q.run, n_runs);
+        unit0[i] = (int)units;
+        if (q.R == 0 && q.C == 0) {
+            units += (q.end - q.start + REFRESH_CHUNK - 1) / REFRESH_CHUNK;
+        } else {
+            DICOW_REQUIRE(q.R > 0 && q.C > 0 && q.end - q.start == (int64_t)q.R * q.C, "adamw_refresh_plan: matrix item %d: bad shape", i);
+            DICOW_REQUIRE(q.dst || q.dst_t, "adamw_refresh_plan: matrix item %d has no destination (make it a linear item)", i);
+            DICOW_REQUIRE((!q.dst || q.ld >= q.C) && (!q.dst_t || q.ld_t >= q.R), "adamw_refresh_plan: matrix item %d: leading dimensions too small", i);
+            DICOW_REQUIRE(refresh_vector_ok(q), "adamw_refresh_plan: matrix item %d does not meet the vector conditions (R, C, ld, ld_t "
+                          "multiples of 4, 8-byte destinations): make it a linear item and cast it separately", i);
+            units += (int64_t)dicow_cdiv(q.R, 64) * dicow_cdiv(q.C, 64);
+        }
+        DICOW_REQUIRE(units < (int64_t)1 << 31, "adamw_refresh_plan: more than 2^31 workgroups");
+        prev_end = q.end;
+    }
+    unit0[n_items] = (int)units;
+    return DICOW_OK;
+}
+
+extern "C" int dicow_adamw_refresh(float* p, const float* g, float* m, float* v, const dicow_refresh_item* items_dev,
+                                   const int* unit0_dev, int n_items, int n_units, const float* hyper, float beta1, float beta2,
+                                   float eps, const float* gnorm_sq, float max_norm, void* stream) {
+    DICOW_REQUIRE(p && g && m && v && items_dev && unit0_dev && n_items >= 1 && n_units >= 1 && hyper, "adamw_refresh: bad args");
+    DICOW_REQUIRE((uintptr_t)p % 16 == 0 && (uintptr_t)g % 16 == 0 && (uintptr_t)m % 16 == 0 && (uintptr_t)v % 16 == 0,
+                  "adamw_refresh: the flat buffers must be 16-byte aligned");
+    hipLaunchKernelGGL(adamw_refresh_kernel, dim3(n_units), dim3(256), 0, (hipStream_t)stream, p, g, m, v, items_dev, unit0_dev, n_items,
+                       hyper, beta1, beta2, eps, gnorm_sq, max_norm);
+    DICOW_CHECK_LAUNCH("adamw_refresh");
     return DICOW_OK;
 }
 
diff --git a/ts-asr-whisper_amd/engine.py b/ts-asr-whisper_amd/engine.py
--- a/ts-asr-whisper_amd/engine.py
+++ b/ts-asr-whisper_amd/engine.py
@@ -118,19 +118,25 @@
 _BIAS_COPIES = None
 
 
-def prep_linear(weights, biases, dev, need_t=True, n_pad=None, scale_info=None, bias_buf=None):
+def prep_linear(weights, biases, dev, need_t=True, n_pad=None, scale_info=None, bias_buf=None, keep=None, fresh=()):
     K = weights[0].shape[1]
     Ns = [w.shape[0] for w in weights]
     N = sum(Ns)
     Np = N if n_pad is None else n_pad
     lw = LinW()
     lw.N, lw.K = Np, K
-    lw.w = torch.zeros(Np, K, dtype=BF16, device=dev) if Np != N else _e((Np, K), BF16, dev)
-    lw.wt = (torch.zeros(K, Np, dtype=BF16, device=dev) if Np != N else _e((K, Np), BF16, dev)) if need_t else None
+    if keep is not None:
+        lw.w, lw.wt = keep.buffers(Np, K, need_t, dev)
+    else:
+        lw.w = torch.zeros(Np, K, dtype=BF16, device=dev) if Np != N else _e((Np, K), BF16, dev)
+        lw.wt = (torch.zeros(K, Np, dtype=BF16, device=dev) if Np != N else _e((K, Np), BF16, dev)) if need_t else None
     off = 0
     for w, n in zip(weights, Ns):
-        ops.cast_transpose_bf16(w.detach(), out=lw.w[off:off + n], out_t=None if lw.wt is None else lw.wt[:, off:off + n],
-                                ld=K, ld_t=Np)
+        out, out_t = lw.w[off:off + n], None if lw.wt is None else lw.wt[:, off:off + n]
+        if keep is not None:
+            keep.views.append((w, out, K, out_t, Np))
+        if keep is None or id(w) not in fresh:
+            ops.cast_transpose_bf16(w.detach(), out=out, out_t=out_t, ld=K, ld_t=Np)
         off += n
     if biases is None or all(b is None for b in biases):
         lw.b = None
@@ -148,15 +154,40 @@
     return lw
 
 
-def prep_attention(att, dev, fuse_qkv=True, bias_buf=None):
+class PersistentCopies:
+
+    class _Slot:
+        def __init__(self, owner, key):
+            self.owner, self.key, self.views = owner, key, owner.views
+
+        def buffers(self, N, K, need_t, dev):
+            have = self.owner._buf.get(self.key)
+            if have is None or have[0].shape != (N, K) or have[0].device != dev or (have[1] is None) == need_t:
+                have = (torch.zeros(N, K, dtype=BF16, device=dev), torch.zeros(K, N, dtype=BF16, device=dev) if need_t else None)
+                self.owner._buf[self.key] = have
+                self.owner.version += 1
+            return have
+
+    def __init__(self):
+        self._buf, self.views, self.version = {}, [], 0
+
+    def begin(self):
+        self.views = []
+
+    def slot(self, key):
+        return self._Slot(self, key)
+
+
+def prep_attention(att, dev, fuse_qkv=True, bias_buf=None, keep=None, fresh=()):
+    slot = (lambda name: None) if keep is None else (lambda name: keep[0].slot(keep[1] + (name,)))
     a = NS()
     if fuse_qkv:
         a.qkv = prep_linear([att.q_proj.weight, att.k_proj.weight, att.v_proj.weight],
-                            [att.q_proj.bias, None, att.v_proj.bias], dev, bias_buf=bias_buf)
+                            [att.q_proj.bias, None, att.v_proj.bias], dev, bias_buf=bias_buf, keep=slot("qkv"), fresh=fresh)
     else:
-        a.q = prep_linear([att.q_proj.weight], [att.q_proj.bias], dev)
-        a.kv = prep_linear([att.k_proj.weight, att.v_proj.weight], [None, att.v_proj.bias], dev)
-    a.o = prep_linear([att.out_proj.weight], [att.out_proj.bias], dev)
+        a.q = prep_linear([att.q_proj.weight], [att.q_proj.bias], dev, keep=slot("q"), fresh=fresh)
+        a.kv = prep_linear([att.k_proj.weight, att.v_proj.weight], [None, att.v_proj.bias], dev, keep=slot("kv"), fresh=fresh)
+    a.o = prep_linear([att.out_proj.weight], [att.out_proj.bias], dev, keep=slot("o"), fresh=fresh)
     return a
 
 
@@ -444,7 +475,7 @@
         self.enc = enc
         self.cfg = enc.config
 
-    def prepare(self):
+    def prepare(self, fresh=()):
         enc, cfg = self.enc, self.cfg
         dev = enc.conv1.weight.device
         D, M = cfg.d_model, cfg.num_mel_bins
@@ -452,35 +483,55 @@
         W.k1 = _ceil(3 * M, 64)
         W.conv1, W.conv1_t = ops.conv_weight_pack(enc.conv1.weight.detach(), W.k1, want_t=True)
         W.conv2, W.conv2_t = ops.conv_weight_pack(enc.conv2.weight.detach(), 3 * D, want_t=True)
-        W.layers = []
         global _BIAS_COPIES
         if getattr(self, "_qkv_bias", None) is None or self._qkv_bias[0].device != dev:
             self._qkv_bias = [torch.zeros(3 * D, dtype=F32, device=dev) for _ in enc.layers]
-        _BIAS_COPIES = []
-        for li, lyr in enumerate(enc.layers):
-            w = NS()
-            with ops.cast_group():
-                w.att = prep_attention(lyr.self_attn, dev, bias_buf=self._qkv_bias[li])
-                w.fc1 = prep_linear([lyr.fc1.weight], [lyr.fc1.bias], dev)
-                w.fc2 = prep_linear([lyr.fc2.weight], [lyr.fc2.bias], dev)
-            W.layers.append(w)
-        if _BIAS_COPIES:
-            torch._foreach_copy_([d for d, _ in _BIAS_COPIES], [s_ for _, s_ in _BIAS_COPIES])
-        _BIAS_COPIES = None
+        if getattr(self, "_copies", None) is None:
+            self._copies = PersistentCopies()
+        prev, keep = getattr(self, "W", None), self._copies
+        n_layer = getattr(self, "_n_layer_views", 0)
+        if fresh and prev is not None and n_layer and prev.conv1.device == dev and all(id(v[0]) in fresh for v in keep.views[:n_layer]):
+            W.layers = prev.layers
+            if self._bias_pairs:
+                torch._foreach_copy_([d for d, _ in self._bias_pairs], [s_ for _, s_ in self._bias_pairs])
+            del keep.views[n_layer:]
+        else:
+            W.layers = []
+            keep.begin()
+            _BIAS_COPIES = []
+            for li, lyr in enumerate(enc.layers):
+                w = NS()
+                with ops.cast_group():
+                    w.att = prep_attention(lyr.self_attn, dev, bias_buf=self._qkv_bias[li], keep=(keep, ("layer", li)), fresh=fresh)
+                    w.fc1 = prep_linear([lyr.fc1.weight], [lyr.fc1.bias], dev, keep=keep.slot(("layer", li, "fc1")), fresh=fresh)
+                    w.fc2 = prep_linear([lyr.fc2.weight], [lyr.fc2.bias], dev, keep=keep.slot(("layer", li, "fc2")), fresh=fresh)
+                W.layers.append(w)
+            if _BIAS_COPIES:
+                torch._foreach_copy_([d for d, _ in _BIAS_COPIES], [s_ for _, s_ in _BIAS_COPIES])
+            self._bias_pairs, _BIAS_COPIES = _BIAS_COPIES, None
+            self._n_layer_views = len(keep.views)
         W.scb = []
         if cfg.use_enrollments and cfg.scb_layers:
-            for blk in enc.ca_enrolls:
+            for bi, blk in enumerate(enc.ca_enrolls):
                 s = NS()
                 with ops.cast_group():
-                    s.att = prep_attention(blk.cae.cross_attn, dev, fuse_qkv=False)
-                    s.f0 = prep_linear([blk.cae.ffn[0].weight], [blk.cae.ffn[0].bias], dev)
-                    s.f3 = prep_linear([blk.cae.ffn[3].weight], [blk.cae.ffn[3].bias], dev)
+                    s.att = prep_attention(blk.cae.cross_attn, dev, fuse_qkv=False, keep=(keep, ("scb", bi)), fresh=fresh)
+                    s.f0 = prep_linear([blk.cae.ffn[0].weight], [blk.cae.ffn[0].bias], dev, keep=keep.slot(("scb", bi, "f0")), fresh=fresh)
+                    s.f3 = prep_linear([blk.cae.ffn[3].weight], [blk.cae.ffn[3].bias], dev, keep=keep.slot(("scb", bi, "f3")), fresh=fresh)
                 W.scb.append(s)
+        return self._prepare_rest(W, dev)
+
+    def _prepare_rest(self, W, dev):
+        enc, cfg = self.enc, self.cfg
         W.full_init = prep_full_fddt(enc.initial_fddt, dev) if (cfg.use_fddt and cfg.use_pre_pos_fddt and fddt_is_full(enc.initial_fddt)) else None
         W.full = [prep_full_fddt(f, dev) if fddt_is_full(f) else None for f in (enc.fddts if cfg.use_fddt else [])]
         W.fold = None
         self.W = W
         return W
+
+    def matrix_copies(self):
+        keep = getattr(self, "_copies", None)
+        return (0, []) if keep is None else (keep.version, list(keep.views))
 
     def prepare_fold(self):
         W, enc = self.W, self.enc
diff --git a/ts-asr-whisper_amd/modeling.py b/ts-asr-whisper_amd/modeling.py
--- a/ts-asr-whisper_amd/modeling.py
+++ b/ts-asr-whisper_amd/modeling.py
@@ -347,12 +347,23 @@
         if self._eng is None:
             self._eng = EncoderEngine(self)
         if prepare:
-            ctc_ids = {id(p) for p in self.ctc_parameters()} if self.ctc_weight > 0.0 else set()
-            sig = _param_sig([p for p in self.parameters() if id(p) not in ctc_ids])
+            sig = self._main_sig()
             if sig != self._sig:
-                self._eng.prepare()
+                held = self._sig
+                fused = isinstance(held, tuple) and len(held) == 3 and held[0] == "fused" and held[1] == sig
+                self._eng.prepare(fresh=held[2] if fused else ())
                 self._sig = sig
         return self._eng
+
+    def _main_sig(self):
+        ctc_ids = {id(p) for p in self.ctc_parameters()} if self.ctc_weight > 0.0 else set()
+        return _param_sig([p for p in self.parameters() if id(p) not in ctc_ids])
+
+    def copies_written_by_optimizer(self, ids):
+        held = self._sig
+        if isinstance(held, tuple) and len(held) == 3 and held[0] == "fused":
+            held = held[1]
+        self._sig = None if held is None else ("fused", held, frozenset(ids))
 
     def get_max_len(self):
         return self.config.max_source_positions * 2
diff --git a/ts-asr-whisper_amd/ops.py b/ts-asr-whisper_amd/ops.py
--- a/ts-asr-whisper_amd/ops.py
+++ b/ts-asr-whisper_amd/ops.py
@@ -578,6 +578,72 @@
            eps, wd, _p(gnorm_sq), max_norm, L.stream())
 
 
+class AdamwRefreshPlan:
+
+    def __init__(self, numel, n_runs, ranges, matrices, device):
+        items, self.fused, self._keep = [], [], []
+        mats = sorted(range(len(matrices)), key=lambda i: matrices[i][0])
+        accepted = {}
+        for i in mats:
+            off, R, Cc, out, out_t = matrices[i]
+            it = L.RefreshItem()
+            it.start, it.end, it.R, it.C = off, off + R * Cc, R, Cc
+            ok = (out is not None or out_t is not None) and R > 0 and Cc > 0
+            for t, shape in ((out, (R, Cc)), (out_t, (Cc, R))):
+                if t is not None:
+                    _req(t, BF16, "adamw_refresh.dst")
+                    assert tuple(t.shape) == shape and t.stride(1) == 1, "adamw_refresh: destination views are [R, C] / [C, R], unit column stride"
+            it.dst, it.ld = _p(out), (Cc if out is None else out.stride(0))
+            it.dst_t, it.ld_t = _p(out_t), (R if out_t is None else out_t.stride(0))
+            accepted[i] = it if ok and L.lib().dicow_adamw_refresh_vector_ok(C.byref(it)) == 1 else None
+        self.fused = [accepted[i] is not None for i in range(len(matrices))]
+        order = [accepted[i] for i in mats if accepted[i] is not None]
+        k = 0
+        for a, b, run, wd in ranges:
+            cur = a
+            while k < len(order) and order[k].start < b:
+                it = order[k]
+                assert it.start >= cur and it.end <= b, "adamw_refresh: a matrix straddles the ranges"
+                if it.start > cur:
+                    items.append(self._linear(cur, it.start, run, wd))
+                it.run, it.weight_decay = run, wd
+                items.append(it)
+                cur = it.end
+                k += 1
+            if b > cur:
+                items.append(self._linear(cur, b, run, wd))
+        assert k == len(order), "adamw_refresh: a matrix lies outside the ranges"
+        for i, f in enumerate(self.fused):
+            if f:
+                self._keep += [matrices[i][3], matrices[i][4]]
+        self.n_items = len(items)
+        self.n_units = 0
+        if not items:
+            return
+        arr = (L.RefreshItem * len(items))(*items)
+        unit0 = (C.c_int * (len(items) + 1))()
+        L.call("dicow_adamw_refresh_plan", arr, len(items), int(numel), int(n_runs), unit0)
+        self.n_units = int(unit0[len(items)])
+        self.items = torch.frombuffer(bytearray(bytes(arr)), dtype=torch.uint8).to(device)
+        self.unit0 = torch.tensor(list(unit0), dtype=torch.int32).to(device)
+
+    @staticmethod
+    def _linear(a, b, run, wd):
+        it = L.RefreshItem()
+        it.start, it.end, it.run, it.weight_decay = a, b, run, wd
+        return it
+
+
+def adamw_refresh(plan, p, g, m, v, hyper, beta1, beta2, eps, gnorm_sq=None, max_norm=0.0):
+    if plan.n_items == 0:
+        return
+    for t in (p, g, m, v):
+        _req(t, F32, "adamw_refresh")
+        assert t.is_contiguous() and t.numel() == p.numel()
+    L.call("dicow_adamw_refresh", p.data_ptr(), g.data_ptr(), m.data_ptr(), v.data_ptr(), plan.items.data_ptr(), plan.unit0.data_ptr(),
+           plan.n_items, plan.n_units, hyper.data_ptr(), beta1, beta2, eps, _p(gnorm_sq), max_norm, L.stream())
+
+
 def multi_adamw(tensors_ptr, chunks_ptr, n_chunks, classes, cls_base=0, clip_coef=None):
     L.check(L.lib().dicow_multi_adamw_f32(tensors_ptr, chunks_ptr, n_chunks, C.byref(classes), cls_base, _p(clip_coef), L.stream()),
             "dicow_multi_adamw_f32")
diff --git a/ts-asr-whisper_amd/trainer.py b/ts-asr-whisper_amd/trainer.py
--- a/ts-asr-whisper_amd/trainer.py
+++ b/ts-asr-whisper_amd/trainer.py
@@ -159,6 +159,30 @@
         self.counters = torch.zeros(1 + len(store.runs), dtype=torch.int32, device=dev)
         self.hyper = torch.zeros(len(store.runs), 3, dtype=F32, device=dev)
         self.is_pre = torch.tensor([int(pre) for _, _, pre in store.runs], dtype=torch.int32, device=dev)
+        self._mats, self._mats_key, self._plans = [], None, {}
+
+    def set_matrices(self, key, mats):
+        if key == self._mats_key:
+            return False
+        self._mats, self._mats_key, self._plans = list(mats), key, {}
+        return True
+
+    def plan(self, preheat_only=False):
+        pl = self._plans.get(bool(preheat_only))
+        if pl is None:
+            s = self.s
+            ranges = [(a, b, i, 0.0 if pre else self.wd) for i, (a, b, pre) in enumerate(s.runs) if pre or not preheat_only]
+            where = {id(p): (o, n) for p, o, n, _ in getattr(s, "entries", ())}
+            mats, owners = [], []
+            if not preheat_only:
+                for p, out, ld, out_t, ld_t in self._mats:
+                    if id(p) in where and p.dim() == 2 and where[id(p)][1] == p.numel():
+                        mats.append((where[id(p)][0], p.shape[0], p.shape[1], out, out_t))
+                        owners.append(p)
+            pl = ops.AdamwRefreshPlan(s.params.numel(), len(s.runs), ranges, mats, s.params.device)
+            pl.fused_ids = frozenset(id(p) for p, f in zip(owners, pl.fused) if f)
+            self._plans[bool(preheat_only)] = pl
+        return pl
 
     def sync_counters(self):
         self.counters.copy_(torch.tensor([self.t] + list(self.run_t), dtype=torch.int32))
@@ -189,15 +213,14 @@
                 int(self.schedule == "cosine"), float(self.betas[0]), float(self.betas[1]), L_.stream())
         self.gnorm_sq.zero_()
         ops.sumsq(s.grads, self.gnorm_sq)
-        for i, (a, b, pre) in enumerate(s.runs):
-            if preheat_only and not pre:
-                continue
-            ops.adamw_dev(s.params[a:b], s.grads[a:b], s.exp_avg[a:b], s.exp_avg_sq[a:b], self.hyper[i], self.betas[0], self.betas[1],
-                          self.eps, 0.0 if pre else self.wd, gnorm_sq=self.gnorm_sq, max_norm=self.max_norm)
+        pl = self.plan(preheat_only)
+        ops.adamw_refresh(pl, s.params, s.grads, s.exp_avg, s.exp_avg_sq, self.hyper, self.betas[0], self.betas[1], self.eps,
+                          gnorm_sq=self.gnorm_sq, max_norm=self.max_norm)
+        return pl
 
     def step(self, preheat_only=False):
         self.advance(preheat_only)
-        self.launch(preheat_only)
+        return self.launch(preheat_only)
 
 
 def _bit_checksum(t):
@@ -522,13 +545,26 @@
             self.reducer.finish()
         if self.first_writer and not self.warmup_phase:
             self.store.settle_first_writers()
+        self._bind_matrix_copies()
         with tracing.range("optimizer"):
-            self.opt.step(preheat_only=self.warmup_phase)
+            pl = self.opt.step(preheat_only=self.warmup_phase)
         enc = self.model.model.encoder
         if not (self.warmup_phase and self._preheat_is_vectors_only):
-            enc._sig = None
+            fused = getattr(pl, "fused_ids", None)
+            if fused and not self.warmup_phase:
+                enc.copies_written_by_optimizer(fused)
+            else:
+                enc._sig = None
             enc._ctc_sig = None
         self._invalidate_decoder_copies()
+
+    def _bind_matrix_copies(self):
+        eng = getattr(self.model.model.encoder, "_eng", None)
+        if eng is None:
+            return
+        version, views = eng.matrix_copies()
+        if self.opt.set_matrices((id(eng), version), views):
+            self._graphs.clear()
 
     def _micro(self, batch, scale):
         if self.split_streams and self._can_split(batch):
@@ -640,17 +676,18 @@
                 self._graph_pool = torch.cuda.graph_pool_handle()
             static = self._clone(batch)
             self._invalidate_weight_copies()
+            self._bind_matrix_copies()
             torch.cuda.synchronize()
             g = torch.cuda.CUDAGraph()
             with torch.cuda.graph(g, pool=self._graph_pool):
                 self.store.zero_grad(first_writer=self.first_writer and not self.warmup_phase)
                 out = self.model(**static)
                 out.loss.backward()
-                self.opt.launch(preheat_only=self.warmup_phase)
+                plan = self.opt.launch(preheat_only=self.warmup_phase)
                 loss = out.loss.detach()
-            self._graphs[key] = (g, static, loss)
+            self._graphs[key] = (g, static, loss, plan)
         self._graphs.move_to_end(key)
-        g, static, loss = self._graphs[key]
+        g, static, loss, _ = self._graphs[key]
         self._copy_into(static, batch)
         self.opt.advance(preheat_only=self.warmup_phase)
         g.replay()
```

Measured after the change: 128.3 utt/s, median of 6. 1.02x the previous value.
